# Jan-Celin/SCCG-genome-compression

Measured on AMD Instinct MI355X. Metric: target bases compressed/sec at 1/2/4/8 GPUs; bit-exact record stream vs CPU ref, higher is better.
Workload: dtype u8

## Files before the change

### sccg-genome-compression_amd/csrc/common.h

```cpp
#pragma once

#include <hip/hip_runtime.h>
#include <stdint.h>

#define SCCG_WAVE 64
#define SCCG_BLOCK 256

__host__ __device__ __forceinline__ bool c_isspace(uint8_t c) { return c == ' ' || (c >= 9 && c <= 13); }
__host__ __device__ __forceinline__ bool c_islower(uint8_t c) { return c >= 'a' && c <= 'z'; }
__host__ __device__ __forceinline__ uint8_t c_toupper(uint8_t c) { return c_islower(c) ? (uint8_t)(c - 32) : c; }
__host__ __device__ __forceinline__ uint8_t c_tolower(uint8_t c) { return (c >= 'A' && c <= 'Z') ? (uint8_t)(c + 32) : c; }
__host__ __device__ __forceinline__ uint32_t base2(uint8_t c) {
    return c == 'A' ? 0u : c == 'C' ? 1u : c == 'G' ? 2u : c == 'T' ? 3u : 4u;
}

#define KEY_EXOTIC 0x80000000u
__host__ __device__ __forceinline__ uint32_t exotic_key(const uint8_t* s, int k) {
    uint32_t h = 2166136261u;
    for (int i = 0; i < k; i++) { h ^= s[i]; h *= 16777619u; }
    return KEY_EXOTIC | (h & 0x7fffffffu);
}
__host__ __device__ __forceinline__ uint32_t kmer_key(const uint8_t* s, int k) {
    uint32_t code = 0;
    for (int i = 0; i < k; i++) {
        uint32_t b = base2(s[i]);
        if (b > 3) return exotic_key(s, k);
        code = (code << 2) | b;
    }
    return code;
}
__host__ __device__ __forceinline__ uint32_t slot_hash(uint32_t key, int bits) {
    return (key * 0x9E3779B1u) >> (32 - bits);
}
__host__ __device__ __forceinline__ int ndigits_u32(uint32_t v) {
    int n = 1;
    while (v >= 10) { v /= 10; n++; }
    return n;
}
__host__ __device__ __forceinline__ int ndigits_i32(int32_t v) {
    return v < 0 ? 1 + ndigits_u32((uint32_t)0 - (uint32_t)v) : ndigits_u32((uint32_t)v);
}
__device__ __forceinline__ int write_i32(uint8_t* dst, int32_t v) {
    uint32_t u = v < 0 ? (uint32_t)0 - (uint32_t)v : (uint32_t)v;
    int n = ndigits_u32(u) + (v < 0);
    int w = n;
    do { dst[--w] = (uint8_t)('0' + u % 10); u /= 10; } while (u);
    if (v < 0) dst[0] = '-';
    return n;
}

__device__ __forceinline__ uint32_t swar_codes(uint32_t w, uint32_t& diff) {
    const uint32_t c = ((w >> 1) ^ (w >> 2)) & 0x03030303u;
    diff = __builtin_amdgcn_perm(0x54474341u, 0x54474341u, c) ^ w;
    const uint32_t p = c | (c >> 6);
    return (p | (p >> 12)) & 0xffu;
}
__device__ __forceinline__ uint32_t nz_bytes(uint32_t diff) {
    const uint32_t nz = ((((diff & 0x7f7f7f7fu) + 0x7f7f7f7fu) | diff) & 0x80808080u) >> 7;
    return (nz | (nz >> 7) | (nz >> 14) | (nz >> 21)) & 0xfu;
}
template <int ND>
__device__ __forceinline__ void pack_codes(const uint32_t (&w)[ND], uint64_t& code, uint32_t& bad) {
    uint32_t d[ND], acc = 0;
    code = 0;
#pragma unroll
    for (int i = 0; i < ND; i++) {
        code |= (uint64_t)swar_codes(w[i], d[i]) << (8 * i);
        acc |= d[i];
    }
    bad = 0;
    if (acc) {
#pragma unroll
        for (int i = 0; i < ND; i++) bad |= nz_bytes(d[i]) << (4 * i);
    }
}
template <int ND>
__device__ __forceinline__ void loadw(const uint8_t* p, uint32_t (&o)[ND]) {
    const uint32_t sh = (uint32_t)((uintptr_t)p & 3);
    const uint32_t* w = reinterpret_cast<const uint32_t*>(p - sh);
    uint32_t v[ND + 1];
#pragma unroll
    for (int i = 0; i <= ND; i++) v[i] = w[i];
#pragma unroll
    for (int i = 0; i < ND; i++) o[i] = __builtin_amdgcn_alignbyte(v[i + 1], v[i], sh);
}
__device__ __forceinline__ uint32_t walk_key(const uint8_t* s, int k) {
    uint32_t code = 0;
    for (int i = 0; i < k; i++) {
        const uint32_t b = base2(s[i]);
        if (b > 3) return exotic_key(s, k);
        code |= b << (2 * i);
    }
    return code;
}

__device__ __forceinline__ int lane_id() { return (int)(threadIdx.x & 63); }
__device__ __forceinline__ int wave_in_block() { return (int)(threadIdx.x >> 6); }

__device__ __forceinline__ void wave_sync() {
    __builtin_amdgcn_fence(__ATOMIC_RELEASE, "wavefront");
    __builtin_amdgcn_wave_barrier();
    __builtin_amdgcn_fence(__ATOMIC_ACQUIRE, "wavefront");
}

template <typename T>
__device__ __forceinline__ T wave_incl_add(T v) {
    const int lane = lane_id();
#pragma unroll
    for (int d = 1; d < 64; d <<= 1) {
        T o = __shfl_up(v, d, 64);
        if (lane >= d) v += o;
    }
    return v;
}
__device__ __forceinline__ uint32_t wave_incl_add_dpp(uint32_t v) {
    v += (uint32_t)__builtin_amdgcn_update_dpp(0, (int)v, 0x111, 0xf, 0xf, true);
    v += (uint32_t)__builtin_amdgcn_update_dpp(0, (int)v, 0x112, 0xf, 0xf, true);
    v += (uint32_t)__builtin_amdgcn_update_dpp(0, (int)v, 0x114, 0xf, 0xf, true);
    v += (uint32_t)__builtin_amdgcn_update_dpp(0, (int)v, 0x118, 0xf, 0xf, true);
    v += (uint32_t)__builtin_amdgcn_update_dpp(0, (int)v, 0x142, 0xa, 0xf, false);
    v += (uint32_t)__builtin_amdgcn_update_dpp(0, (int)v, 0x143, 0xc, 0xf, false);
    return v;
}
template <typename T>
__device__ __forceinline__ T wave_sum(T v) {
#pragma unroll
    for (int d = 32; d > 0; d >>= 1) v += __shfl_xor(v, d, 64);
    return v;
}
template <typename T>
__device__ __forceinline__ T wave_max(T v) {
#pragma unroll
    for (int d = 32; d > 0; d >>= 1) { T o = __shfl_xor(v, d, 64); v = o > v ? o : v; }
    return v;
}
template <typename T>
__device__ __forceinline__ T wave_min(T v) {
#pragma unroll
    for (int d = 32; d > 0; d >>= 1) { T o = __shfl_xor(v, d, 64); v = o < v ? o : v; }
    return v;
}
__device__ __forceinline__ int first_lane(unsigned long long m) { return m ? __ffsll((long long)m) - 1 : 64; }
__device__ __forceinline__ int32_t uni(int32_t v) { return __builtin_amdgcn_readfirstlane(v); }
__device__ __forceinline__ int32_t lane_val(int32_t v, int l) { return __builtin_amdgcn_readlane(v, l); }
__device__ __forceinline__ uint32_t lane_val(uint32_t v, int l) { return (uint32_t)__builtin_amdgcn_readlane((int32_t)v, l); }

template <typename T>
__device__ __forceinline__ T block_excl_add(T v, T* tmp, T* total) {
    T incl = wave_incl_add(v);
    const int w = wave_in_block(), lane = lane_id();
    if (lane == 63) tmp[w] = incl;
    __syncthreads();
    if (threadIdx.x == 0) {
        T s = 0;
        for (int i = 0; i < (int)(blockDim.x >> 6); i++) { T t = tmp[i]; tmp[i] = s; s += t; }
        tmp[4] = s;
    }
    __syncthreads();
    T r = incl - v + tmp[w];
    if (total) *total = tmp[4];
    __syncthreads();
    return r;
}

#define SCCG_HIP(expr)                                              \
    do {                                                            \
        hipError_t e_ = (expr);                                     \
        if (e_ != hipSuccess) return sccg_hip_fail(e_, #expr, __FILE__, __LINE__); \
    } while (0)

int sccg_hip_fail(hipError_t e, const char* what, const char* file, int line);

static inline unsigned grid_for(int64_t n, int per_block) {
    int64_t g = (n + per_block - 1) / per_block;
    return (unsigned)(g < 1 ? 1 : g);
}
```

### sccg-genome-compression_amd/csrc/ingest.hip

```cpp
#include "internal.h"

namespace {

constexpr int PER_T = INGEST_TILE / SCCG_BLOCK;
constexpr int WPB = SCCG_BLOCK / 64;


constexpr int64_t FM_CHUNK = 16384;
template <int NW>
__device__ __forceinline__ uint8_t wb(const uint32_t (&w)[NW], int i) { return (uint8_t)(w[i >> 2] >> (8 * (i & 3))); }
template <int NW>
__device__ __forceinline__ void load_words(const uint8_t* __restrict__ buf, int64_t n, int64_t off, uint32_t (&w)[NW]);
__global__ __launch_bounds__(SCCG_BLOCK) void k_first_match(const uint8_t* __restrict__ buf, int64_t n,
                                                            const int64_t* __restrict__ from_slot, int mode, uint8_t c,
                                                            int64_t* __restrict__ res, unsigned int* __restrict__ ticket) {
    __shared__ int64_t s_cs;
    const int64_t from = from_slot ? *from_slot + 1 : 0;
    const int64_t base = from & ~(int64_t)63;
    constexpr int PER = FM_CHUNK / SCCG_BLOCK;
    for (;;) {
        if (threadIdx.x == 0) {
            const int64_t cs = base + (int64_t)atomicAdd(ticket, 1u) * FM_CHUNK;
            const int64_t best = (int64_t)__hip_atomic_load((unsigned long long*)res, __ATOMIC_RELAXED, __HIP_MEMORY_SCOPE_AGENT);
            s_cs = (cs >= n || cs >= best) ? -1 : cs;
// ... 198 lines not shown
        if (c == '(') par |= bit;
    }
    const uint64_t fk = ~drop;
    const int64_t lim = n - off;
    const uint64_t valid = lim >= 64 ? ~0ull : (lim > 0 ? (1ull << lim) - 1ull : 0ull);
    StripMasks r{0, 0, fk, par, -1, lo, nn, odd ? 1ull : 0ull};
    if (MODE == INGEST_TGT) {
        const int64_t lo = h - off < 0 ? 0 : (h - off > 64 ? 64 : h - off);
        const int64_t hi = he - off < 0 ? 0 : (he - off > 64 ? 64 : he - off);
        r.known = ~ws & valid & ~(below64((int)hi) & ~below64((int)lo));
        return r;
    }
    const uint64_t ls = ((nl << 1) | (uint64_t)(off == 0 || prev == '\n')) & valid;
    const int first = ls ? __builtin_ctzll(ls) : 64;
    r.unknown = ~ws & valid & below64(first);
    uint64_t keep = 0;
    if ((gt & ls) == 0) {
        keep = ~below64(first);
        r.last = ls ? 1 : -1;
    } else {
        uint64_t rem = ls;
        while (rem) {
            const int j = __builtin_ctzll(rem);
            rem &= rem - 1;
            const int nx = rem ? __builtin_ctzll(rem) : 64;
            const int32_t st = !((gt >> j) & 1ull);
            if (st) keep |= below64(nx) & ~below64(j);
            r.last = st;
        }
    }
    r.known = ~ws & valid & keep;
    return r;
}

template <IngestMode MODE, bool RUNS = false, bool ODD = false>
__device__ __forceinline__ StripMasks strip_tile(FilterMode fm, const uint8_t* __restrict__ buf, int64_t n, int64_t h,
                                                 int64_t he, int64_t off, uint32_t (&w)[SNW], int32_t& prior,
                                                 uint64_t& lsm, uint4* tin) {
    const int lane = lane_id();
    load_words<SNW>(buf, n, off, w);
    wave_sync();
#pragma unroll
    for (int q = 0; q < SNW / 4; q++) tin[4 * lane + q] = make_uint4(w[4 * q], w[4 * q + 1], w[4 * q + 2], w[4 * q + 3]);
    wave_sync();
    uint8_t prev = '\n';
    if (MODE == INGEST_REF) {
        const uint32_t up = (uint32_t)__shfl_up((int)w[SNW - 1], 1, 64) >> 24;
        prev = lane ? (uint8_t)up : ((off > 0 && off - 1 < n) ? buf[off - 1] : (uint8_t)'\n');
    }
    const StripMasks r = strip_masks<MODE, RUNS, ODD>(fm, w, prev, off, n, h, he, reinterpret_cast<const uint8_t*>(tin + 4 * lane));
    wave_sync();
    prior = -1;
    lsm = 0;
    if (MODE == INGEST_REF) {
        lsm = __ballot(r.last >= 0);
        const uint64_t m = lsm & below64(lane);
        const int src = m ? 63 - __builtin_clzll(m) : 0;
        const int32_t v = __shfl(r.last, src, 64);
        prior = m ? v : -1;
    }
    return r;
}

template <IngestMode MODE, bool KC>
__global__ __launch_bounds__(SCCG_BLOCK) void k_strip_summary(FilterMode fm, const uint8_t* __restrict__ buf, int64_t n,
                                                              const int64_t* __restrict__ hdr, int64_t* __restrict__ ta,
                                                              int64_t* __restrict__ tb, int64_t* __restrict__ tfa,
                                                              int64_t* __restrict__ tfb, int32_t* __restrict__ tlast,
                                                              uint16_t* __restrict__ kc, int32_t* __restrict__ kflag) {
    __shared__ uint4 tin_all[WPB][STRIP_WTILE / 16];
    const int64_t tile = (int64_t)blockIdx.x * WPB + wave_in_block();
    if (tile * STRIP_WTILE >= n) return;
    const int lane = lane_id();
    const int64_t off = tile * STRIP_WTILE + (int64_t)lane * SL;
    const int64_t h = MODE == INGEST_TGT ? hdr[0] : 0, he = MODE == INGEST_TGT ? hdr[1] : 0;
    uint32_t w[SNW];
    int32_t prior;
    uint64_t lsm;
    const StripMasks r = strip_tile<MODE, false, KC>(fm, buf, n, h, he, off, w, prior, lsm, tin_all[wave_in_block()]);
    if (KC) {
        const uint64_t hole = ~(r.known | (prior != 0 ? r.unknown : 0ull));
        const uint32_t h1 = hole ? (uint32_t)__builtin_ctzll(hole) : 64u, h2 = hole ? 63u - (uint32_t)__builtin_clzll(hole) : 64u;
        kc[tile * 64 + lane] = (uint16_t)(h1 | (h2 << 7));
        const uint64_t odd = __ballot(r.odd != 0 || __popcll(hole) > 2);
        const uint64_t sens = __ballot(MODE == INGEST_REF && prior < 0 && r.unknown != 0);
        if (lane == 0) kflag[tile] = (odd ? 0 : 1) | (sens ? 2 : 0);
    }
    const uint64_t ra = (uint64_t)__popcll(r.unknown), rb = (uint64_t)__popcll(r.known);
    const uint64_t rfa = (uint64_t)__popcll(r.unknown & r.fk), rfb = (uint64_t)__popcll(r.known & r.fk);
    const uint64_t A = prior < 0 ? ra : 0, B = rb + (prior == 1 ? ra : 0);
    const uint64_t FA = prior < 0 ? rfa : 0, FB = rfb + (prior == 1 ? rfa : 0);
    const uint32_t t_ab = lane_val(wave_incl_add_dpp((uint32_t)(A | (B << 16))), 63);
    const uint32_t t_f = lane_val(wave_incl_add_dpp((uint32_t)(FA | (FB << 16))), 63);
    const uint64_t tot = (uint64_t)t_ab | ((uint64_t)t_f << 32);
    if (lane == 0) {
        ta[tile] = (int64_t)(tot & 0xffff);
        tb[tile] = (int64_t)((tot >> 16) & 0xffff);
        tfa[tile] = (int64_t)((tot >> 32) & 0xffff);
        tfb[tile] = (int64_t)(tot >> 48);
    }
    if (MODE == INGEST_REF) {
        const int32_t last = lsm ? __shfl(r.last, 63 - __builtin_clzll(lsm), 64) : -1;
        if (lane == 0) tlast[tile] = last;
    } else if (lane == 0) {
        tlast[tile] = -1;
    }
}

struct TileSum {
    int64_t a, b, fa, fb;
    int32_t last;
};
__device__ __forceinline__ TileSum ts_compose(const TileSum& x, const TileSum& y) {
    TileSum r;
    r.a = x.a + (x.last < 0 ? y.a : 0);
    r.b = x.b + y.b + (x.last == 1 ? y.a : 0);
    r.fa = x.fa + (x.last < 0 ? y.fa : 0);
    r.fb = x.fb + y.fb + (x.last == 1 ? y.fa : 0);
    r.last = y.last >= 0 ? y.last : x.last;
    return r;
}
__device__ __forceinline__ TileSum ts_shfl_up(const TileSum& v, int d) {
    TileSum r;
    r.a = __shfl_up(v.a, d, 64); r.b = __shfl_up(v.b, d, 64);
    r.fa = __shfl_up(v.fa, d, 64); r.fb = __shfl_up(v.fb, d, 64);
    r.last = __shfl_up(v.last, d, 64);
    return r;
}

constexpr int SCAN_B = 1024;
__device__ __forceinline__ TileSum block_scan_tiles(TileSum v, TileSum* wsum, TileSum* total) {
    const TileSum id{0, 0, 0, 0, -1};
    const int lane = lane_id(), w = (int)(threadIdx.x >> 6), nw = (int)(blockDim.x >> 6);
    TileSum incl = v;
#pragma unroll
    for (int d = 1; d < 64; d <<= 1) {
        const TileSum o = ts_shfl_up(incl, d);
        if (lane >= d) incl = ts_compose(o, incl);
    }
    if (lane == 63) wsum[w] = incl;
    __syncthreads();
    if (threadIdx.x == 0) {
        TileSum run = id;
        for (int i = 0; i < nw; i++) { const TileSum x = wsum[i]; wsum[i] = run; run = ts_compose(run, x); }
        wsum[16] = run;
    }
    __syncthreads();
    TileSum ex = ts_shfl_up(incl, 1);
    if (lane == 0) ex = id;
    if (total) *total = wsum[16];
    return ts_compose(wsum[w], ex);
}

constexpr int SCAN_T = 1024, SCAN_PER = SCAN_B / SCAN_T;
__global__ __launch_bounds__(SCAN_T) void k_strip_scan_local(int64_t ntiles, int64_t* __restrict__ ta, int64_t* __restrict__ tb,
                                                          int64_t* __restrict__ tfa, int64_t* __restrict__ tfb,
                                                          int32_t* __restrict__ tlast, TileSum* __restrict__ btot) {
    __shared__ TileSum wsum[17];
    const TileSum id{0, 0, 0, 0, -1};
    const int64_t t0 = (int64_t)blockIdx.x * SCAN_B + (int64_t)threadIdx.x * SCAN_PER;
    TileSum v[SCAN_PER], agg = id;
#pragma unroll
    for (int k = 0; k < SCAN_PER; k++) {
        const int64_t t = t0 + k;
        v[k] = t < ntiles ? TileSum{ta[t], tb[t], tfa[t], tfb[t], tlast[t]} : id;
        agg = ts_compose(agg, v[k]);
    }
    TileSum tot;
    TileSum run = block_scan_tiles(agg, wsum, &tot);
#pragma unroll
    for (int k = 0; k < SCAN_PER; k++) {
        const int64_t t = t0 + k;
        if (t < ntiles) { ta[t] = run.a; tb[t] = run.b; tfa[t] = run.fa; tfb[t] = run.fb; tlast[t] = run.last; }
        run = ts_compose(run, v[k]);
    }
    if (threadIdx.x == 0) btot[blockIdx.x] = tot;
}

__global__ __launch_bounds__(SCAN_T) void k_strip_scan_blocks(int64_t nblk, TileSum* __restrict__ btot) {
    __shared__ TileSum wsum[17];
    const TileSum id{0, 0, 0, 0, -1};
    const int64_t i0 = (int64_t)threadIdx.x * SCAN_PER;
    TileSum v[SCAN_PER], agg = id;
#pragma unroll
    for (int k = 0; k < SCAN_PER; k++) {
        v[k] = i0 + k < nblk ? btot[i0 + k] : id;
        agg = ts_compose(agg, v[k]);
    }
    TileSum tot;
    TileSum run = block_scan_tiles(agg, wsum, &tot);
#pragma unroll
    for (int k = 0; k < SCAN_PER; k++) {
        if (i0 + k < nblk) btot[i0 + k] = run;
        run = ts_compose(run, v[k]);
    }
    if (threadIdx.x == 0) btot[SCAN_B] = tot;
}

__global__ void k_strip_scan_apply(int64_t ntiles, const int64_t* __restrict__ ta, const int64_t* __restrict__ tb,
                                   const int64_t* __restrict__ tfa, const int64_t* __restrict__ tfb,
                                   const int32_t* __restrict__ tlast, const TileSum* __restrict__ btot,
                                   int64_t* __restrict__ toff, int64_t* __restrict__ toff2, int32_t* __restrict__ tcarry,
                                   int64_t* __restrict__ d_len, int64_t* __restrict__ d_len2) {
    const TileSum start{0, 0, 0, 0, 1};
    for (int64_t t = (int64_t)blockIdx.x * blockDim.x + threadIdx.x; t < ntiles; t += (int64_t)gridDim.x * blockDim.x) {
        const TileSum r = ts_compose(ts_compose(start, btot[t / SCAN_B]), TileSum{ta[t], tb[t], tfa[t], tfb[t], tlast[t]});
        toff[t] = r.b;
        toff2[t] = r.fb;
        tcarry[t] = r.last;
    }
    if (blockIdx.x == 0 && threadIdx.x == 0) {
        const TileSum r = ts_compose(start, btot[SCAN_B]);
        *d_len = r.b;
        if (d_len2) *d_len2 = r.fb;
    }
}

__device__ __forceinline__ void run_events(uint64_t p, uint64_t K, uint32_t cin, uint64_t& st, uint64_t& en) {
    const uint64_t D = ~K;
    const uint64_t x = p & K;
    const uint64_t sd = ((x << 1) | cin) & D;
    const uint64_t g = x | (D & ~(D + sd));
    const uint64_t prev = (g << 1) | cin;
    st = K & g & ~prev;
    en = K & ~g & prev;
}

template <IngestMode MODE, bool RUNS>
__global__ __launch_bounds__(SCCG_BLOCK) void k_strip_write(FilterMode fm, const uint8_t* __restrict__ buf, int64_t n,
                                                            const int64_t* __restrict__ hdr,
                                                            const int64_t* __restrict__ toff,
                                                            const int64_t* __restrict__ toff2,
                                                            const int32_t* __restrict__ tcarry,
                                                            uint8_t* __restrict__ out, uint8_t* __restrict__ out2,
                                                            int32_t* __restrict__ flags, RunSlots rsl,
                                                            const uint16_t* __restrict__ kc, const int32_t* __restrict__ kflag) {
    __shared__ uint4 stage_all4[WPB][(STAGE_WORDS + 3) / 4];
    __shared__ uint32_t tab[16];
    if (threadIdx.x < 16) tab[threadIdx.x] = compact_sel(threadIdx.x);
    __syncthreads();
    const int64_t tile = (int64_t)blockIdx.x * WPB + wave_in_block();
    if (tile * STRIP_WTILE >= n) return;
    const int lane = lane_id();
    uint32_t* st4 = reinterpret_cast<uint32_t*>(stage_all4[wave_in_block()]);
    uint8_t* s1 = reinterpret_cast<uint8_t*>(st4);
    const int64_t off = tile * STRIP_WTILE + (int64_t)lane * SL;
    const int64_t h = MODE == INGEST_TGT ? hdr[0] : 0, he = MODE == INGEST_TGT ? hdr[1] : 0;
    uint32_t w[SNW];
    int32_t prior;
    uint64_t lsm;
    StripMasks r;
    const int32_t kf = kc ? uni(kflag[tile]) : 0;
    if ((kf & 1) && (MODE == INGEST_TGT || !(kf & 2) || uni(tcarry[tile]) == 1)) {
        load_words<SNW>(buf, n, off, w);
        const uint32_t code = kc[tile * 64 + lane], h1 = code & 127u, h2 = code >> 7;
        const uint64_t keep = ~((h1 < 64 ? 1ull << h1 : 0ull) | (h2 < 64 ? 1ull << h2 : 0ull));
        r = StripMasks{keep, 0ull, ~0ull, 0ull, -1, RUNS ? lower_fast(w) : 0ull, 0ull, 0ull};
        prior = 1;
    } else {
        r = strip_tile<MODE, RUNS>(fm, buf, n, h, he, off, w, prior, lsm, stage_all4[wave_in_block()]);
        if (MODE == INGEST_REF && prior < 0) prior = tcarry[tile];
    }
    const uint64_t keep = r.known | (prior == 1 ? r.unknown : 0ull), fkeep = keep & r.fk;
    const uint32_t c = (uint32_t)__popcll(keep) | ((uint32_t)__popcll(fkeep) << 16);
    const uint32_t incl = wave_incl_add_dpp(c), tot = lane_val(incl, 63);
    const uint32_t ex = incl - c;
    if (RUNS) {
        const bool has = keep != 0;
        const int fb = has ? __builtin_ctzll(keep) : 0, lb = has ? 63 - __builtin_clzll(keep) : 0;
        const uint32_t first2 = (uint32_t)((r.lower >> fb) & 1u) | ((uint32_t)((r.nn >> fb) & 1u) << 1);
        const uint32_t last2 = (uint32_t)((r.lower >> lb) & 1u) | ((uint32_t)((r.nn >> lb) & 1u) << 1);
        const uint64_t hm = __ballot(has);
        const uint64_t before = hm & below64(lane);
        const int src = before ? 63 - __builtin_clzll(before) : 0;
        const uint32_t pl = (uint32_t)__shfl((int)last2, src, 64);
        const uint32_t cin = before ? pl : first2;
        uint64_t sl = 0, el = 0, sn = 0, en = 0;
        if (has) {
            run_events(r.lower, keep, cin & 1u, sl, el);
            run_events(r.nn, keep, cin >> 1, sn, en);
        }
        const uint64_t cc = (uint64_t)__popcll(sl) | ((uint64_t)__popcll(el) << 16) | ((uint64_t)__popcll(sn) << 32) |
                            ((uint64_t)__popcll(en) << 48);
        const uint32_t ci_lo = wave_incl_add_dpp((uint32_t)cc), ci_hi = wave_incl_add_dpp((uint32_t)(cc >> 32));
        const uint64_t ci = (uint64_t)ci_lo | ((uint64_t)ci_hi << 32);
        const uint64_t ct = (uint64_t)lane_val(ci_lo, 63) | ((uint64_t)lane_val(ci_hi, 63) << 32);
        const uint64_t cx = ci - cc;
        const int fl = hm ? first_lane(hm) : 0, ll = hm ? 63 - __builtin_clzll(hm) : 0;
        const uint32_t tf = (uint32_t)__shfl((int)first2, fl, 64), tl = (uint32_t)__shfl((int)last2, ll, 64);
        if (lane == 0) {
            rsl.rc[tile] = ct;
            rsl.rf[tile] = (hm ? 1 : 0) | (int32_t)(tf << 1) | (int32_t)(tl << 3);
        }
        if ((sl | el | sn | en) != 0) {
            const int64_t o0 = toff[tile] + (int64_t)(ex & 0xffff);
            int32_t* const dst[4] = {rsl.sl, rsl.el, rsl.sn, rsl.en};
            const uint64_t ev[4] = {sl, el, sn, en};
#pragma unroll
            for (int q = 0; q < 4; q++) {
                uint32_t at = (uint32_t)(cx >> (16 * q)) & 0xffffu;
                for (uint64_t m = ev[q]; m; m &= m - 1) {
                    const int b = __builtin_ctzll(m);
                    if (at < RUN_SLOT) dst[q][(size_t)tile * RUN_SLOT + at] = (int32_t)(o0 + __popcll(keep & below64(b)));
                    else atomicOr(rsl.ovf, 1);
                    at++;
                }
            }
        }
    }
    if (flags && __ballot((keep & r.par) != 0) && lane == 0) atomicOr(flags, 1);
    if (out) {
        stage_lane<false>(s1, tab, w, keep, (int)(ex & 0xffff));
        wave_sync();
        stage_out(st4, (int)(tot & 0xffff), out, toff[tile]);
    }
    if (out2) {
        if (out && !__ballot(fkeep != keep)) {
            stage_out<true>(st4, (int)(tot >> 16), out2, toff2[tile]);
        } else {
            wave_sync();
            stage_lane<true>(s1, tab, w, fkeep, (int)(ex >> 16));
            wave_sync();
            stage_out(st4, (int)(tot >> 16), out2, toff2[tile]);
        }
    }
}

template <IngestMode MODE>
__global__ __launch_bounds__(64) void k_strip_gather(const uint8_t* __restrict__ buf, int64_t n,
                                                     const int64_t* __restrict__ hdr, const int64_t* __restrict__ toff,
                                                     const int32_t* __restrict__ tcarry, const int64_t* __restrict__ d_len,
                                                     const int32_t* __restrict__ segs, uint8_t* __restrict__ dst) {
    __shared__ uint4 tin[STRIP_WTILE / 16];
    const int lane = lane_id();
    const int32_t seg = segs[blockIdx.x];
    if (seg < 0) return;
    const int64_t len = *d_len;
    const int64_t q0 = (int64_t)seg * SEG_L;
    const int64_t q1 = q0 + SEG_L < len ? q0 + SEG_L : len;
    uint8_t* out = dst + (size_t)blockIdx.x * SEG_GATHER_B;
    if (q0 >= q1) return;
    const int64_t ntiles = (n + STRIP_WTILE - 1) / STRIP_WTILE;
    int64_t lo = 0, hi = ntiles - 1;
    while (lo < hi) {
        const int64_t span = hi - lo;
        const int64_t p = lo + (span * (lane + 1) + 63) / 64;
        const bool le = p <= hi && toff[p] <= q0;
        const unsigned long long m = __ballot(le);
        if (!m) { hi = lo + (span + 63) / 64 - 1; if (hi < lo) hi = lo; continue; }
        const int l = 63 - __builtin_clzll(m);
        const int64_t pl = lo + (span * (l + 1) + 63) / 64;
        const int64_t pn = l < 63 ? lo + (span * (l + 2) + 63) / 64 - 1 : hi;
        lo = pl;
        hi = pn < hi ? pn : hi;
        if (hi < lo) hi = lo;
    }
    const int64_t h = MODE == INGEST_TGT ? hdr[0] : 0, he = MODE == INGEST_TGT ? hdr[1] : 0;
    for (int64_t tile = lo; tile < ntiles && toff[tile] < q1; tile++) {
        const int64_t off = tile * STRIP_WTILE + (int64_t)lane * SL;
        uint32_t w[SNW];
        int32_t prior;
        uint64_t lsm;
        const StripMasks r = strip_tile<MODE>(FILTER_UPPER, buf, n, h, he, off, w, prior, lsm, tin);
        int32_t pr = prior;
        if (MODE == INGEST_REF && pr < 0) pr = tcarry[tile];
        const uint64_t keep = r.known | (pr == 1 ? r.unknown : 0ull);
        const uint32_t c = (uint32_t)__popcll(keep);
        const uint32_t ex = wave_incl_add<uint32_t>(c) - c;
        int64_t pos = toff[tile] + ex;
        if (pos < q1 && pos + c > q0) {
            for (uint64_t m = keep; m; m &= m - 1, pos++) {
                const int b = __builtin_ctzll(m);
                if (pos >= q0 && pos < q1) out[pos - q0] = (uint8_t)(w[b >> 2] >> (8 * (b & 3)));
            }
        }
        wave_sync();
    }
}

__device__ __forceinline__ bool run_pred(RunPred p, uint8_t c) {
    return p == RUN_LOWER ? c_islower(c) : (c == 'N' || c == 'n');
}

__device__ __forceinline__ void pred_masks(const uint8_t* __restrict__ in, int64_t n, int64_t off, uint32_t& ml,
                                           uint32_t& mn) {
    uint32_t w[PER_T / 4];
    load_words(in, n, off, w);
    ml = 0;
    mn = 0;
#pragma unroll
    for (int q = 0; q < PER_T / 4; q++) {
        const uint32_t x = w[q];
        ml |= sw_bits(sw_lt(x, 'z' + 1) & ~sw_lt(x, 'a')) << (4 * q);
        mn |= sw_bits(sw_eq(x, 'N') | sw_eq(x, 'n')) << (4 * q);
    }
}

__global__ __launch_bounds__(SCCG_BLOCK) void k_runs_count(const uint8_t* __restrict__ in, int64_t n,
                                                           int64_t* __restrict__ cnt_l, int64_t* __restrict__ cnt_n) {
    __shared__ int32_t tmp32[8];
    const int64_t off = (int64_t)blockIdx.x * INGEST_TILE + (int64_t)threadIdx.x * PER_T;
    uint32_t ml, mn;
    pred_masks(in, n, off, ml, mn);
    const bool in_prev = off > 0 && off - 1 < n;
    const uint32_t pl = in_prev && run_pred(RUN_LOWER, in[off - 1]), pn = in_prev && run_pred(RUN_N, in[off - 1]);
    const int32_t c = __popc(ml & ~((ml << 1) | pl)) | (__popc(mn & ~((mn << 1) | pn)) << 16);
    int32_t tot;
    block_excl_add<int32_t>(c, tmp32, &tot);
    if (threadIdx.x == 0) { cnt_l[blockIdx.x] = tot & 0xffff; cnt_n[blockIdx.x] = tot >> 16; }
}

__device__ __forceinline__ void put_positions(uint32_t bits, int64_t off, int32_t* __restrict__ dst, int64_t at) {
    while (bits) {
        dst[at++] = (int32_t)(off + __ffs((int)bits) - 1);
        bits &= bits - 1;
    }
}

__global__ __launch_bounds__(SCCG_BLOCK) void k_runs_write(const uint8_t* __restrict__ in, int64_t n,
                                                           const int64_t* __restrict__ toff_l,
                                                           const int64_t* __restrict__ toff_n, int32_t* __restrict__ rs_l,
                                                           int32_t* __restrict__ re_l, int32_t* __restrict__ rs_n,
                                                           int32_t* __restrict__ re_n) {
    __shared__ int32_t tmp32[8];
    const int64_t tile0 = (int64_t)blockIdx.x * INGEST_TILE;
    const int64_t off = tile0 + (int64_t)threadIdx.x * PER_T;
    uint32_t ml, mn;
    pred_masks(in, n, off, ml, mn);
    const bool in_prev = off > 0 && off - 1 < n, in_next = off + PER_T < n;
    const uint32_t pl = in_prev && run_pred(RUN_LOWER, in[off - 1]), pn = in_prev && run_pred(RUN_N, in[off - 1]);
    const uint32_t nl = in_next && run_pred(RUN_LOWER, in[off + PER_T]), nn = in_next && run_pred(RUN_N, in[off + PER_T]);
    const uint32_t sl = ml & ~((ml << 1) | pl), el = ml & ~((ml >> 1) | (nl << 31));
    const uint32_t sn = mn & ~((mn << 1) | pn), en = mn & ~((mn >> 1) | (nn << 31));
    const bool t_in = tile0 > 0 && tile0 < n;
    const bool open_l = t_in && run_pred(RUN_LOWER, in[tile0 - 1]) && run_pred(RUN_LOWER, in[tile0]);
    const bool open_n = t_in && run_pred(RUN_N, in[tile0 - 1]) && run_pred(RUN_N, in[tile0]);
    const int32_t xs = block_excl_add<int32_t>(__popc(sl) | (__popc(sn) << 16), tmp32, nullptr);
    const int32_t xe = block_excl_add<int32_t>(__popc(el) | (__popc(en) << 16), tmp32, nullptr);
    put_positions(sl, off, rs_l, toff_l[blockIdx.x] + (xs & 0xffff));
    put_positions(el, off, re_l, toff_l[blockIdx.x] - (open_l ? 1 : 0) + (xe & 0xffff));
    put_positions(sn, off, rs_n, toff_n[blockIdx.x] + (xs >> 16));
    put_positions(en, off, re_n, toff_n[blockIdx.x] - (open_n ? 1 : 0) + (xe >> 16));
}

constexpr int RUNS_LOOKBACK = 64;
__global__ void k_runs_tiles(int64_t ntiles, const uint64_t* __restrict__ rc, const int32_t* __restrict__ rf,
                             int64_t* __restrict__ cs, int64_t* __restrict__ ce, int32_t* __restrict__ bev,
                             int32_t* __restrict__ ovf) {
    for (int64_t t = (int64_t)blockIdx.x * blockDim.x + threadIdx.x; t < ntiles; t += (int64_t)gridDim.x * blockDim.x) {
        const int32_t f = rf[t];
        const uint64_t c = rc[t];
        int32_t b = 0;
        if (f & 1) {
            uint32_t prev = 0;
            int64_t q = t - 1;
            for (; q >= 0 && t - q <= RUNS_LOOKBACK; q--) {
                const int32_t g = rf[q];
                if (g & 1) { prev = (uint32_t)(g >> 3) & 3u; break; }
            }
            if (q >= 0 && t - q > RUNS_LOOKBACK) atomicOr(ovf, 2);
            const uint32_t first = (uint32_t)(f >> 1) & 3u;
#pragma unroll
            for (int p = 0; p < 2; p++) {
                const uint32_t fp = (first >> p) & 1u, pp = (prev >> p) & 1u;
                if (fp && !pp) b |= 1 << (2 * p);
                if (!fp && pp) b |= 2 << (2 * p);
            }
        }
        bev[t] = b;
        cs[t] = (int64_t)((c & 0xffff) + (b & 1)) | ((int64_t)(((c >> 32) & 0xffff) + ((b >> 2) & 1)) << 32);
        ce[t] = (int64_t)(((c >> 16) & 0xffff) + ((b >> 1) & 1)) | ((int64_t)((c >> 48) + ((b >> 3) & 1)) << 32);
    }
}

__global__ void k_runs_copy(int64_t ntiles, const int64_t* __restrict__ toff, const uint64_t* __restrict__ rc,
                            const int32_t* __restrict__ bev, const int64_t* __restrict__ cs, const int64_t* __restrict__ ce,
                            RunSlots rsl, int32_t* __restrict__ rs_l, int32_t* __restrict__ re_l,
                            int32_t* __restrict__ rs_n, int32_t* __restrict__ re_n) {
    for (int64_t t = (int64_t)blockIdx.x * blockDim.x + threadIdx.x; t < ntiles; t += (int64_t)gridDim.x * blockDim.x) {
        const uint64_t c = rc[t];
        const int32_t b = bev[t];
        const int32_t t0 = (int32_t)toff[t];
        const size_t sb = (size_t)t * RUN_SLOT;
        int32_t* const dst[4] = {rs_l, re_l, rs_n, re_n};
        const int32_t* const src[4] = {rsl.sl, rsl.el, rsl.sn, rsl.en};
        const int64_t base[4] = {cs[t] & 0xffffffff, ce[t] & 0xffffffff, cs[t] >> 32, ce[t] >> 32};
#pragma unroll
        for (int q = 0; q < 4; q++) {
            const int end = q & 1;
            int64_t at = base[q];
            if ((b >> q) & 1) dst[q][at++] = t0 - end;
            const int nq = (int)((c >> (16 * q)) & 0xffff);
            for (int k = 0; k < nq && k < RUN_SLOT; k++) dst[q][at++] = src[q][sb + k] - end;
        }
    }
}

__global__ void k_runs_fin(const int64_t* __restrict__ tot, const int64_t* __restrict__ d_nT, int32_t* __restrict__ re_l,
                           int32_t* __restrict__ re_n, int64_t* __restrict__ d_nruns) {
    const int64_t sl = tot[0] & 0xffffffff, sn = tot[0] >> 32, el = tot[1] & 0xffffffff, en = tot[1] >> 32;
    if (sl > el) re_l[sl - 1] = (int32_t)(*d_nT - 1);
    if (sn > en) re_n[sn - 1] = (int32_t)(*d_nT - 1);
    d_nruns[0] = sl;
    d_nruns[1] = sn;
}

__device__ __forceinline__ int64_t run_text_len(int32_t d, int32_t len, bool at_end) {
    return len == 1 ? (int64_t)ndigits_i32(d) + (at_end ? 0 : 1) : (int64_t)(3 + ndigits_i32(d) + ndigits_i32(len));
}

__global__ void k_run_textlen(const int32_t* __restrict__ rs, const int32_t* __restrict__ re, int64_t nr,
                              int64_t n, int64_t* __restrict__ len) {
    for (int64_t r = (int64_t)blockIdx.x * blockDim.x + threadIdx.x; r < nr; r += (int64_t)gridDim.x * blockDim.x) {
        const int32_t d = rs[r] - (r ? rs[r - 1] : 0);
        len[r] = run_text_len(d, re[r] - rs[r] + 1, (int64_t)re[r] == n - 1);
    }
}

__global__ void k_run_textwrite(const int32_t* __restrict__ rs, const int32_t* __restrict__ re, int64_t nr,
                                int64_t n, const int64_t* __restrict__ off, uint8_t* __restrict__ out) {
    for (int64_t r = (int64_t)blockIdx.x * blockDim.x + threadIdx.x; r < nr; r += (int64_t)gridDim.x * blockDim.x) {
        const int32_t d = rs[r] - (r ? rs[r - 1] : 0);
        const int32_t len = re[r] - rs[r] + 1;
        uint8_t* o = out + off[r];
        if (len == 1) {
            o += write_i32(o, d);
            if ((int64_t)re[r] != n - 1) *o = ',';
        } else {
            *o++ = '(';
            o += write_i32(o, d);
            *o++ = ',';
            o += write_i32(o, len);
            *o = ')';
        }
    }
}

}

constexpr int FH_T = 256, FH_PER = 64;
__global__ __launch_bounds__(FH_T) void k_find_header(const uint8_t* __restrict__ buf, int64_t n, int64_t* __restrict__ d_sc) {
    __shared__ unsigned long long s_hit;
    int64_t res[2] = {n, n};
    for (int ph = 0; ph < 2; ph++) {
        if (ph == 1 && res[0] >= n) break;
        const int64_t from = ph == 0 ? 0 : res[0] + 1;
        for (int64_t cs = from & ~(int64_t)63; cs < n; cs += (int64_t)FH_T * FH_PER) {
            if (threadIdx.x == 0) s_hit = ~0ull;
            __syncthreads();
            const int64_t p0 = cs + (int64_t)threadIdx.x * FH_PER;
            if (p0 < n) {
                uint32_t w[FH_PER / 4];
                load_words<FH_PER / 4>(buf, n, p0, w);
                uint8_t prev = p0 > 0 ? buf[p0 - 1] : (uint8_t)'\n';
                int64_t hit = -1;
#pragma unroll
                for (int i = 0; i < FH_PER; i++) {
                    const uint8_t c = wb(w, i);
                    const int64_t p = p0 + i;
                    const bool ok = p >= from && p < n && (ph == 0 ? (c == '>' && prev == '\n') : c == '\n');
                    if (ok && hit < 0) hit = p;
                    prev = c;
                }
                if (hit >= 0) atomicMin(&s_hit, (unsigned long long)hit);
            }
            __syncthreads();
            const unsigned long long h = s_hit;
            __syncthreads();
            if (h != ~0ull) { res[ph] = (int64_t)h; break; }
        }
    }
    if (threadIdx.x == 0) { d_sc[0] = res[0]; d_sc[1] = res[1]; d_sc[2] = 0; d_sc[3] = 0; }
}

int launch_first_match(const uint8_t* buf, int64_t n, const int64_t* from_slot, int mode, uint8_t c, int64_t* res,
                       int64_t* ticket_slot, hipStream_t s) {
    int rc = dev_set_i64(res, 1, {n}, s);
    if (!rc) rc = dev_set_i64(ticket_slot, 1, {0}, s);
    if (rc) return rc;
    if (n > 0) {
        hipLaunchKernelGGL(k_first_match, dim3(64), dim3(SCCG_BLOCK), 0, s, buf, n, from_slot, mode, c, res,
                           reinterpret_cast<unsigned int*>(ticket_slot));
        SCCG_HIP(hipGetLastError());
    }
    return 0;
}

int launch_find_header(const uint8_t* buf, int64_t n, int64_t* d_sc, hipStream_t s) {
    hipLaunchKernelGGL(k_find_header, dim3(1), dim3(FH_T), 0, s, buf, n, d_sc);
    SCCG_HIP(hipGetLastError());
    return 0;
}

int launch_fasta_strip(IngestMode mode, const uint8_t* buf, int64_t n, const int64_t* d_header, uint8_t* out,
                       int64_t* d_len, int32_t* d_flags, const IngestScratch& sc, hipStream_t s, FilterMode fmode,
                       uint8_t* out2, int64_t* d_len2, const RunSlots* runs) {
    if (n <= 0) {
        SCCG_HIP(hipMemsetAsync(d_len, 0, sizeof(int64_t), s));
        if (d_len2) SCCG_HIP(hipMemsetAsync(d_len2, 0, sizeof(int64_t), s));
        return 0;
    }
    if (!out2) fmode = FILTER_UPPER;
    const int64_t ntiles = (n + STRIP_TILE - 1) / STRIP_TILE;
    const unsigned g = grid_for(ntiles, WPB);
    uint16_t* const kc = sc.keep_cache;
    int32_t* const kf = sc.keep_flag;
#define SUMMARY(M, K)                                                                                                   \
    hipLaunchKernelGGL((k_strip_summary<M, K>), dim3(g), dim3(SCCG_BLOCK), 0, s, fmode, buf, n, d_header, sc.tile_a,   \
                       sc.tile_b, sc.tile_fa, sc.tile_fb, sc.tile_last, kc, kf)
    if (mode == INGEST_TGT && kc) SUMMARY(INGEST_TGT, true);
    else if (mode == INGEST_TGT) SUMMARY(INGEST_TGT, false);
    else if (kc) SUMMARY(INGEST_REF, true);
    else SUMMARY(INGEST_REF, false);
#undef SUMMARY
    const int64_t nblk = (ntiles + SCAN_B - 1) / SCAN_B;
    if (nblk > SCAN_B) return SCCG_E_UNSUPPORTED;
    TileSum* btot = reinterpret_cast<TileSum*>(sc.block_sums);
    hipLaunchKernelGGL(k_strip_scan_local, dim3((unsigned)nblk), dim3(SCAN_T), 0, s, ntiles, sc.tile_a, sc.tile_b,
                       sc.tile_fa, sc.tile_fb, sc.tile_last, btot);
    hipLaunchKernelGGL(k_strip_scan_blocks, dim3(1), dim3(SCAN_T), 0, s, nblk, btot);
    hipLaunchKernelGGL(k_strip_scan_apply, dim3(grid_for(ntiles, 256)), dim3(256), 0, s, ntiles, sc.tile_a, sc.tile_b,
                       sc.tile_fa, sc.tile_fb, sc.tile_last, btot, sc.tile_off, sc.tile_off2, sc.tile_carry, d_len,
                       d_len2);
    const RunSlots rsl = runs ? *runs : RunSlots{};
    if (mode == INGEST_TGT && runs)
        PROF_LAUNCH(PROF_STRIP, s, (k_strip_write<INGEST_TGT, true>), dim3(g), dim3(SCCG_BLOCK), 0, s, fmode, buf, n, d_header,
                    sc.tile_off, sc.tile_off2, sc.tile_carry, out, out2, d_flags, rsl, (const uint16_t*)kc, (const int32_t*)kf);
    else if (mode == INGEST_TGT)
        PROF_LAUNCH(PROF_STRIP, s, (k_strip_write<INGEST_TGT, false>), dim3(g), dim3(SCCG_BLOCK), 0, s, fmode, buf, n, d_header,
                    sc.tile_off, sc.tile_off2, sc.tile_carry, out, out2, d_flags, rsl, (const uint16_t*)kc, (const int32_t*)kf);
    else
        PROF_LAUNCH(PROF_STRIP, s, (k_strip_write<INGEST_REF, false>), dim3(g), dim3(SCCG_BLOCK), 0, s, fmode, buf, n, d_header,
                    sc.tile_off, sc.tile_off2, sc.tile_carry, out, out2, d_flags, rsl, (const uint16_t*)kc, (const int32_t*)kf);
    SCCG_HIP(hipGetLastError());
    return 0;
}

int launch_runs2(const uint8_t* in, int64_t n, int32_t* rs_l, int32_t* re_l, int32_t* rs_n, int32_t* re_n,
                 int64_t* d_nruns, int64_t* d_cnt_l, int64_t* d_cnt_n, int64_t* d_partial, hipStream_t s) {
    if (n <= 0) {
        SCCG_HIP(hipMemsetAsync(d_nruns, 0, 2 * sizeof(int64_t), s));
        return 0;
    }
    const int64_t ntiles = (n + INGEST_TILE - 1) / INGEST_TILE;
    hipLaunchKernelGGL(k_runs_count, dim3((unsigned)ntiles), dim3(SCCG_BLOCK), 0, s, in, n, d_cnt_l, d_cnt_n);
    int rc = dev_excl_sum(d_cnt_l, d_cnt_l, ntiles, d_nruns, d_partial, s);
    if (!rc) rc = dev_excl_sum(d_cnt_n, d_cnt_n, ntiles, d_nruns + 1, d_partial, s);
    if (rc) return rc;
    PROF_LAUNCH(PROF_RUNS, s, k_runs_write, dim3((unsigned)ntiles), dim3(SCCG_BLOCK), 0, s, in, n,
                (const int64_t*)d_cnt_l, (const int64_t*)d_cnt_n, rs_l, re_l, rs_n, re_n);
    SCCG_HIP(hipGetLastError());
    return 0;
}

int launch_runs_from_strip(const RunSlots& rs, int64_t ntiles, const int64_t* toff, const int64_t* d_nT, int32_t* rs_l,
                           int32_t* re_l, int32_t* rs_n, int32_t* re_n, int64_t* d_nruns, int64_t* cs, int64_t* ce,
                           int32_t* bev, int64_t* d_tot, int64_t* d_partial, hipStream_t s) {
    const unsigned g = grid_for(ntiles, 256) > 4096 ? 4096 : grid_for(ntiles, 256);
    hipLaunchKernelGGL(k_runs_tiles, dim3(g), dim3(256), 0, s, ntiles, (const uint64_t*)rs.rc, (const int32_t*)rs.rf, cs, ce,
                       bev, rs.ovf);
    if (const int rc = dev_excl_sum2(cs, cs, d_tot, ce, ce, d_tot + 1, ntiles, d_partial, s)) return rc;
    PROF_LAUNCH(PROF_RUNS, s, k_runs_copy, dim3(g), dim3(256), 0, s, ntiles, toff, (const uint64_t*)rs.rc, (const int32_t*)bev,
                (const int64_t*)cs, (const int64_t*)ce, rs, rs_l, re_l, rs_n, re_n);
    hipLaunchKernelGGL(k_runs_fin, dim3(1), dim3(1), 0, s, (const int64_t*)d_tot, d_nT, re_l, re_n, d_nruns);
    SCCG_HIP(hipGetLastError());
    return 0;
}

int launch_run_text(const int32_t* rs, const int32_t* re, int64_t nruns, int64_t n, uint8_t* out, int64_t* d_len,
                    int64_t* d_tmp, int64_t* d_partial, hipStream_t s) {
    if (nruns <= 0) {
        SCCG_HIP(hipMemsetAsync(d_len, 0, sizeof(int64_t), s));
        return 0;
    }
    const unsigned g = grid_for(nruns, 256) > 4096 ? 4096 : grid_for(nruns, 256);
    hipLaunchKernelGGL(k_run_textlen, dim3(g), dim3(256), 0, s, rs, re, nruns, n, d_tmp);
    int rc = dev_excl_sum(d_tmp, d_tmp, nruns, d_len, d_partial, s);
    if (rc) return rc;
    PROF_LAUNCH(PROF_RUNTEXT, s, k_run_textwrite, dim3(g), dim3(256), 0, s, rs, re, nruns, n, (const int64_t*)d_tmp, out);
    SCCG_HIP(hipGetLastError());
    return 0;
}

int launch_strip_gather(IngestMode mode, const uint8_t* buf, int64_t n, const int64_t* d_header, const int64_t* toff,
                        const int32_t* tcarry, const int64_t* d_len, const int32_t* segs, int nslots, uint8_t* dst,
                        hipStream_t s) {
    if (n <= 0 || nslots <= 0) return 0;
    if (mode == INGEST_TGT)
        hipLaunchKernelGGL(k_strip_gather<INGEST_TGT>, dim3(nslots), dim3(64), 0, s, buf, n, d_header, toff, tcarry, d_len,
                           segs, dst);
    else
        hipLaunchKernelGGL(k_strip_gather<INGEST_REF>, dim3(nslots), dim3(64), 0, s, buf, n, d_header, toff, tcarry, d_len,
                           segs, dst);
    SCCG_HIP(hipGetLastError());
    return 0;
}

int launch_strip_rewrite(IngestMode mode, const uint8_t* buf, int64_t n, const int64_t* d_header, uint8_t* out,
                         const IngestScratch& sc, hipStream_t s) {
    if (n <= 0) return 0;
    const int64_t ntiles = (n + STRIP_TILE - 1) / STRIP_TILE;
    const unsigned g = grid_for(ntiles, WPB);
    const RunSlots rsl{};
    if (mode == INGEST_TGT)
        PROF_LAUNCH(PROF_STRIP, s, (k_strip_write<INGEST_TGT, false>), dim3(g), dim3(SCCG_BLOCK), 0, s, FILTER_UPPER, buf, n,
                    d_header, sc.tile_off, sc.tile_off2, sc.tile_carry, out, (uint8_t*)nullptr, (int32_t*)nullptr, rsl,
                    (const uint16_t*)nullptr, (const int32_t*)nullptr);
    else
        PROF_LAUNCH(PROF_STRIP, s, (k_strip_write<INGEST_REF, false>), dim3(g), dim3(SCCG_BLOCK), 0, s, FILTER_UPPER, buf, n,
                    d_header, sc.tile_off, sc.tile_off2, sc.tile_carry, out, (uint8_t*)nullptr, (int32_t*)nullptr, rsl,
                    (const uint16_t*)nullptr, (const int32_t*)nullptr);
    SCCG_HIP(hipGetLastError());
    return 0;
}
```

### sccg-genome-compression_amd/csrc/internal.h

```cpp
#pragma once

#include "common.h"
#include "../../include/sccg.h"

enum ProfId {
    PROF_STRIP = 0,
    PROF_RUNS,
    PROF_RUNTEXT,
    PROF_LOCAL14,
    PROF_LOCAL10,
    PROF_LOCAL_EMIT,
    PROF_FILTER,
    PROF_ANCHOR,
    PROF_WALK,
    PROF_PRESENCE,
    PROF_FULLC,
    PROF_MATCH_EMIT,
    PROF_WALK_CHAIN,
    PROF_DC_DECODE,
    PROF_DC_FORMAT,
    PROF_WALK_CARRY,
    PROF_FETCH,
    PROF_COUNT
};
void prof_begin(hipStream_t s, int id);
void prof_end(hipStream_t s, int id);
#define PROF_LAUNCH(id, strm, ...)        \
    do {                                  \
        prof_begin(strm, id);             \
        hipLaunchKernelGGL(__VA_ARGS__);  \
        prof_end(strm, id);               \
    } while (0)

#include <initializer_list>
struct RbItem {
    const void* src;
    void* dst;
    int bytes;
};
int dev_readback(const RbItem* items, int n, hipStream_t s);
int dev_set_i64(int64_t* p, int n, std::initializer_list<int64_t> vals, hipStream_t s);
int dev_set_i32(int32_t* p, int n, std::initializer_list<int32_t> vals, hipStream_t s);
int dev_put_bytes(uint8_t* p, const char* bytes, int n, hipStream_t s);
int dev_put_frame(uint8_t* out, const uint8_t* hdr, int64_t hlen, int64_t total, hipStream_t s);
int dev_put_framed(uint8_t* dst, const uint8_t* src, int64_t n, char pre, char post, hipStream_t s);
int64_t scan_partials_needed(int64_t n);
int dev_excl_sum(const int64_t* in, int64_t* out, int64_t n, int64_t* d_total, int64_t* d_partial,
                 hipStream_t s);
int dev_excl_sum2(const int64_t* in0, int64_t* out0, int64_t* d_total0, const int64_t* in1, int64_t* out1,
                  int64_t* d_total1, int64_t n, int64_t* d_partial, hipStream_t s);
int dev_excl_max(const int64_t* in, int64_t* out, int64_t n, int64_t* d_total, int64_t* d_partial,
                 hipStream_t s);

constexpr int INGEST_TILE = 8192;
constexpr int STRIP_TILE = 4096;
enum IngestMode { INGEST_REF = 0, INGEST_TGT = 1 };
enum FilterMode { FILTER_DROP_N_UPPER = 0, FILTER_DROP_UPPERN_ONLY = 1, FILTER_UPPER = 2 };
enum RunPred { RUN_LOWER = 0, RUN_N = 1 };

struct IngestScratch {
    int64_t* tile_a;
    int64_t* tile_b;
    int64_t* tile_fa;
    int64_t* tile_fb;
    int32_t* tile_last;
    int64_t* tile_off;
    int64_t* tile_off2;
    int32_t* tile_carry;
    void* block_sums;
    int64_t* scalars;
    uint16_t* keep_cache = nullptr;
    int32_t* keep_flag = nullptr;
};

int launch_find_header(const uint8_t* buf, int64_t n, int64_t* d_scalars, hipStream_t s);
int launch_first_match(const uint8_t* buf, int64_t n, const int64_t* from_slot, int mode, uint8_t c, int64_t* res,
                       int64_t* ticket_slot, hipStream_t s);
constexpr int RUN_SLOT = 32;
struct RunSlots {
    int32_t* sl = nullptr;
    int32_t* el = nullptr;
    int32_t* sn = nullptr;
    int32_t* en = nullptr;
    uint64_t* rc = nullptr;
    int32_t* rf = nullptr;
    int32_t* ovf = nullptr;
};
int launch_runs_from_strip(const RunSlots& rs, int64_t ntiles, const int64_t* toff, const int64_t* d_nT, int32_t* rs_l,
                           int32_t* re_l, int32_t* rs_n, int32_t* re_n, int64_t* d_nruns, int64_t* cs, int64_t* ce,
                           int32_t* bev, int64_t* d_tot, int64_t* d_partial, hipStream_t s);
int launch_fasta_strip(IngestMode mode, const uint8_t* buf, int64_t n, const int64_t* d_header,
                       uint8_t* out, int64_t* d_len, int32_t* d_flags, const IngestScratch& sc,
                       hipStream_t s, FilterMode fmode = FILTER_UPPER, uint8_t* out2 = nullptr,
                       int64_t* d_len2 = nullptr, const RunSlots* runs = nullptr);
constexpr int SEG_GATHER_B = 1024;
int launch_strip_gather(IngestMode mode, const uint8_t* buf, int64_t n, const int64_t* d_header, const int64_t* toff,
                        const int32_t* tcarry, const int64_t* d_len, const int32_t* segs, int nslots, uint8_t* dst,
                        hipStream_t s);
int launch_strip_rewrite(IngestMode mode, const uint8_t* buf, int64_t n, const int64_t* d_header, uint8_t* out,
                         const IngestScratch& sc, hipStream_t s);
int launch_runs2(const uint8_t* s_in, int64_t n, int32_t* rs_l, int32_t* re_l, int32_t* rs_n, int32_t* re_n,
                 int64_t* d_nruns, int64_t* d_cnt_l, int64_t* d_cnt_n, int64_t* d_partial, hipStream_t s);
int launch_run_text(const int32_t* run_s, const int32_t* run_e, int64_t nruns, int64_t n,
                    uint8_t* out, int64_t* d_len, int64_t* d_tmp, int64_t* d_partial, hipStream_t s);

constexpr int SEG_L = 1000;
constexpr int SEG_REC_CAP = 256;
struct SegStat {
    int32_t nrec;
    int32_t nmatch;
    int32_t lit;
    int32_t pass;
    int32_t non_n;
    int32_t first_p;
    int32_t last_p;
    int32_t pad;
};
constexpr int32_t PASS_PROVEN = -1;
int launch_local_proven(const uint8_t* R, int64_t nR, const uint8_t* T, int64_t nT, int64_t iters, uint32_t* recs,
                        SegStat* stat, hipStream_t s);
int launch_local_pass(int k, int pass, int upper, const uint8_t* R, int64_t nR, const uint8_t* T, int64_t nT, int64_t seg0,
                      int64_t seg_end, uint32_t* recs, SegStat* stat, hipStream_t s);
int launch_local_all(const uint8_t* R, const int64_t* d_nR, const uint8_t* T, const int64_t* d_nT, int64_t nseg_max,
                     uint32_t* recs, SegStat* stat, int32_t* cls, int32_t gen, int32_t* ctl, hipStream_t s);
constexpr int PROBE_PAIRS = 16 * 8;
int local_probe_applies(int64_t nseg_max);
int launch_probe_segs(const int64_t* d_nR, const int64_t* d_nT, int32_t* segs, hipStream_t s);
int launch_segment_copy(const uint8_t* src, const int64_t* d_len, const int32_t* segs, int nslots, uint8_t* dst,
                        hipStream_t s);
int launch_local_probe(const uint8_t* gR, const int64_t* d_nR, const uint8_t* gT, const int64_t* d_nT, const int32_t* segs,
                       int32_t* pout, hipStream_t s);
int local_probe_window(const int32_t* pout);
int launch_local_emit(const uint8_t* T, int64_t nT, int64_t iters, const uint32_t* recs,
                      const SegStat* stat, uint8_t* out, int64_t* d_len, int64_t* d_tmp_a,
                      int64_t* d_tmp_b, int64_t* d_partial, hipStream_t s, bool abs_p = false);

struct WalkWorkspace;
struct WalkResult {
    int64_t n_matches;
    int64_t rounds;
    int64_t chunks;
    int64_t chains;
};
size_t walk_workspace_bytes(int64_t nR, int64_t nT, int k, int chunk);
int global_prepare(const uint8_t* Rp, int64_t nRp, const uint8_t* Tp, int64_t nTp, int k, int m, int chunk, void* ws,
                   size_t ws_bytes, hipStream_t s);
void global_prepare_reset();
void walk_forget_workspace(const void* ws);
int global_sweep_early(const uint8_t* Rp, int64_t nRp_bound, const int64_t* d_nRp, const uint8_t* tgt_fa, int64_t tn,
                       const int64_t* d_hdr, int k, int m, int chunk, void* ws, size_t ws_bytes, hipStream_t s);
struct EmitTarget {
    int (*resolve)(void* user, uint8_t** out);
    void* user;
    int (*abandon)(void* user) = nullptr;
    int (*round1_queued)(void* user, hipStream_t s) = nullptr;
};
constexpr int WALK_ABANDONED = -1;
int global_match_and_emit(const uint8_t* Rp, int64_t nRp, const uint8_t* Tp, int64_t nTp, int k, int m,
                          int chunk, void* ws, size_t ws_bytes, uint8_t* out, int64_t* out_len,
                          WalkResult* res, hipStream_t s, bool abs_p = false, const EmitTarget* late_out = nullptr,
                          bool keep_flat = true);
int global_walk_range(const uint8_t* Rp, int64_t nRp, const uint8_t* Tp, int64_t nTp, int k, int m, int chunk, void* ws,
                      size_t ws_bytes, int64_t x0, int64_t P0, int64_t x_end, int64_t* exit_x, int64_t* exit_P,
                      WalkResult* res, hipStream_t s);
int global_matches(void* ws, const int32_t** t, const int32_t** p, const int32_t** l, int64_t* n);

size_t delta_workspace_bytes(int64_t n);
int delta_encode_dev(const uint8_t* X, int64_t n, uint8_t* out, int64_t out_cap, int64_t* out_len,
                     bool* stoi_fail, void* ws, hipStream_t s);
```

### sccg-genome-compression_amd/csrc/sccg_api.cpp

```cpp
#include <algorithm>
#include <hip/hip_runtime.h>

#include <fcntl.h>
#include <sys/stat.h>
#include <unistd.h>

#include <atomic>
#include <chrono>
#include <condition_variable>
#include <cstdarg>
#include <cstdio>
#include <cstdlib>
#include <cstring>
#include <functional>
#include <future>
#include <mutex>
#include <string>
#include <thread>
#include <vector>

#include "decomp.h"
#include "internal.h"

static thread_local char g_hip_err[512];

int sccg_hip_fail(hipError_t e, const char* what, const char* file, int line) {
    snprintf(g_hip_err, sizeof g_hip_err, "%s:%d: %s -> %s", file, line, what, hipGetErrorString(e));
    return e == hipErrorOutOfMemory ? SCCG_E_NOMEM : SCCG_E_HIP;
}

namespace {

enum Slot {
    B_RFA, B_TFA, B_R, B_T, B_TILE_A, B_TILE_B, B_TILE_FA, B_TILE_FB, B_TILE_LAST, B_TILE_OFF, B_TILE_OFF2, B_TILE_CARRY, B_TILE_BSUM,
    B_SCAL, B_PARTIAL,
    B_RUN_S, B_RUN_E, B_TMP64, B_RUN_SN, B_RUN_EN, B_TMP64N, B_NLINE, B_RECS, B_STAT, B_SEGCLS, B_SEG_A, B_SEG_B, B_RP, B_TP, B_WALK, B_OUT,
    B_D_LP, B_D_FLAG, B_D_DLT, B_D_CONTRIB, B_D_OFF, B_D_DSUM, B_D_LS, B_D_LL, B_D_LC, B_D_NS, B_D_NL, B_D_NC, B_D_DEC, B_D_FIDX, B_D_NLPOS, B_D_LP2, B_D_DLT2, B_PARTIAL2,
    B_DX, B_DELTA,
    B_TILE2_A, B_TILE2_B, B_TILE2_FA, B_TILE2_FB, B_TILE2_LAST, B_TILE2_OFF, B_TILE2_OFF2, B_TILE2_CARRY, B_TILE2_BSUM,
    B_RSLOT = 62, B_RTILE,
    B_COUNT
};
static_assert(B_RSLOT == 62 && B_D_DEC == 43 && B_COUNT <= 64, "SCCG_TEST_OOM slot numbers moved");

constexpr int WALK_CHUNK_MIN = 16384, WALK_CHUNK_MAX = 32768;
constexpr int64_t WALK_CHUNKS_TARGET = 7800;
int walk_chunk(int64_t target_bytes) {
    static const int env = [] {
        const char* e = getenv("SCCG_WALK_CHUNK");
        const int c = e ? atoi(e) : 0;
        return c >= 1024 && c <= (1 << 20) ? c : 0;
    }();
    if (env) return env;
    const int64_t c = (target_bytes / WALK_CHUNKS_TARGET) & ~int64_t(4095);
    return (int)(c < WALK_CHUNK_MIN ? WALK_CHUNK_MIN : c > WALK_CHUNK_MAX ? WALK_CHUNK_MAX : c);
}
constexpr int DPAD = 4096;

bool oom_slot(int slot) {
    static const uint64_t mask = [] {
        uint64_t m = 0;
        const char* e = getenv("SCCG_TEST_OOM");
        while (e && *e) {
            char* end = nullptr;
            const long v = strtol(e, &end, 10);
            if (end == e) break;
            if (v >= 0 && v < 64) m |= 1ull << v;
            e = *end ? end + 1 : end;
        }
        return m;
    }();
    static std::atomic<uint64_t> failed{0};
    if (slot < 0 || slot >= 64 || !((mask >> slot) & 1)) return false;
    return !((failed.fetch_or(1ull << slot) >> slot) & 1);
}

}

struct HostWorker {
    std::thread th;
    std::mutex mu;
    std::condition_variable cv;
    std::function<int()> task;
    bool has_task = false, done = true, quit = false;
    int rc = 0;

    void start(int device) {
        th = std::thread([this, device] {
            (void)hipSetDevice(device);
            std::unique_lock<std::mutex> lk(mu);
            for (;;) {
                cv.wait(lk, [this] { return has_task || quit; });
                if (quit) return;
                std::function<int()> f = std::move(task);
                has_task = false;
                lk.unlock();
                const int r = f();
                lk.lock();
                rc = r;
                done = true;
                cv.notify_all();
            }
        });
    }
    void submit(std::function<int()> f) {
        std::lock_guard<std::mutex> lk(mu);
        task = std::move(f);
        has_task = true;
        done = false;
        cv.notify_all();
    }
    int wait() {
        std::unique_lock<std::mutex> lk(mu);
        cv.wait(lk, [this] { return done; });
        return rc;
    }
    void stop() {
        if (!th.joinable()) return;
        {
            std::lock_guard<std::mutex> lk(mu);
            quit = true;
            cv.notify_all();
        }
        th.join();
    }
};

struct sccg_ctx {
    int device = 0;
    HostWorker worker;
    hipStream_t stream = nullptr;
    hipStream_t side = nullptr;
    hipStream_t side2 = nullptr;
    hipEvent_t ev_fork = nullptr, ev_fork2 = nullptr, ev_join = nullptr, ev_lines = nullptr, ev_rstrip = nullptr, ev_hdr = nullptr, ev_tstrip = nullptr,
               ev_local = nullptr, ev_probe = nullptr;
    int64_t* h_switch = nullptr;
    int32_t* h_probe = nullptr;
    std::string err;
    sccg_stats stats{};
    void* buf[B_COUNT] = {};
    size_t cap[B_COUNT] = {};
    uint8_t* stage[16] = {};
    hipEvent_t stage_ev[16] = {};
    hipStream_t copy_ref = nullptr, copy_tgt = nullptr;
    hipEvent_t ev_ref_in = nullptr, ev_tgt_in = nullptr;
    void* cls_buf = nullptr;
    size_t cls_cap = 0;
    int32_t cls_gen = 0;
    bool exact_switch = false;

    int fail(int rc, const char* fmt, ...) {
        char tmp[512];
        va_list ap;
        va_start(ap, fmt);
        vsnprintf(tmp, sizeof tmp, fmt, ap);
        va_end(ap);
        err = tmp;
        return rc;
    }
    int hipfail(int rc) {
        err = g_hip_err;
        return rc;
    }
    void* get(int slot, size_t bytes) {
        bytes = (bytes + DPAD + 255) & ~(size_t)255;
        if (cap[slot] >= bytes) return buf[slot];
        if (buf[slot]) { walk_forget_workspace(buf[slot]); (void)hipFree(buf[slot]); }
        buf[slot] = nullptr;
        cap[slot] = 0;
        void* p = nullptr;
        if (oom_slot(slot)) bytes = (size_t)1 << 62;
        if (hipMalloc(&p, bytes) != hipSuccess) {
            (void)hipGetLastError();
            return nullptr;
        }
        buf[slot] = p;
        cap[slot] = bytes;
        return p;
    }
};

constexpr int REF_ERASED = 0, REF_KEPT = 1;
struct sccg_reference {
    sccg_ctx* ctx = nullptr;
    void* mem[2] = {nullptr, nullptr};
    size_t bytes[2] = {0, 0};
    int64_t holds = 1;
    const int64_t* d_len(int form) const {
        return reinterpret_cast<const int64_t*>(reinterpret_cast<const uint8_t*>(mem[form]) + bytes[form] - 256);
    }
};

struct sccg_reader {
    sccg_ctx* ctx = nullptr;
    sccg_reference* ref = nullptr;
    size_t mem_bytes = 0;
    void* mem = nullptr;
    DcFetchSrc src{};
    int64_t length = 0;
    std::string header;
    void* d_reg = nullptr;
    int64_t* h_reg = nullptr;
    size_t reg_cap = 0;
    void* d_out = nullptr;
    size_t out_cap = 0;
};

struct sccg_cohort {
    sccg_ctx* ctx = nullptr;
    std::vector<int64_t> length;
    void* d_tab = nullptr;
    void* d_reg = nullptr;
    int64_t* h_reg = nullptr;
    size_t reg_cap = 0;
    void* d_out = nullptr;
    size_t out_cap = 0;
};

#define TRY(expr)                                  \
    do {                                           \
        int rc_ = (expr);                          \
        if (rc_) return ctx->hipfail(rc_);         \
    } while (0)
#define HIPTRY(expr)                               \
    do {                                           \
        hipError_t e_ = (expr);                    \
        if (e_ != hipSuccess) return ctx->hipfail(sccg_hip_fail(e_, #expr, __FILE__, __LINE__)); \
    } while (0)
#define GET(T, var, slot, n)                                                            \
    T* var = reinterpret_cast<T*>(ctx->get(slot, (size_t)(n) * sizeof(T)));            \
    if (!var) return ctx->fail(SCCG_E_NOMEM, "device allocation of %zu bytes failed", (size_t)(n) * sizeof(T))

extern "C" {

int sccg_ctx_create(int device, sccg_ctx** out) {
    if (!out) return SCCG_E_INVALID;
    *out = nullptr;
    int n = 0;
    if (hipGetDeviceCount(&n) != hipSuccess || n <= 0) return SCCG_E_HIP;
    if (device < 0 || device >= n) return SCCG_E_INVALID;
    if (hipSetDevice(device) != hipSuccess) return SCCG_E_HIP;
    sccg_ctx* c = new sccg_ctx();
    c->device = device;
    int prio_lo = 0, prio_hi = 0;
    (void)hipDeviceGetStreamPriorityRange(&prio_lo, &prio_hi);
    if (hipStreamCreateWithFlags(&c->stream, hipStreamNonBlocking) != hipSuccess ||
        hipStreamCreateWithPriority(&c->side, hipStreamNonBlocking, prio_lo) != hipSuccess ||
        hipStreamCreateWithFlags(&c->side2, hipStreamNonBlocking) != hipSuccess ||
        hipEventCreateWithFlags(&c->ev_fork, hipEventDisableTiming) != hipSuccess ||
        hipEventCreateWithFlags(&c->ev_fork2, hipEventDisableTiming) != hipSuccess ||
        hipEventCreateWithFlags(&c->ev_join, hipEventDisableTiming) != hipSuccess ||
        hipEventCreateWithFlags(&c->ev_lines, hipEventDisableTiming) != hipSuccess ||
        hipEventCreateWithFlags(&c->ev_tstrip, hipEventDisableTiming) != hipSuccess ||
        hipEventCreateWithFlags(&c->ev_rstrip, hipEventDisableTiming) != hipSuccess ||
        hipEventCreateWithFlags(&c->ev_hdr, hipEventDisableTiming) != hipSuccess ||
        hipEventCreateWithFlags(&c->ev_local, hipEventDisableTiming) != hipSuccess ||
        hipEventCreateWithFlags(&c->ev_probe, hipEventDisableTiming) != hipSuccess ||
        hipHostMalloc(reinterpret_cast<void**>(&c->h_probe), 2 * PROBE_PAIRS * sizeof(int32_t), hipHostMallocDefault) != hipSuccess ||
        hipHostMalloc(reinterpret_cast<void**>(&c->h_switch), 64, hipHostMallocDefault) != hipSuccess) {
        delete c;
        return SCCG_E_HIP;
    }
    c->worker.start(device);
    *out = c;
    return SCCG_OK;
}

void sccg_ctx_destroy(sccg_ctx* ctx) {
    if (!ctx) return;
    ctx->worker.stop();
    (void)hipSetDevice(ctx->device);
    (void)hipStreamSynchronize(ctx->stream);
    (void)hipStreamSynchronize(ctx->side);
    (void)hipStreamSynchronize(ctx->side2);
    for (int i = 0; i < B_COUNT; i++)
        if (ctx->buf[i]) { walk_forget_workspace(ctx->buf[i]); (void)hipFree(ctx->buf[i]); }
    (void)hipEventDestroy(ctx->ev_fork);
    (void)hipEventDestroy(ctx->ev_fork2);
    (void)hipEventDestroy(ctx->ev_join);
    (void)hipEventDestroy(ctx->ev_lines);
    (void)hipEventDestroy(ctx->ev_tstrip);
    (void)hipEventDestroy(ctx->ev_rstrip);
    (void)hipEventDestroy(ctx->ev_hdr);
    (void)hipEventDestroy(ctx->ev_local);
    if (ctx->ev_probe) (void)hipEventDestroy(ctx->ev_probe);
    if (ctx->h_probe) (void)hipHostFree(ctx->h_probe);
    if (ctx->h_switch) (void)hipHostFree(ctx->h_switch);
    for (int i = 0; i < 16; i++) {
        if (ctx->stage[i]) (void)hipHostFree(ctx->stage[i]);
        if (ctx->stage_ev[i]) (void)hipEventDestroy(ctx->stage_ev[i]);
    }
    if (ctx->copy_ref) (void)hipStreamDestroy(ctx->copy_ref);
    if (ctx->copy_tgt) (void)hipStreamDestroy(ctx->copy_tgt);
    if (ctx->ev_ref_in) (void)hipEventDestroy(ctx->ev_ref_in);
    if (ctx->ev_tgt_in) (void)hipEventDestroy(ctx->ev_tgt_in);
    (void)hipStreamDestroy(ctx->side);
    (void)hipStreamDestroy(ctx->side2);
    (void)hipStreamDestroy(ctx->stream);
    delete ctx;
}

const char* sccg_last_error(const sccg_ctx* ctx) { return ctx ? ctx->err.c_str() : "null context"; }

int sccg_ctx_set_option(sccg_ctx* ctx, int option, int64_t value) {
    if (!ctx) return SCCG_E_INVALID;
    switch (option) {
        case SCCG_OPT_EXACT_SWITCH: ctx->exact_switch = value != 0; return SCCG_OK;
        default: return SCCG_E_INVALID;
    }
}

int sccg_last_stats(const sccg_ctx* ctx, sccg_stats* out) {
    if (!ctx || !out) return SCCG_E_INVALID;
    *out = ctx->stats;
    return SCCG_OK;
}

void sccg_buf_free(sccg_buf* b) {
    if (!b) return;
    free(b->data);
    b->data = nullptr;
    b->len = 0;
}

void sccg_records_free(sccg_records* r) {
    if (!r) return;
    free(r->kind); free(r->pos); free(r->len); free(r->t);
    memset(r, 0, sizeof *r);
}

size_t sccg_compress_bound(size_t ref_len, size_t tgt_len) {
    (void)ref_len;
    return 12 * tgt_len + 4096;
}

}

namespace {

int d2h_i64(sccg_ctx* ctx, const int64_t* d, int64_t* h, int n, hipStream_t s = nullptr) {
    const RbItem it{d, h, n * (int)sizeof(int64_t)};
    TRY(dev_readback(&it, 1, s ? s : ctx->stream));
    return 0;
}

int strip(sccg_ctx* ctx, IngestMode mode, const uint8_t* fa, int64_t n, const int64_t* d_hdr, uint8_t* out,
          int64_t* d_len, int32_t* d_flags, int64_t* h_len, FilterMode fmode = FILTER_UPPER, uint8_t* out2 = nullptr,
          int set = 0, hipStream_t s = nullptr, const RunSlots* runs = nullptr) {
    const int64_t ntiles = (n + STRIP_TILE - 1) / STRIP_TILE + 1;
    const int o = set ? B_TILE2_A - B_TILE_A : 0;
    static_assert(B_TILE_BSUM - B_TILE_A == B_TILE2_BSUM - B_TILE2_A, "scratch sets line up");
    IngestScratch sc;
    GET(int64_t, ta, B_TILE_A + o, ntiles);
    GET(int64_t, tb, B_TILE_B + o, ntiles);
    GET(int64_t, tfa, B_TILE_FA + o, ntiles);
    GET(int64_t, tfb, B_TILE_FB + o, ntiles);
    GET(int32_t, tl, B_TILE_LAST + o, ntiles);
    GET(int64_t, to, B_TILE_OFF + o, ntiles);
    GET(int64_t, to2, B_TILE_OFF2 + o, ntiles);
    GET(int32_t, tc, B_TILE_CARRY + o, ntiles);
    static const bool kc_on = [] { const char* e = getenv("SCCG_STRIP_KC"); return !e || atoi(e) > 0; }();
    constexpr int64_t KC_AT = 5152;
    GET(int64_t, bs, B_TILE_BSUM + o, kc_on ? KC_AT + ntiles * 16 + (ntiles + 1) / 2 : 1025 * 5);
    sc.tile_a = ta; sc.tile_b = tb; sc.tile_fa = tfa; sc.tile_fb = tfb; sc.tile_last = tl; sc.tile_off = to;
    sc.tile_off2 = to2; sc.tile_carry = tc; sc.block_sums = bs; sc.scalars = nullptr;
    if (kc_on) {
        sc.keep_cache = reinterpret_cast<uint16_t*>(bs + KC_AT);
        sc.keep_flag = reinterpret_cast<int32_t*>(bs + KC_AT + ntiles * 16);
    }
    TRY(launch_fasta_strip(mode, fa, n, d_hdr, out, d_len, d_flags, sc, s ? s : ctx->stream, fmode, out2,
                           out2 ? d_len + 1 : nullptr, runs));
    return h_len ? d2h_i64(ctx, d_len, h_len, out2 ? 2 : 1, s) : 0;
}

struct StripRuns {
    RunSlots rs;
    int64_t ntiles = 0;
    int64_t* cs = nullptr;
    int64_t* ce = nullptr;
    int32_t* bev = nullptr;
};
bool strip_runs(sccg_ctx* ctx, int64_t fa_len, StripRuns* out) {
    const int64_t nt = (fa_len + STRIP_TILE - 1) / STRIP_TILE + 1;
    const size_t slots = (size_t)nt * RUN_SLOT;
    uint8_t* a = reinterpret_cast<uint8_t*>(ctx->get(B_RSLOT, 4 * slots * 4 + (size_t)nt * 12 + 64));
    uint8_t* b = reinterpret_cast<uint8_t*>(ctx->get(B_RTILE, (size_t)nt * 20 + 64));
    if (!a || !b) return false;
    RunSlots& r = out->rs;
    r.sl = reinterpret_cast<int32_t*>(a);
    r.el = r.sl + slots;
    r.sn = r.el + slots;
    r.en = r.sn + slots;
    r.rc = reinterpret_cast<uint64_t*>(r.en + slots);
    r.rf = reinterpret_cast<int32_t*>(r.rc + nt);
    r.ovf = r.rf + nt;
    out->ntiles = (fa_len + STRIP_TILE - 1) / STRIP_TILE;
    out->cs = reinterpret_cast<int64_t*>(b);
    out->ce = out->cs + nt;
    out->bev = reinterpret_cast<int32_t*>(out->ce + nt);
    return true;
}

int run_lines(sccg_ctx* ctx, const uint8_t* s_in, int64_t n, uint8_t* out_lower, uint8_t** out_n, int64_t* d_sc,
              int64_t* h_lens, hipStream_t s, const StripRuns* sr = nullptr, const int64_t* toff = nullptr,
              const int64_t* d_n = nullptr, const std::function<int(hipStream_t)>& need_input = {}) {
    const int64_t maxruns = n / 2 + 2;
    const int64_t ntiles = (n + INGEST_TILE - 1) / INGEST_TILE + 1;
    const int64_t ntmp = maxruns > ntiles ? maxruns : ntiles;
    GET(int32_t, rs_l, B_RUN_S, maxruns);
    GET(int32_t, re_l, B_RUN_E, maxruns);
    GET(int64_t, tmp_l, B_TMP64, ntmp);
    GET(int32_t, rs_n, B_RUN_SN, maxruns);
    GET(int32_t, re_n, B_RUN_EN, maxruns);
    GET(int64_t, tmp_n, B_TMP64N, ntmp);
    const int64_t npart = ntmp > (sr ? sr->ntiles : 0) ? ntmp : sr->ntiles;
    GET(int64_t, part, B_PARTIAL, 2 * scan_partials_needed(npart) + 16);
    int64_t nruns[3] = {0, 0, 1};
    if (sr) {
        TRY(launch_runs_from_strip(sr->rs, sr->ntiles, toff, d_n, rs_l, re_l, rs_n, re_n, d_sc, sr->cs, sr->ce, sr->bev,
                                   d_sc + 4, part, s));
        int32_t ovf = 0;
        const RbItem it[2] = {{d_sc, nruns, 16}, {sr->rs.ovf, &ovf, 4}};
        TRY(dev_readback(it, 2, s));
        nruns[2] = ovf;
    }
    if (nruns[2]) {
        if (need_input) TRY(need_input(s));
        TRY(launch_runs2(s_in, n, rs_l, re_l, rs_n, re_n, d_sc, tmp_l, tmp_n, part, s));
        TRY(d2h_i64(ctx, d_sc, nruns, 2, s));
    }
    TRY(launch_run_text(rs_l, re_l, nruns[0], n, out_lower, d_sc + 2, tmp_l, part, s));
    GET(uint8_t, nline, B_NLINE, 24 * nruns[1] + 16);
    *out_n = nline;
    TRY(launch_run_text(rs_n, re_n, nruns[1], n, nline, d_sc + 3, tmp_n, part, s));
    return d2h_i64(ctx, d_sc + 2, h_lens, 2, s);
}

int paren_delta(sccg_ctx* ctx, const uint8_t* X, int64_t n, uint8_t* out, int64_t cap, int64_t* len, bool* stoi_fail) {
    void* ws = ctx->get(B_DELTA, delta_workspace_bytes(n));
    if (!ws) return ctx->fail(SCCG_E_NOMEM, "delta workspace of %zu bytes", delta_workspace_bytes(n));
    TRY(delta_encode_dev(X, n, out, cap, len, stoi_fail, ws, ctx->stream));
    return 0;
}

int check_params(sccg_ctx* ctx, const sccg_params& P) {
    if (P.m < 0 || 2 * P.m + 1 > 256)
        return ctx->fail(SCCG_E_UNSUPPORTED, "m = %d: the global walk's window takes 0 <= m <= 127", P.m);
    if (P.local) {
        if (P.k != 14 || P.k2 != 10 || P.L != SEG_L || P.T1 != 0.5f || P.T2 != 4)
            return ctx->fail(SCCG_E_UNSUPPORTED, "local = 1 takes the reference's k = 14, k2 = 10, L = 1000, T1 = 0.5, T2 = 4 "
                                                 "(use local = 0 for other k)");
    } else if (P.k < 1 || P.k > 32) {
        return ctx->fail(SCCG_E_UNSUPPORTED, "k = %d: the global walk takes 1 <= k <= 32", P.k);
    }
    return 0;
}

struct InputReady {
    int (*ref)(void* user, hipEvent_t* ev);
    int (*tgt)(void* user, hipEvent_t* ev);
    void* user;
};

int compress_device_impl(sccg_ctx* ctx, const sccg_params& P, const uint8_t* rfa, int64_t rn, const uint8_t* tfa,
                         int64_t tn, uint8_t* out, int64_t out_cap, int64_t* out_len, const InputReady* rdy = nullptr) {
    hipStream_t s = ctx->stream;
    if (const int rc = check_params(ctx, P)) return rc;
    const bool force_global = !P.local;
    const int kg = P.k, mg = P.m;
    sccg_stats st{};
    st.switch_segment = -1;
    const bool dbg = getenv("SCCG_DEBUG") != nullptr;
    auto t_last = std::chrono::steady_clock::now();
    auto mark = [&](const char* what) {
        if (!dbg) return;
        (void)hipStreamSynchronize(s);
        const auto t = std::chrono::steady_clock::now();
        fprintf(stderr, "[phase] %-14s %8.3f ms\n", what, std::chrono::duration<double, std::milli>(t - t_last).count());
        t_last = t;
    };
    GET(int64_t, sc, B_SCAL, 64);
    GET(uint8_t, T, B_T, tn + 64);
    GET(uint8_t, R, B_R, rn + 64);
    GET(uint8_t, Tp, B_TP, tn + 64);
    GET(uint8_t, Rp, B_RP, rn + 64);
    const int64_t iters_max = ((rn < tn ? rn : tn) + SEG_L - 1) / SEG_L;
    const bool probe_mode = !force_global && !ctx->exact_switch && iters_max > 0 && local_probe_applies(iters_max);
    const bool lean_R = probe_mode || force_global;
    int32_t* d_flags = reinterpret_cast<int32_t*>(sc + 32);
    HIPTRY(hipMemsetAsync(d_flags, 0, sizeof(int32_t), s));
    TRY(dev_set_i64(sc + 20, 2, {(int64_t)INT32_MAX << 32, (int64_t)INT32_MAX}, s));

    global_prepare_reset();
    HIPTRY(hipEventRecord(ctx->ev_fork, s));
    if (!rdy) TRY(launch_find_header(tfa, tn, sc, s));
    HIPTRY(hipStreamWaitEvent(ctx->side, ctx->ev_fork, 0));
    if (rdy) {
        hipEvent_t e = nullptr;
        if (const int rc = rdy->ref(rdy->user, &e)) return rc;
        HIPTRY(hipStreamWaitEvent(ctx->side, e, 0));
    }
    TRY(strip(ctx, INGEST_REF, rfa, rn, nullptr, lean_R ? nullptr : R, sc + 7, nullptr, nullptr, FILTER_DROP_N_UPPER, Rp, 1,
              ctx->side));
    HIPTRY(hipEventRecord(ctx->ev_rstrip, ctx->side));
    if (rdy) {
        hipEvent_t e = nullptr;
        if (const int rc = rdy->tgt(rdy->user, &e)) return rc;
        HIPTRY(hipStreamWaitEvent(s, e, 0));
        TRY(launch_find_header(tfa, tn, sc, s));
    }
    HIPTRY(hipEventRecord(ctx->ev_hdr, s));
    StripRuns sruns;
    const bool have_runs = strip_runs(ctx, tn, &sruns);
    if (have_runs) HIPTRY(hipMemsetAsync(sruns.rs.ovf, 0, sizeof(int32_t), s));
    const bool lean_T = lean_R && have_runs;
    TRY(strip(ctx, INGEST_TGT, tfa, tn, sc, lean_T ? nullptr : T, sc + 2, d_flags, nullptr, FILTER_DROP_N_UPPER, Tp, 0,
              nullptr, have_runs ? &sruns.rs : nullptr));
    auto rewrite = [&](IngestMode mode, hipStream_t st) -> int {
        const int o = mode == INGEST_REF ? B_TILE2_A - B_TILE_A : 0;
        IngestScratch isc{};
        isc.tile_off = reinterpret_cast<int64_t*>(ctx->buf[B_TILE_OFF + o]);
        isc.tile_off2 = reinterpret_cast<int64_t*>(ctx->buf[B_TILE_OFF2 + o]);
        isc.tile_carry = reinterpret_cast<int32_t*>(ctx->buf[B_TILE_CARRY + o]);
        return mode == INGEST_REF ? launch_strip_rewrite(INGEST_REF, rfa, rn, nullptr, R, isc, st)
                                  : launch_strip_rewrite(INGEST_TGT, tfa, tn, sc, T, isc, st);
    };
    HIPTRY(hipEventRecord(ctx->ev_tstrip, s));
    hipStream_t s3 = ctx->side2;
    HIPTRY(hipStreamWaitEvent(s3, ctx->ev_tstrip, 0));
    uint8_t* nline = nullptr;
    int64_t rl_len[2] = {0, 0};
    int64_t h4[4] = {0, 0, 0, 0}, lr[2] = {0, 0};
    HIPTRY(hipStreamWaitEvent(s3, ctx->ev_rstrip, 0));
    int32_t flags = 0;
    std::promise<int> lens_read;
    std::future<int> lens = lens_read.get_future();
    ctx->worker.submit([&, s3]() -> int {
        {
            const RbItem it[3] = {{sc, h4, (int)sizeof h4}, {d_flags, &flags, (int)sizeof flags}, {sc + 7, lr, (int)sizeof lr}};
            const int rc = dev_readback(it, 3, s3);
            lens_read.set_value(rc);
            if (rc) return ctx->hipfail(rc);
        }
        const bool hh = h4[0] < tn;
        const int64_t hl = hh ? h4[1] - h4[0] : 0;
        if (h4[2] >= INT32_MAX - 8 || out_cap < hl + 1 + 11 * h4[2] + 64) return 0;
        if (hh) {
            HIPTRY(hipMemcpyAsync(out, tfa + h4[0], (size_t)hl, hipMemcpyDeviceToDevice, s3));
            TRY(dev_put_bytes(out + hl, "\n", 1, s3));
        }
        TRY(run_lines(ctx, T, h4[2], out + (hh ? hl + 1 : 0), &nline, sc + 10, rl_len, s3, have_runs ? &sruns : nullptr,
                      reinterpret_cast<const int64_t*>(ctx->buf[B_TILE_OFF]), sc + 2,
                      lean_T ? std::function<int(hipStream_t)>([&](hipStream_t st) { return rewrite(INGEST_TGT, st); })
                             : std::function<int(hipStream_t)>()));
        HIPTRY(hipEventRecord(ctx->ev_lines, s3));
        return 0;
    });
    struct WorkerJoin {
        HostWorker* w;
        bool joined = false;
        int join() {
            if (joined) return 0;
            joined = true;
            return w->wait();
        }
        ~WorkerJoin() { join(); }
    } lines{&ctx->worker};
    const size_t wsb = walk_workspace_bytes(rn, tn, kg, walk_chunk(tn));
    if (rn < INT32_MAX - 8 && tn < INT32_MAX - 8) {
        HIPTRY(hipStreamWaitEvent(ctx->side, ctx->ev_hdr, 0));
        void* ws_early = ctx->get(B_WALK, wsb);
        if (!ws_early) return ctx->fail(SCCG_E_NOMEM, "walk workspace of %zu bytes", wsb);
        TRY(global_sweep_early(Rp, rn, sc + 8, tfa, tn, sc, kg, mg, walk_chunk(tn), ws_early, wsb, ctx->side));
    }
    HIPTRY(hipStreamWaitEvent(s, ctx->ev_rstrip, 0));
    hipStream_t s2 = ctx->side;
    HIPTRY(hipEventRecord(ctx->ev_fork, s));
    HIPTRY(hipStreamWaitEvent(s2, ctx->ev_fork, 0));
    GET(uint32_t, recs, B_RECS, (iters_max > 0 ? iters_max : 1) * SEG_REC_CAP);
    GET(SegStat, stat, B_STAT, iters_max > 0 ? iters_max : 1);
    constexpr int64_t PROBE_WORDS = 3 * PROBE_PAIRS + 2 * PROBE_PAIRS * SEG_GATHER_B / 4;
    GET(int32_t, cls, B_SEGCLS, (iters_max > 0 ? iters_max : 1) + PROBE_WORDS + 64);
    int32_t* probe_out = cls + (((iters_max > 0 ? iters_max : 1) + 63) & ~int64_t(63));
    int32_t* probe_segs = probe_out + 2 * PROBE_PAIRS;
    uint8_t* probe_gT = reinterpret_cast<uint8_t*>(probe_segs + PROBE_PAIRS);
    uint8_t* probe_gR = probe_gT + PROBE_PAIRS * SEG_GATHER_B;
    int32_t* ctl = reinterpret_cast<int32_t*>(sc + 20);
    bool probe_pending = false;
    auto launch_inorder = [&]() -> int {
        if (cls != ctx->cls_buf || ctx->cap[B_SEGCLS] != ctx->cls_cap || ctx->cls_gen >= (1 << 28)) {
            HIPTRY(hipMemsetAsync(cls, 0, ctx->cap[B_SEGCLS], s));
            ctx->cls_buf = cls;
            ctx->cls_cap = ctx->cap[B_SEGCLS];
            ctx->cls_gen = 0;
        }
        const int32_t gen = ++ctx->cls_gen;
        TRY(launch_local_all(R, sc + 7, T, sc + 2, iters_max, recs, stat, cls, gen, ctl, s));
        return 0;
    };
    if (probe_mode) {
        TRY(launch_probe_segs(sc + 7, sc + 2, probe_segs, s));
        if (lean_T) {
            TRY(launch_strip_gather(INGEST_TGT, tfa, tn, sc, reinterpret_cast<const int64_t*>(ctx->buf[B_TILE_OFF]),
                                    reinterpret_cast<const int32_t*>(ctx->buf[B_TILE_CARRY]), sc + 2, probe_segs,
                                    PROBE_PAIRS, probe_gT, s));
        } else {
            TRY(launch_segment_copy(T, sc + 2, probe_segs, PROBE_PAIRS, probe_gT, s));
        }
        TRY(launch_strip_gather(INGEST_REF, rfa, rn, nullptr, reinterpret_cast<const int64_t*>(ctx->buf[B_TILE2_OFF]),
                                reinterpret_cast<const int32_t*>(ctx->buf[B_TILE2_CARRY]), sc + 7, probe_segs,
                                PROBE_PAIRS, probe_gR, s));
        TRY(launch_local_probe(probe_gR, sc + 7, probe_gT, sc + 2, probe_segs, probe_out, s));
        HIPTRY(hipMemcpyAsync(ctx->h_probe, probe_out, 2 * PROBE_PAIRS * sizeof(int32_t), hipMemcpyDeviceToHost, s));
        HIPTRY(hipEventRecord(ctx->ev_probe, s));
        probe_pending = true;
    } else if (iters_max > 0 && !force_global) {
        TRY(launch_inorder());
    }
    TRY(lens.get());
    const int64_t hdr[2] = {h4[0], h4[1]}, lt[2] = {h4[2], h4[3]};
    const int64_t nT = lt[0], nR = lr[0];
    if (nT >= INT32_MAX - 8 || nR >= INT32_MAX - 8)
        return ctx->fail(SCCG_E_UNSUPPORTED, "sequence longer than the reference's int positions allow");
    const bool paren = (flags & 1) != 0;
    bool stoi_fail = false;
    st.target_bases = nT;
    st.reference_bases = nR;
    st.walk_reference_bases = lr[1];
    mark("ingest");
    const bool has_hdr = hdr[0] < tn;
    const int64_t hlen = has_hdr ? hdr[1] - hdr[0] : 0;
    if (out_cap < hlen + 1 + 11 * nT + 64) return ctx->fail(SCCG_E_INVALID, "output capacity too small");

    const int64_t nRs = (nR + SEG_L - 1) / SEG_L, nTs = (nT + SEG_L - 1) / SEG_L;
    const int64_t iters = nRs < nTs ? nRs : nTs;
    int64_t sw = -1;

    const int64_t np[2] = {lt[1], lr[1]};
    void* ws = ctx->get(B_WALK, wsb);
    if (!ws) return ctx->fail(SCCG_E_NOMEM, "walk workspace of %zu bytes", wsb);
    TRY(global_prepare(Rp, np[1], Tp, np[0], kg, mg, walk_chunk(tn), ws, wsb, s2));
    HIPTRY(hipEventRecord(ctx->ev_join, s2));

    int64_t pos = 0;
    auto join_lines = [&](hipStream_t on) -> int {
        TRY(lines.join());
        HIPTRY(hipStreamWaitEvent(on, ctx->ev_lines, 0));
        pos = (has_hdr ? hlen + 1 : 0) + rl_len[0];
        return 0;
    };

    bool sw_known = iters <= 0 || force_global;
    auto local_tail = [&]() -> int {
        if (iters > 0 && !force_global) HIPTRY(hipMemcpyAsync(ctx->h_switch, sc + 21, sizeof(int64_t), hipMemcpyDeviceToHost, s));
        HIPTRY(hipEventRecord(ctx->ev_local, s));
        return 0;
    };
    auto decide_probe = [&]() -> int {
        if (!probe_pending) return 0;
        probe_pending = false;
        HIPTRY(hipEventSynchronize(ctx->ev_probe));
        const int32_t w = local_probe_window(ctx->h_probe);
        if (w >= 0) {
            sw = w;
            sw_known = true;
            HIPTRY(hipEventRecord(ctx->ev_local, s));
            return 0;
        }
        if (lean_T) TRY(rewrite(INGEST_TGT, s));
        if (lean_R) TRY(rewrite(INGEST_REF, s));
        TRY(launch_inorder());
        return local_tail();
    };
    auto read_switch = [&]() -> int {
        TRY(decide_probe());
        if (sw_known) return 0;
        HIPTRY(hipEventSynchronize(ctx->ev_local));
        const int64_t h_sw = *ctx->h_switch;
        sw = h_sw >= INT32_MAX ? -1 : h_sw;
        sw_known = true;
        return 0;
    };
    if (!probe_pending) TRY(local_tail());

    bool global_done = false;
    int64_t g_rlen = 0;
    uint8_t* X = nullptr;
    WalkResult wr{};
    if (iters > 0 || force_global) {
        struct Late {
            std::function<int(uint8_t**)> f;
            std::function<int()> poll;
            static int call(void* u, uint8_t** o) { return static_cast<Late*>(u)->f(o); }
            static int abandon(void* u) { return static_cast<Late*>(u)->poll(); }
            std::function<int(hipStream_t)> r1;
            static int round1(void* u, hipStream_t st) { return static_cast<Late*>(u)->r1(st); }
        } late{[&](uint8_t** o) -> int {
                   TRY(read_switch());
                   if (sw < 0 && !force_global) return WALK_ABANDONED;
                   TRY(join_lines(s2));
                   const int64_t nlen = rl_len[1];
                   TRY(dev_put_framed(out + pos, nline, nlen, '\n', '\n', s2));
                   pos += nlen + 2;
                   X = out + pos;
                   if (paren) {
                       GET(uint8_t, xb, B_DX, out_cap - pos);
                       X = xb;
                   }
                   *o = X;
                   return 0;
               },
               [&]() -> int {
                   if (force_global) return 0;
                   if (decide_probe()) return 0;
                   if (!sw_known && hipEventQuery(ctx->ev_local) != hipSuccess) return 0;
                   if (read_switch()) return 0;
                   return sw < 0;
               },
               [&](hipStream_t) -> int {
                   return decide_probe();
               }};
        const EmitTarget target{&Late::call, &late, &Late::abandon, &Late::round1};
        const int rc = global_match_and_emit(Rp, np[1], Tp, np[0], kg, mg, walk_chunk(tn), ws, wsb, nullptr, &g_rlen, &wr,
                                             s2, paren, &target, false);
        if (rc != WALK_ABANDONED) {
            TRY(rc);
            if (!X) return ctx->fail(SCCG_E_INTERNAL, "record text position never resolved");
// ... 1331 lines not shown
```

### sccg-genome-compression_amd/csrc/walk.hip

```cpp
#include "internal.h"

#include <algorithm>
#include <chrono>
#include <map>
#include <mutex>
#include <cstdio>
#include <cstdlib>
#include <vector>

namespace {

constexpr int WPB = 4;
constexpr int WWPB = 4;
constexpr int WCAP = 256;
constexpr int32_t INVALID = INT32_MIN;
constexpr int32_t NEVER = INT32_MIN + 1;
constexpr int ANCHOR_K = 32;
constexpr int KEY_K = 15;
constexpr int KMAX = 32;
constexpr int KB_COUNT = 32;
constexpr int ANCHOR_STEP = 64;
constexpr int ANCHOR_LOAD = 1;
constexpr int ANCHOR_PROBE_BATCHES = 2;
constexpr uint32_t A_MULTI = 0xFFFFFFFFu;
// ... 610 lines not shown
                const int cl_ = __ffsll((long long)cm) - 1;
                cm &= cm - 1;
                const int32_t c = W.lo + 4 * cl_ + qq;
                const int32_t l = ext_k(A, L, B, c, y);
                ncand++;
                if (!l) continue;
                if (l > bl) { bl = l; bcnt = 1; bhas0 = (c == 0); bkey = c ? pick_key(c, P) : ~0ull; }
                else if (l == bl) {
                    bcnt++;
                    if (c == 0) bhas0 = true;
                    else { const uint64_t pk = pick_key(c, P); bkey = pk < bkey ? pk : bkey; }
                }
            }
        }
        if (!bcnt) {
            x = y + 1;
            continue;
        }
        uint64_t pk;
        if (bcnt >= 2 && bhas0) pk = bkey;
        else { const uint64_t k0 = bhas0 ? pick_key(0, P) : ~0ull; pk = k0 < bkey ? k0 : bkey; }
        const int32_t p = (int32_t)(uint32_t)pk;
        if (p == 0) {
            escalated = true;
            if (lane == 0 && !CARRY) {
                if (kind == KIND_SPEC) { KC->cnt[ob][j] = 0; KC->exitX[j] = INVALID; KC->exitP[j] = INVALID; }
                else {
                    KC->status[j] = ST_ESC;
                    KC->escX[j] = y; KC->escP[j] = P; KC->escN[j] = n; KC->escQ[j] = q;
                    atomicAdd(&KC->scal[1], 1);
                }
            }
            break;
        }
        {
            const int slot = n - rb_n0;
            if (lane == slot) { rbt = y; rbp = p; rbl = bl; }
            n++;
            if (slot == 63) flush_recs();
        }
        if (DBG) { dbg_c[0]++; dbg_c[4] += ncand; dbg_c[5] += bl; tick(8); }
        if (cb >= 0) {
            for (;;) {
                if (q >= cq0 + 64) load_prev(q);
                const int32_t qi = cq0 + lane;
                const bool ge = qi >= q && (qi >= cc || ctv >= y);
                const unsigned long long gm = __ballot(ge);
                if (gm) { q = cq0 + first_lane(gm); break; }
                q = cq0 + 64;
            }
            const int ql = q - cq0;
            if (q < cc && q >= old_seedq && lane_val(ctv, ql) == y && lane_val(cpv, ql) == p && lane_val(clv, ql) == bl) {
                flush_recs();
                const int32_t rest = cc - q - 1;
                for (int i = lane; i < rest; i += 64) {
                    W_OT[n + i] = W_CT[q + 1 + i];
                    W_OP[n + i] = W_CP[q + 1 + i];
                    W_OL[n + i] = W_CL[q + 1 + i];
                }
                n += rest;
                rb_n0 = n;
                converged = true;
                break;
            }
        }
        lme = y + bl;
        P = p + bl - 1;
        x = y + bl;
    }
    flush_recs();
    if (escalated) return;
    const int32_t nx = converged ? uni(KC->exitX[j]) : x, np = converged ? uni(KC->exitP[j]) : P;
    const bool frozen_end = !converged && x == hi_j && x - lme >= FROZEN_MIN;
    const bool trapped = !converged && x - x_entry >= A.S / 2 && (P - P_entry < TRAP_P && P_entry - P < TRAP_P);
    const bool exit_changed = nx != uni(KC->exitX[j]) || np != uni(KC->exitP[j]);
    if (!CARRY) {
        if (DBG && lane == 0 && (A.dbg_round < 0 || A.dbg_round == A.round)) {
            tick(9);
            uint64_t* d = KC->dbg + (size_t)j * DBG_SLOTS;
            d[0] = wall_clock64() - dbg_t0;
            for (int i = 0; i < 13; i++) d[1 + i] = dbg_c[i];
            d[14] = (uint64_t)A.round;
            d[15] = dbg_t0;
        }
        if (lane == 0) {
            KC->cnt[ob][j] = n;
            if (cb < 0) {
                KC->exitX[j] = x; KC->exitP[j] = P;
                KC->seedq[j] = seedq;
            } else {
                KC->newX[j] = nx; KC->newP[j] = np;
                KC->conv[j] = converged;
                KC->changed[j] = exit_changed;
                KC->walked[j] = A.round;
                KC->frozen[j] = frozen_end;
                KC->trapped[j] = trapped;
            }
            KC->status[j] = converged ? ST_CONV : ST_DONE;
        }
        if (kind != KIND_FIX || (j > 0 && uni(KC->lround[j - 1]) == A.round)) return;
        if (converged || !exit_changed || frozen_end || trapped) return;
        const int32_t j1 = j + 1;
        if (j1 >= A.C || uni(KC->lround[j1]) == A.round || (j1 + 1 < A.C && uni(KC->lround[j1 + 1]) == A.round)) return;
        if (lane == 0) {
            const int32_t at = atomicAdd(&KC->scal[11], 1);
            if (at < A.C) KC->clist[at] = j1;
            atomicOr(&KC->cbits[j1 >> 5], 1u << (j1 & 31));
        }
        return;
    } else {
        if (frozen_end) return;
        if (lane == 0) {
            KC->cnt[ob][j] = n;
            KC->cur[j] = ob;
            KC->exitX[j] = nx; KC->exitP[j] = np;
            KC->usedX[j] = x_entry; KC->usedP[j] = P_entry;
            KC->seedq[j] = 0;
            KC->conv[j] = converged;
            KC->changed[j] = exit_changed;
            KC->walked[j] = A.round;
            KC->frozen[j] = 0;
            KC->trapped[j] = trapped;
        }
    }
    if (converged || !exit_changed || frozen_end || trapped) return;
    const int32_t j1 = j + 1;
    if (j1 >= A.C || uni(KC->lround[j1]) == A.round || (j1 + 1 < A.C && uni(KC->lround[j1 + 1]) == A.round)) return;
    j = j1;
    lo_j = chunk_lo(A, j);
    hi_j = chunk_hi(A, j);
    scan_end = hi_j < lastk + 1 ? hi_j : lastk + 1;
    cb = uni(KC->cur[j]);
    ob = 1 - cb;
    cc = uni(KC->cnt[cb][j]);
    old_seedq = uni(KC->seedq[j]);
    n = 0;
    q = 0;
    rb_n0 = 0;
    seedq = 0;
    converged = false;
    x_entry = x;
    P_entry = P;
    load_prev(0);
    }
}

#undef W_OT
#undef W_OP
#undef W_OL
#undef W_CT
#undef W_CP
#undef W_CL

__global__ void k_commit(WalkPtrs A, const int32_t* __restrict__ list, int32_t nlist, const int32_t* __restrict__ nlist_dev) {
    if (A.scal[9]) return;
    if (nlist_dev) nlist = *nlist_dev;
    if (blockIdx.x == 0 && threadIdx.x < FROZEN_MAX) A.fy[threadIdx.x] = INT32_MAX;
    if (blockIdx.x == 0 && threadIdx.x == 0) A.scal[11] = 0;
    for (int32_t i = (int32_t)(blockIdx.x * blockDim.x + threadIdx.x); i < nlist; i += (int32_t)(gridDim.x * blockDim.x)) {
        const int32_t j = list[i];
        if (A.kind[j] == KIND_SPEC || A.status[j] == ST_ESC) continue;
        const int32_t round = A.round;
        const bool pred_changed = j > 0 && A.walked[j - 1] == round && A.changed[j - 1];
        if (!(A.conv[j] || !pred_changed)) continue;
        A.cur[j] = 1 - A.cur[j];
        A.exitX[j] = A.newX[j];
        A.exitP[j] = A.newP[j];
        A.usedX[j] = A.snapX[j];
        A.usedP[j] = A.snapP[j];
        A.seedq[j] = 0;
        if (A.frozen[j]) {
            A.flist[atomicAdd(&A.scal[5], 1)] = j;
            atomicOr(&A.fbits[j >> 5], 1u << (j & 31));
        }
    }
}

constexpr int LS_T = 256;
__global__ __launch_bounds__(LS_T) void k_list_sort(WalkPtrs A, int32_t* __restrict__ list, const int32_t* __restrict__ count,
                                                    uint32_t* __restrict__ bits) {
    if (A.scal[9]) return;
    __shared__ int32_t wsum[LS_T / 64 + 1];
    if (*count <= 0) return;
    const int32_t nw = (A.C + 31) >> 5;
    const int32_t per = (nw + LS_T - 1) / LS_T, w0 = (int32_t)threadIdx.x * per;
    const int32_t w1 = w0 + per < nw ? w0 + per : nw;
    int c = 0;
    for (int32_t w = w0; w < w1; w++) c += __popc(bits[w]);
    const int incl = wave_incl_add<int>(c);
    const int wv = (int)(threadIdx.x >> 6), lane = lane_id();
    if (lane == 63) wsum[wv] = incl;
    __syncthreads();
    if (threadIdx.x == 0) {
        int run = 0;
        for (int i = 0; i < LS_T / 64; i++) { const int x = wsum[i]; wsum[i] = run; run += x; }
    }
    __syncthreads();
    int at = wsum[wv] + incl - c;
    for (int32_t w = w0; w < w1; w++) {
        uint32_t b = bits[w];
        if (!b) continue;
        bits[w] = 0;
        for (; b; b &= b - 1) list[at++] = (w << 5) + __ffs((int)b) - 1;
    }
}

constexpr unsigned FZ_GRID = 256;
constexpr int FZ_T = SCCG_BLOCK;
__global__ __launch_bounds__(SCCG_BLOCK) void k_frozen_scan(WalkPtrs A, int fbase) {
    __shared__ WalkLds lds_all[WPB];
    if (A.scal[9]) return;
    const int fi = (int)blockIdx.y, f = fbase + fi;
    if (f >= A.scal[5]) return;
    const int32_t j = A.flist[f];
    const int32_t x0 = A.exitX[j], P = A.exitP[j];
    WalkLds& L = lds_all[wave_in_block()];
    RegWin W;
    reg_window(A, P, W);
    if (W.n <= 0) return;
    bloom_window(W, L);
    const int32_t end = A.nT - A.k + 1 < A.xhi ? A.nT - A.k + 1 : A.xhi;
    const int64_t gw = (int64_t)blockIdx.x * WPB + wave_in_block(), G = (int64_t)gridDim.x * WPB;
    for (int64_t base = x0 + gw * 64 * WIDE; base < end; base += G * 64 * WIDE) {
        if (base >= (int64_t)__hip_atomic_load(&A.fy[fi], __ATOMIC_RELAXED, __HIP_MEMORY_SCOPE_AGENT)) return;
        const int32_t seg_end = base + 64 * WIDE < end ? (int32_t)(base + 64 * WIDE) : end;
        const int32_t y = wide_scan(A, L, W, (int32_t)base, seg_end);
        if (y < seg_end) {
            if (lane_id() == 0) atomicMin(&A.fy[fi], y);
            return;
        }
    }
}

__device__ __forceinline__ int32_t fill_last(const WalkPtrs& A, int32_t j, int32_t y) {
    const int32_t lastk1 = A.nT - A.k + 1;
    const int32_t cap = A.xhi < lastk1 ? A.xhi : lastk1;
    if (y >= cap) return A.C - 1;
    if (y < A.xlo) return j;
    const int32_t q = (y - A.xlo) / A.S - 1;
    return q < j ? j : (q > A.C - 1 ? A.C - 1 : q);
}
template <bool DEV>
__global__ void k_walk_init(WalkPtrs A, int32_t startX, int32_t startP) {
    if (DEV && blockIdx.x == 0 && threadIdx.x == 0) {
        const unsigned long long* r = A.fc + 4;
        if (r[8] != 2 && r[0] == 0 && r[4] > 0) {
            const uint64_t k0 = 1ull << 32;
            const uint64_t pk = (r[5] >= 2 && r[6]) ? r[7] : ((r[6] && k0 < r[7]) ? k0 : r[7]);
            startX = (int32_t)r[4];
            startP = (int32_t)(uint32_t)pk + (int32_t)r[4] - 1;
        } else {
            startX = A.nT - A.k + 1;
            startP = INVALID;
        }
    }
    if (blockIdx.x == 0 && threadIdx.x == 0) A.scal[9] = DEV && startP == INVALID ? 1 : 0;
    for (int32_t j = (int32_t)(blockIdx.x * blockDim.x + threadIdx.x); j < A.C; j += (int32_t)(gridDim.x * blockDim.x)) {
        A.cur[j] = 0;
        A.cnt[0][j] = 0;
        A.cnt[1][j] = 0;
        A.usedX[j] = NEVER;
        A.usedP[j] = NEVER;
        A.exitX[j] = INVALID;
        A.exitP[j] = INVALID;
        A.kind[j] = j ? KIND_SPEC : KIND_FIX;
        A.plist[j] = j;
        A.lround[j] = 1;
        A.seedq[j] = 0;
        A.trapped[j] = 0;
        A.tflag[j] = 0;
        A.hintY[j] = -1;
        A.walked[j] = 0;
        A.changed[j] = 0;
        A.conv[j] = 0;
        A.frozen[j] = 0;
    }
    for (int32_t w = (int32_t)(blockIdx.x * blockDim.x + threadIdx.x); w <= A.C / 32; w += (int32_t)(gridDim.x * blockDim.x)) {
        A.fbits[w] = 0;
        A.cbits[w] = 0;
    }
    if (blockIdx.x == 0 && threadIdx.x == 0) {
        A.scal[0] = 0; A.scal[1] = 0; A.scal[2] = startX; A.scal[3] = startP;
        A.scal[5] = 0;
        A.scal[11] = 0;
        A.snapX[0] = startX;
        A.snapP[0] = startP;
    }
}

__global__ void k_spec_rest(WalkPtrs A) {
    const int32_t next = A.round + 1;
    for (int32_t q = (int32_t)(blockIdx.x * blockDim.x + threadIdx.x); q < A.C; q += (int32_t)(gridDim.x * blockDim.x)) {
        if (A.usedX[q] != NEVER || A.lround[q] == next) continue;
        A.kind[q] = KIND_SPEC;
        A.lround[q] = next;
        A.plist[atomicAdd(&A.scal[0], 1)] = q;
    }
}

constexpr int RESPEC_T = 1024;
__global__ __launch_bounds__(FROZEN_MAX) void k_round_fill(WalkPtrs A, int fbase, int fcap) {
    if (A.scal[9]) return;
    __shared__ int32_t rj[FROZEN_MAX], ry[FROZEN_MAX], sj[FROZEN_MAX], sy[FROZEN_MAX];
    const int t = (int)threadIdx.x;
    int nf = fcap > 0 ? A.scal[5] - fbase : 0;
    if (nf > fcap) nf = fcap;
    if (nf < 0) nf = 0;
    int32_t j = 0, y = 0;
    if (t < nf) { j = A.flist[fbase + t]; y = A.fy[t]; rj[t] = j; ry[t] = y; }
    __syncthreads();
    if (t < nf) {
        int r = 0;
        for (int f = 0; f < nf; f++) r += rj[f] < j || (rj[f] == j && f < t);
        sj[r] = j;
        sy[r] = y;
    }
    __syncthreads();
    if (t == 0) {
        int na = 0;
        int32_t filled_to = -1;
        for (int r = 0; r < nf; r++) {
            const int32_t jr = sj[r];
            if (jr <= filled_to || jr + 1 >= A.C) continue;
            const int32_t last = fill_last(A, jr, sy[r]);
            if (last > jr) { A.fa_j[na] = jr; A.fa_l[na] = last; A.fa_p[na] = A.exitP[jr]; na++; }
            if (last + 1 < A.C && sy[r] != INT32_MAX) { A.hintY[last + 1] = sy[r]; A.hintP[last + 1] = A.exitP[jr]; }
            filled_to = last;
        }
        A.scal[13] = na;
        A.scal[0] = 0;
        A.scal[12] = 0;
    }
}

__global__ __launch_bounds__(256) void k_round_fillg(WalkPtrs A) {
    if (A.scal[9]) return;
    __shared__ int32_t fj[FROZEN_MAX], fl[FROZEN_MAX], fp[FROZEN_MAX];
    const int na = A.scal[13];
    if (!na) return;
    for (int i = (int)threadIdx.x; i < na; i += 256) { fj[i] = A.fa_j[i]; fl[i] = A.fa_l[i]; fp[i] = A.fa_p[i]; }
    __syncthreads();
    const int32_t q = (int32_t)(blockIdx.x * blockDim.x + threadIdx.x);
    if (q >= A.C) return;
    int lo = 0, hi = na;
    while (lo < hi) {
        const int mid = (lo + hi) >> 1;
        if (fj[mid] < q) lo = mid + 1; else hi = mid;
    }
    if (lo == 0 || q > fl[lo - 1]) return;
    const int32_t P = fp[lo - 1];
    const int32_t lastk1 = A.nT - A.k + 1;
    const int32_t lo_q = chunk_lo(A, q), hi_q = chunk_hi(A, q);
    A.cnt[A.cur[q]][q] = 0;
    A.usedX[q] = lo_q < lastk1 ? lo_q : lastk1;
    A.usedP[q] = P;
    A.exitX[q] = hi_q < lastk1 ? hi_q : lastk1;
    A.exitP[q] = P;
    A.changed[q] = 0;
    A.seedq[q] = 0;
    A.trapped[q] = 0;
}

__global__ __launch_bounds__(256) void k_round_pending(WalkPtrs A) {
    if (A.scal[9]) return;
    const int32_t next = A.round + 1;
    const int32_t j = (int32_t)(blockIdx.x * blockDim.x + threadIdx.x);
    if (j >= A.C) return;
    const int32_t ex = j ? A.exitX[j - 1] : A.scal[2];
    const int32_t ep = j ? A.exitP[j - 1] : A.scal[3];
    const int32_t ux = A.usedX[j], up = A.usedP[j], lr = A.lround[j];
    const bool pend = ex != INVALID && !(ex == ux && ep == up);
    if (!pend) {
        if (lr == next) A.lround[j] = A.round;
        return;
    }
    A.snapX[j] = ex;
    A.snapP[j] = ep;
    A.kind[j] = KIND_FIX;
    A.lround[j] = next;
    A.plist[atomicAdd(&A.scal[0], 1)] = j;
    const bool trig = j > 0 && A.trapped[j - 1] && A.walked[j - 1] == A.round;
    A.tflag[j] = trig ? A.round : -1;
    if (trig) atomicAdd(&A.scal[12], 1);
}

__global__ __launch_bounds__(RESPEC_T) void k_round_respec(WalkPtrs A) {
    if (A.scal[9]) return;
    const int ntrig = A.scal[12];
    if (!ntrig) return;
    const int32_t next = A.round + 1;
    __shared__ int32_t trig[RESPEC_MAX_TRIGGERS];
    __shared__ int32_t wsum[RESPEC_T / 64 + 1];
    {
        const int32_t per = (A.C + RESPEC_T - 1) / RESPEC_T, c0 = (int32_t)threadIdx.x * per;
        int cnt = 0;
        for (int32_t q = c0; q < c0 + per && q < A.C; q++) cnt += A.tflag[q] == A.round && A.lround[q] == next;
        const int incl = wave_incl_add<int>(cnt);
        const int w = (int)(threadIdx.x >> 6), lane = lane_id();
        if (lane == 63) wsum[w] = incl;
        __syncthreads();
        if (threadIdx.x == 0) {
            int run = 0;
            for (int i = 0; i < RESPEC_T / 64; i++) { const int x = wsum[i]; wsum[i] = run; run += x; }
            wsum[RESPEC_T / 64] = run;
        }
        __syncthreads();
        int at = wsum[w] + incl - cnt;
        for (int32_t q = c0; q < c0 + per && q < A.C && at < RESPEC_MAX_TRIGGERS; q++)
            if (A.tflag[q] == A.round && A.lround[q] == next) trig[at++] = q;
        __syncthreads();
    }
    const int nt = wsum[RESPEC_T / 64] < RESPEC_MAX_TRIGGERS ? wsum[RESPEC_T / 64] : RESPEC_MAX_TRIGGERS;
    const int w = (int)(threadIdx.x >> 6), nw = (int)(blockDim.x >> 6), lane = lane_id();
    for (int t = w; t < nt; t += nw) {
        const int32_t j = trig[t], P = A.snapP[j];
        for (int32_t q0 = j + 1; q0 <= j + RESPEC_AHEAD && q0 < A.C; q0 += 64) {
            const int32_t q = q0 + lane;
            const bool ok = q < A.C && q <= j + RESPEC_AHEAD && A.lround[q] != next;
            const unsigned long long okm = __ballot(ok);
            const unsigned long long run = ~okm ? okm & ((1ull << first_lane(~okm)) - 1) : okm;
            if ((run >> lane) & 1ull) {
                A.kind[q] = KIND_SPEC;
                A.guess[q] = P;
                A.lround[q] = next;
                A.plist[atomicAdd(&A.scal[0], 1)] = q;
            }
            if (run != ~0ull) break;
        }
    }
}

int launch_round_end(const WalkPtrs& A, int fbase, int fcap, hipStream_t s) {
    hipLaunchKernelGGL(k_round_fill, dim3(1), dim3(FROZEN_MAX), 0, s, A, fbase, fcap);
    if (fcap > 0) hipLaunchKernelGGL(k_round_fillg, dim3(grid_for(A.C, 256)), dim3(256), 0, s, A);
    hipLaunchKernelGGL(k_round_pending, dim3(grid_for(A.C, 256)), dim3(256), 0, s, A);
    hipLaunchKernelGGL(k_round_respec, dim3(1), dim3(RESPEC_T), 0, s, A);
    SCCG_HIP(hipGetLastError());
    return 0;
}

__global__ void k_chain_init(WalkPtrs A) {
    if (A.scal[9]) return;
    const int lane = lane_id();
    const int nf = A.scal[5];
    int32_t pmin = INT32_MAX;
    if (A.ch_settled) {
        const int np = A.scal[0];
        for (int i = lane; i < np; i += 64) { const int32_t q = A.plist[i]; pmin = q < pmin ? q : pmin; }
        pmin = wave_min(pmin);
    }
    int32_t jm = INT32_MAX;
    for (int f = lane; f < nf; f += 64) { const int32_t j = A.flist[f]; jm = j < jm && j < pmin ? j : jm; }
    jm = wave_min(jm);
    if (lane) return;
    if (jm == INT32_MAX) { A.chs[0] = 0; A.chs[4] = -1; A.chs[5] = 0; return; }
    const int32_t x0 = A.exitX[jm], P0 = A.exitP[jm];
    A.chs[0] = 1; A.chs[1] = x0; A.chs[2] = P0; A.chs[3] = 0; A.chs[4] = jm; A.chs[5] = 0;
    A.chs[8] = 0; A.chs[9] = x0; A.chs[10] = P0; A.chs[11] = 0; A.chs[12] = 0; A.chs[13] = INT32_MAX;
}

__device__ __forceinline__ uint32_t ch_slot(uint32_t key) { return slot_hash(key, CH_TBITS); }
constexpr uint32_t CH_EMPTY = 0xFFFFFFFFu;

__global__ __launch_bounds__(1024) void k_chain_scan(WalkPtrs A) {
    __shared__ uint32_t tab[1 << CH_TBITS];
    __shared__ int32_t wsum[17];
    __shared__ int32_t trunc_s;
    __shared__ int32_t s_first;
    if (!A.chs[0]) return;
    const int tid = (int)threadIdx.x, lane = lane_id(), w = wave_in_block(), k = A.k;
    const int32_t x = A.chs[1], P = A.chs[2];
    const bool first_only = A.chs[12] != 0;
    const int32_t half = first_only ? A.m : CH_BAND;
    const int32_t blo = P - half < 0 ? 0 : P - half;
    const int32_t bhi = P + half < A.nR - k ? P + half : A.nR - k;
    if (blockIdx.x == 0 && tid == 0) { A.chs[6] = blo; A.chs[7] = bhi; }
    for (int i = tid; i < (1 << CH_TBITS); i += 1024) tab[i] = CH_EMPTY;
    if (tid == 0) trunc_s = INT32_MAX;
    __syncthreads();
    const int kp = A.kp;
    const uint32_t MASK = (1u << (2 * kp)) - 1u, KM = (1u << kp) - 1u;
    for (int32_t q = blo + tid; q <= bhi; q += 1024) {
        uint32_t wv[4], bad;
        uint64_t code;
        loadw<4>(A.R + q, wv);
        pack_codes<4>(wv, code, bad);
        uint32_t key = bad & KM ? exotic_key(A.R + q, kp) : (uint32_t)code & MASK;
        if (key == CH_EMPTY) key = CH_EMPTY - 1;
        uint32_t sl = ch_slot(key);
        for (;;) {
            const uint32_t prev = atomicCAS(&tab[sl], CH_EMPTY, key);
            if (prev == CH_EMPTY || prev == key) break;
            sl = (sl + 1) & ((1u << CH_TBITS) - 1);
        }
    }
    __syncthreads();
    auto in_band = [&](uint32_t key) -> bool {
        if (key == CH_EMPTY) key = CH_EMPTY - 1;
        uint32_t sl = ch_slot(key);
        for (;;) {
            const uint32_t v = tab[sl];
            if (v == key) return true;
            if (v == CH_EMPTY) return false;
            sl = (sl + 1) & ((1u << CH_TBITS) - 1);
        }
    };
    const int32_t lastk1 = A.nT - k + 1;
    int64_t total = (int64_t)lastk1 - x;
    if (total > CH_FF_SPAN * CH_GRID) total = CH_FF_SPAN * CH_GRID;
    const int64_t end = (int64_t)x + (total > 0 ? total : 0);
    if (blockIdx.x == 0 && tid == 0) A.chs[14] = end < lastk1 ? (int32_t)end : INT32_MAX;
    int64_t span = total > 0 ? (total + CH_GRID - 1) / CH_GRID : 0;
    span = (span + 15) & ~(int64_t)15;
    const int64_t b0 = (int64_t)x + (int64_t)blockIdx.x * span;
    const int64_t b1 = b0 + span < end ? b0 + span : end;
    int32_t* oy = A.chh_y + (size_t)blockIdx.x * CH_HCAP;
    uint32_t* ok = A.chh_k + (size_t)blockIdx.x * CH_HCAP;
    int32_t cnt = 0;
    int64_t covered = b1;
    for (int64_t base = b0; base < b1; base += 16 * 1024) {
        if (first_only) {
            if (tid == 0) s_first = __hip_atomic_load(&A.chs[13], __ATOMIC_RELAXED, __HIP_MEMORY_SCOPE_AGENT);
            __syncthreads();
            const bool stop = base > (int64_t)s_first;
            __syncthreads();
            if (stop) {
                covered = base;
                break;
            }
        }
        const int64_t p0 = base + 16 * tid;
        uint32_t mask = 0;
        uint64_t code = 0;
        uint32_t bad = 0;
        if (p0 < b1) {
            uint32_t wv[8];
            loadw<8>(A.T + p0, wv);
            pack_codes<8>(wv, code, bad);
            const int lim = b1 - p0 < 16 ? (int)(b1 - p0) : 16;
            for (int st = 0; st < lim; st++) {
                const uint32_t key = (bad >> st) & KM ? exotic_key(A.T + p0 + st, kp) : (uint32_t)(code >> (2 * st)) & MASK;
                if (in_band(key)) mask |= 1u << st;
            }
        }
        const int c = __popc(mask);
        const int incl = wave_incl_add(c);
        if (lane == 63) wsum[w] = incl;
        __syncthreads();
        if (tid == 0) {
            int acc = 0;
            for (int i = 0; i < 16; i++) { const int t = wsum[i]; wsum[i] = acc; acc += t; }
            wsum[16] = acc;
        }
        __syncthreads();
        int idx = cnt + wsum[w] + incl - c;
        const int tot = wsum[16];
        for (uint32_t m = mask; m; m &= m - 1) {
            const int st = __ffs((int)m) - 1;
            const int32_t y = (int32_t)(p0 + st);
            if (idx < CH_HCAP) {
                oy[idx] = y;
                ok[idx] = (bad >> st) & KM ? exotic_key(A.T + y, kp) : (uint32_t)(code >> (2 * st)) & MASK;
            } else if (idx == CH_HCAP) {
                trunc_s = y;
            }
            idx++;
        }
        cnt += tot;
        __syncthreads();
        if (cnt > CH_HCAP) { covered = trunc_s; break; }
        if (first_only && cnt > 0) {
            const int32_t y0 = oy[0];
            if (tid == 0) atomicMin(&A.chs[13], y0);
            cnt = 1;
            covered = (int64_t)y0 + 1;
            break;
        }
    }
    if (tid == 0) {
        A.chh_n[blockIdx.x] = cnt < CH_HCAP ? cnt : CH_HCAP;
        const bool cut = covered >= b1 && b0 < b1 && b1 == end && end < lastk1;
        A.chh_tr[blockIdx.x] = covered < b1 ? (int32_t)covered : cut ? (int32_t)end : INT32_MAX;
    }
}

constexpr int CH_WBITS = 9;
__device__ void chain_wtab_build(const RegWin& W, uint32_t* tab) {
    const int lane = lane_id();
    for (int i = lane; i < (1 << CH_WBITS); i += 64) tab[i] = CH_EMPTY;
// ... 415 lines not shown
    const int k = A.k, kp = A.kp;
    const uint32_t key0 = walk_key(A.T + x0, kp);
    CandBest best{0, 0, 0, ~0ull};
    for (int i = threadIdx.x; i < (1 << PBBITS); i += blockDim.x) { hkey[i] = 0xffffffffu; hidx[i] = 0xffffffffu; }
    for (int i = threadIdx.x; i < (1 << (PFBITS - 5)); i += blockDim.x) bits[i] = 0;
    __syncthreads();
    for (int i = threadIdx.x; i < nb; i += blockDim.x) {
        uint32_t w[4], bad;
        uint64_t cw;
        loadw<4>(A.T + x0 + i, w);
        pack_codes<4>(w, cw, bad);
        const uint32_t key = bad & ((1u << kp) - 1u) ? exotic_key(A.T + x0 + i, kp) : (uint32_t)cw & ((1u << (2 * kp)) - 1u);
        if (key >= KEY_EXOTIC) { atomicMin(&A.fc[5], (unsigned long long)(x0 + i)); continue; }
        const uint32_t fb = slot_hash(key, PFBITS);
        atomicOr(&bits[fb >> 5], 1u << (fb & 31));
        int slot = (int)slot_hash(key, PBBITS);
        for (;;) {
            const uint32_t prev = atomicCAS(&hkey[slot], 0xffffffffu, key);
            if (prev == 0xffffffffu || prev == key) { atomicMin(&hidx[slot], (uint32_t)i); break; }
            slot = (slot + 1) & ((1 << PBBITS) - 1);
        }
    }
    __syncthreads();
    sweep_kmers(A.R, (int64_t)A.nR - k + 1, kp, [&](uint32_t code, bool pure) {
        const uint32_t fb = slot_hash(code, PFBITS);
        return pure && ((bits[fb >> 5] >> (fb & 31)) & 1u);
    }, [&](int64_t c) {
        uint64_t cw = 0;
        uint32_t bad;
        uint32_t w[4];
        loadw<4>(A.R + c, w);
        pack_codes<4>(w, cw, bad);
        const uint32_t code = (uint32_t)cw & ((1u << (2 * kp)) - 1u);
        if (code == key0 && (k == kp || bytes_eq(A.R + c + kp, A.T + x0 + kp, k - kp))) {
            const uint32_t l = (uint32_t)serial_ext(A.R, A.nR, A.T, A.nT, (int32_t)c, x0, k);
            best = cb_merge(best, CandBest{l, 1u, c == 0 ? 1u : 0u, c ? pick_key((int32_t)c, -1) : ~0ull});
        }
        int slot = (int)slot_hash(code, PBBITS);
        for (;;) {
            const uint32_t hk = hkey[slot];
            if (hk == 0xffffffffu) break;
            if (hk == code) { atomicMin(&A.fc[4], (unsigned long long)(x0 + hidx[slot])); break; }
            slot = (slot + 1) & ((1 << PBBITS) - 1);
        }
    });
    best = cb_wave(best);
    if (lane_id() == 0) wbest[wave_in_block()] = best;
    __syncthreads();
    if (threadIdx.x == 0) {
        for (int i = 1; i < SCCG_BLOCK / 64; i++) best = cb_merge(best, wbest[i]);
        unsigned long long* o = A.fcb + 4 * blockIdx.x;
        o[0] = best.l; o[1] = best.cnt; o[2] = best.has0; o[3] = best.minkey;
    }
}

template <bool ANCH>
__global__ __launch_bounds__(SCCG_BLOCK) void k_key0(WalkPtrs A, int32_t x0) {
    __shared__ CandBest wbest[SCCG_BLOCK / 64];
    const int k = A.k, kp = A.kp;
    const uint32_t key0 = walk_key(A.T + x0, kp);
    CandBest best{0, 0, 0, ~0ull};
    if (key0 < KEY_EXOTIC || ANCH) {
        const bool want = key0 < KEY_EXOTIC;
        sweep_kmers_w(A.R, (int64_t)A.nR - k + 1, kp, [&](uint32_t code, bool pure) { return want && pure && code == key0; },
                      [&](int64_t c) {
                          if (k > kp && !bytes_eq(A.R + c + kp, A.T + x0 + kp, k - kp)) return;
                          const uint32_t l = (uint32_t)serial_ext(A.R, A.nR, A.T, A.nT, (int32_t)c, x0, k);
                          best = cb_merge(best, CandBest{l, 1u, c == 0 ? 1u : 0u, c ? pick_key((int32_t)c, -1) : ~0ull});
                      },
                      [&](int64_t p0, const uint32_t (&cw)[20], const uint32_t (&dw)[20], uint32_t acc) {
                          if (ANCH) anchor_samples(A, A.nR, p0, cw, dw, acc);
                      });
    }
    best = cb_wave(best);
    if (lane_id() == 0) wbest[wave_in_block()] = best;
    __syncthreads();
    if (threadIdx.x == 0) {
        for (int i = 1; i < SCCG_BLOCK / 64; i++) best = cb_merge(best, wbest[i]);
        unsigned long long* o = A.fcb + 4 * blockIdx.x;
        o[0] = best.l; o[1] = best.cnt; o[2] = best.has0; o[3] = best.minkey;
    }
}

__global__ __launch_bounds__(SCCG_BLOCK) void k_first_kmer(const uint8_t* __restrict__ fa, int64_t n,
                                                           const int64_t* __restrict__ hdr, int k, int64_t limit,
                                                           uint8_t* __restrict__ kb) {
    __shared__ int64_t tmp[5];
    constexpr int PER = 64;
    const int64_t h = hdr[0], he = hdr[1];
    const int64_t end = n < limit ? n : limit;
    int64_t found = 0;
    for (int64_t base = 0; base < end && found < k; base += (int64_t)SCCG_BLOCK * PER) {
        const int64_t p0 = base + (int64_t)threadIdx.x * PER;
        uint32_t w[PER / 4];
        if (p0 + PER + 4 <= end) {
            loadw<PER / 4>(fa + p0, w);
        } else {
#pragma unroll
            for (int q = 0; q < PER / 4; q++) {
                uint32_t v = 0;
                for (int i = 0; i < 4; i++) {
                    const int64_t p = p0 + 4 * q + i;
                    v |= (uint32_t)(p < end ? fa[p] : (uint8_t)' ') << (8 * i);
                }
                w[q] = v;
            }
        }
        uint64_t keep = 0;
#pragma unroll
        for (int i = 0; i < PER; i++) {
            const uint8_t b = (uint8_t)(w[i >> 2] >> (8 * (i & 3)));
            const int64_t p = p0 + i;
            const bool kp = p < end && !(p >= h && p < he) && !c_isspace(b) && c_toupper(b) != 'N';
            keep |= (uint64_t)kp << i;
        }
        int64_t total = 0;
        int64_t idx = found + block_excl_add((int64_t)__popcll(keep), tmp, &total);
        for (uint64_t m = keep; m && idx < k; m &= m - 1, idx++) {
            const int i = __ffsll((long long)m) - 1;
            kb[idx] = c_toupper((uint8_t)(w[i >> 2] >> (8 * (i & 3))));
        }
        found += total;
    }
    if (threadIdx.x == 0) *reinterpret_cast<int32_t*>(kb + KB_COUNT) = found < k ? (int32_t)found : k;
}

__global__ __launch_bounds__(SCCG_BLOCK) void k_sweep_early(WalkPtrs A) {
    const int k = A.k, kp = A.kp;
    const int64_t nR = A.dnR ? *A.dnR : A.nR;
    const bool have = *reinterpret_cast<const int32_t*>(A.kb + KB_COUNT) == k;
    const uint32_t key0 = have ? walk_key(A.kb, kp) : KEY_EXOTIC;
    const bool want = key0 < KEY_EXOTIC;
    sweep_kmers_w(A.R, nR - k + 1, kp, [&](uint32_t code, bool pure) { return want && pure && code == key0; },
                  [&](int64_t c) {
                      if (k > kp && !bytes_eq(A.R + c + kp, A.kb + kp, k - kp)) return;
                      const unsigned long long i = atomicAdd(&A.fc[13], 1ull);
                      if (i < (unsigned long long)CAND_CAP) A.cand[i] = (int32_t)c;
                  },
                  [&](int64_t p0, const uint32_t (&cw)[20], const uint32_t (&dw)[20], uint32_t acc) {
                      anchor_samples(A, nR, p0, cw, dw, acc);
                  });
}

constexpr int CAND_STATS_GRID = 256;
__device__ __forceinline__ bool cand_stats_usable(const WalkPtrs& A) {
    const int k = A.k, lane = lane_id();
    const bool head = *reinterpret_cast<const int32_t*>(A.kb + KB_COUNT) == k && A.fc[13] <= (unsigned long long)CAND_CAP &&
                      A.nT >= k;
    const bool same = lane >= k || A.kb[lane] == A.T[lane];
    return head && __ballot(!same) == 0 && walk_key(A.kb, A.kp) < KEY_EXOTIC;
}
__global__ __launch_bounds__(SCCG_BLOCK) void k_cand_stats(WalkPtrs A) {
    __shared__ CandBest wbest[SCCG_BLOCK / 64];
    __shared__ int ok;
    const int k = A.k;
    const unsigned long long cnt = A.fc[13];
    if (threadIdx.x < 64) {
        const bool u = cand_stats_usable(A);
        if (threadIdx.x == 0) ok = u;
    }
    __syncthreads();
    CandBest v{0, 0, 0, ~0ull};
    if (ok) {
        const unsigned long long nw = (unsigned long long)gridDim.x * (SCCG_BLOCK / 64);
        for (unsigned long long i = blockIdx.x * (SCCG_BLOCK / 64) + (threadIdx.x >> 6); i < cnt; i += nw) {
            const int32_t c = A.cand[i];
            int32_t maxlen = A.nR - (c + k);
            if (A.nT - k < maxlen) maxlen = A.nT - k;
            const uint32_t l = (uint32_t)(k + wave_lce_hbm(A.R, c + k, A.T, k, maxlen));
            v = cb_merge(v, CandBest{l, 1u, c == 0 ? 1u : 0u, c ? pick_key(c, -1) : ~0ull});
        }
    }
    if (lane_id() != 0) v = CandBest{0, 0, 0, ~0ull};
    v = cb_wave(v);
    if (lane_id() == 0) wbest[threadIdx.x >> 6] = v;
    __syncthreads();
    if (threadIdx.x == 0) {
        for (int i = 1; i < SCCG_BLOCK / 64; i++) v = cb_merge(v, wbest[i]);
        unsigned long long* o = A.fcb + 4 * blockIdx.x;
        o[0] = v.l; o[1] = v.cnt; o[2] = v.has0; o[3] = v.minkey;
    }
}

__global__ __launch_bounds__(1024) void k_cand_stats_fin(WalkPtrs A, int nblk) {
    __shared__ CandBest wbest[16];
    __shared__ int ok;
    if (threadIdx.x < 64) {
        const bool u = cand_stats_usable(A);
        if (threadIdx.x == 0) { ok = u; A.fc[12] = u ? 1 : 2; }
    }
    __syncthreads();
    if (!ok) return;
    CandBest v{0, 0, 0, ~0ull};
    for (int b = (int)threadIdx.x; b < nblk; b += (int)blockDim.x) {
        const unsigned long long* o = A.fcb + 4 * b;
        v = cb_merge(v, CandBest{(uint32_t)o[0], (uint32_t)o[1], (uint32_t)o[2], o[3]});
    }
    v = cb_wave(v);
    if (lane_id() == 0) wbest[threadIdx.x >> 6] = v;
    __syncthreads();
    if (threadIdx.x == 0) {
        for (int i = 1; i < (int)(blockDim.x >> 6); i++) v = cb_merge(v, wbest[i]);
        A.fc[8] = v.l; A.fc[9] = v.cnt; A.fc[10] = v.has0; A.fc[11] = v.minkey;
        A.fc[4] = v.cnt ? 0ull : ~0ull;
        A.fc[5] = ~0ull;
    }
}

__global__ __launch_bounds__(1024) void k_cand_reduce(WalkPtrs A, int nblk, int32_t x0) {
    __shared__ CandBest wbest[16];
    CandBest v{0, 0, 0, ~0ull};
    for (int b = (int)threadIdx.x; b < nblk; b += (int)blockDim.x) {
        const unsigned long long* o = A.fcb + 4 * b;
        v = cb_merge(v, CandBest{(uint32_t)o[0], (uint32_t)o[1], (uint32_t)o[2], o[3]});
    }
    v = cb_wave(v);
    if (lane_id() == 0) wbest[threadIdx.x >> 6] = v;
    __syncthreads();
    if (threadIdx.x == 0) {
        for (int i = 1; i < (int)(blockDim.x >> 6); i++) v = cb_merge(v, wbest[i]);
        A.fc[8] = v.l; A.fc[9] = v.cnt; A.fc[10] = v.has0; A.fc[11] = v.minkey;
        if (x0 >= 0) { A.fc[4] = v.cnt ? (unsigned long long)x0 : ~0ull; A.fc[5] = ~0ull; A.fc[12] = 0; }
    }
}

__global__ void k_chunk_counts(WalkPtrs A) {
    for (int32_t j = (int32_t)(blockIdx.x * blockDim.x + threadIdx.x); j < A.C; j += (int32_t)(gridDim.x * blockDim.x))
        A.flat_off[j] = A.cnt[A.cur[j]][j];
}

__global__ __launch_bounds__(SCCG_BLOCK) void k_flatten(WalkPtrs A, int32_t first) {
    const int32_t j = (int32_t)blockIdx.x * WPB + wave_in_block();
    if (j >= A.C) return;
    const int lane = lane_id();
    const int32_t b = A.cur[j];
    const int32_t n = A.cnt[b][j];
    const int64_t o = A.flat_off[j] + first;
    const int32_t* t = A.bt[b] + (size_t)j * A.cap;
    const int32_t* p = A.bp[b] + (size_t)j * A.cap;
    const int32_t* l = A.bl[b] + (size_t)j * A.cap;
    for (int i = lane; i < n; i += 64) { A.ft[o + i] = t[i]; A.fp[o + i] = p[i]; A.fl[o + i] = l[i]; }
}

constexpr int64_t LONG_PIECE = 64 * 1024;
__device__ __forceinline__ void queue_long(const WalkPtrs& A, int64_t src, int64_t dst, int64_t len) {
    const int64_t np = (len + LONG_PIECE - 1) / LONG_PIECE;
    const int64_t e = (int64_t)atomicAdd((unsigned long long*)&A.scal64[2], (unsigned long long)np);
    for (int64_t i = 0; i < np && e + i < A.lgap_cap; i++) {
        int64_t* q = A.lgap + 3 * (e + i);
        q[0] = src + i * LONG_PIECE;
        q[1] = dst + i * LONG_PIECE;
        q[2] = len - i * LONG_PIECE < LONG_PIECE ? len - i * LONG_PIECE : LONG_PIECE;
    }
}

__device__ __forceinline__ void wave_copy(const uint8_t* __restrict__ s, uint8_t* __restrict__ d, int64_t n) {
    const int lane = lane_id();
    int64_t head = (int64_t)((16 - ((uintptr_t)d & 15)) & 15);
    if (head > n) head = n;
    if (lane < head) d[lane] = s[lane];
    s += head; d += head; n -= head;
    const int64_t nb = n >> 4;
    uint4* d4 = reinterpret_cast<uint4*>(d);
    for (int64_t c0 = 0; c0 < nb; c0 += 8 * 64) {
        uint32_t w[8][4];
#pragma unroll
        for (int u = 0; u < 8; u++) {
            const int64_t c = c0 + u * 64 + lane;
            if (c < nb) loadw<4>(s + 16 * c, w[u]);
        }
#pragma unroll
        for (int u = 0; u < 8; u++) {
            const int64_t c = c0 + u * 64 + lane;
            if (c < nb) d4[c] = make_uint4(w[u][0], w[u][1], w[u][2], w[u][3]);
        }
    }
    const int64_t t = nb << 4;
    if (t + lane < n) d[t + lane] = s[t + lane];
}

__global__ void k_match_textlen(WalkPtrs A, int64_t nm, int abs_p) {
    for (int64_t i = (int64_t)blockIdx.x * blockDim.x + threadIdx.x; i < nm; i += (int64_t)gridDim.x * blockDim.x) {
        const int32_t pend = i ? A.ft[i - 1] + A.fl[i - 1] : 0;
        const int32_t pprev = i && !abs_p ? A.fp[i - 1] : 0;
        const int32_t d = (int32_t)((uint32_t)A.fp[i] - (uint32_t)pprev);
        A.tlen[i] = (int64_t)(A.ft[i] - pend) + 3 + ndigits_i32(d) + ndigits_i32(A.fl[i]);
    }
}

__global__ __launch_bounds__(SCCG_BLOCK) void k_match_textwrite(WalkPtrs A, int64_t nm, uint8_t* __restrict__ out,
                                                                int abs_p) {
    constexpr int32_t SHORT_GAP = 32;
    const int64_t i = (int64_t)blockIdx.x * blockDim.x + threadIdx.x;
    const bool valid = i < nm;
    int32_t pend = 0, gap = 0;
    int64_t o = 0;
    if (valid) {
        pend = i ? A.ft[i - 1] + A.fl[i - 1] : 0;
        gap = A.ft[i] - pend;
        o = A.tlen[i];
        if (gap <= SHORT_GAP)
            for (int32_t q = 0; q < gap; q++) out[o + q] = A.T[pend + q];
    }
    if (valid && gap >= LONG_GAP) queue_long(A, pend, o, gap);
    for (unsigned long long lm = __ballot(valid && gap > SHORT_GAP && gap < LONG_GAP); lm; lm &= lm - 1) {
        const int l = __ffsll((long long)lm) - 1;
        const int32_t gp = __shfl(pend, l, 64), gg = __shfl(gap, l, 64);
        const int64_t go = __shfl(o, l, 64);
        for (int32_t q = lane_id(); q < gg; q += 64) out[go + q] = A.T[gp + q];
    }
    if (valid) {
        uint8_t* d = out + o + gap;
        const int32_t pprev = i && !abs_p ? A.fp[i - 1] : 0;
        *d++ = '(';
        d += write_i32(d, (int32_t)((uint32_t)A.fp[i] - (uint32_t)pprev));
        *d++ = ',';
        d += write_i32(d, A.fl[i]);
        *d = ')';
    }
}

struct FirstMatch {
    int32_t y, p, l, valid;
};

__global__ void k_chunk_meta(WalkPtrs A) {
    if (A.scal[9]) return;
    for (int32_t j = (int32_t)(blockIdx.x * blockDim.x + threadIdx.x); j < A.C; j += (int32_t)(gridDim.x * blockDim.x)) {
        const int32_t n = A.cnt[A.cur[j]][j];
        A.cprev[j] = n > 0 ? j : -1;
        A.flat_off[j] = n;
    }
}

constexpr int CP_PER = 16, CP_MAX = 1024 * CP_PER;
__global__ __launch_bounds__(1024) void k_chunk_prefix(WalkPtrs A) {
    __shared__ int64_t wsum[16], wmax[16];
    if (A.scal[9]) return;
    const int tid = (int)threadIdx.x, lane = lane_id(), w = wave_in_block();
    const int32_t per = (A.C + 1023) / 1024, base = tid * per;
    int64_t n[CP_PER];
    int64_t s = 0, mx = -1;
#pragma unroll
    for (int i = 0; i < CP_PER; i++) {
        const int32_t j = base + i;
        n[i] = (i < per && j < A.C) ? A.cnt[A.cur[j]][j] : 0;
        s += n[i];
        if (n[i] > 0) mx = j;
    }
    int64_t is = s, im = mx;
#pragma unroll
    for (int d = 1; d < 64; d <<= 1) {
        const int64_t os = __shfl_up(is, d, 64), om = __shfl_up(im, d, 64);
        if (lane >= d) { is += os; im = om > im ? om : im; }
    }
// ... 321 lines not shown
        const RbItem it1{A.chs, cs, (int)sizeof cs};
        const int rc = dev_readback(&it1, 1, s);
        if (rc) return rc;
    }
    *gens = cs[8];
    *trapped = cs[5] == 2 && cs[3] >= CH_HANDBACK_N;
    if (walk_env().debug)
        fprintf(stderr, "[chain] from chunk %d (x %d, P %d): %d generations, %d matches, end x %d P %d, reason %d\n", cs[4], cs[9],
                cs[10], cs[8], cs[3], cs[1], cs[2], cs[5]);
    return 0;
}

int resolve_escalations(WalkPtrs& A, hipStream_t s, std::vector<int32_t>* resumed) {
    const size_t C = (size_t)A.C;
    std::vector<char> seen(C, 0);
    for (;;) {
        int32_t nesc = 0;
        SCCG_HIP(hipMemcpyAsync(&nesc, A.scal + 1, sizeof nesc, hipMemcpyDeviceToHost, s));
        SCCG_HIP(hipStreamSynchronize(s));
        if (!nesc) return 0;
        std::vector<int32_t> st(C), ex(C), ep(C), en(C), cur(C);
        SCCG_HIP(hipMemcpyAsync(st.data(), A.status, C * 4, hipMemcpyDeviceToHost, s));
        SCCG_HIP(hipMemcpyAsync(ex.data(), A.escX, C * 4, hipMemcpyDeviceToHost, s));
        SCCG_HIP(hipMemcpyAsync(ep.data(), A.escP, C * 4, hipMemcpyDeviceToHost, s));
        SCCG_HIP(hipMemcpyAsync(en.data(), A.escN, C * 4, hipMemcpyDeviceToHost, s));
        SCCG_HIP(hipMemcpyAsync(cur.data(), A.cur, C * 4, hipMemcpyDeviceToHost, s));
        SCCG_HIP(hipStreamSynchronize(s));
        std::vector<int32_t> rl;
        for (size_t j = 0; j < C; j++) {
            if (st[j] != ST_ESC) continue;
            FullC f;
            int rc = run_fullc(A, ex[j], ep[j], &f, s);
            if (rc) return rc;
            if (f.lmax <= 0) return SCCG_E_INTERNAL;
            const int32_t ob = 1 - cur[j];
            const size_t at = j * (size_t)A.cap + (size_t)en[j];
            if ((rc = dev_set_i32(A.bt[ob] + at, 1, {ex[j]}, s)) || (rc = dev_set_i32(A.bp[ob] + at, 1, {f.p}, s)) ||
                (rc = dev_set_i32(A.bl[ob] + at, 1, {(int32_t)f.lmax}, s)) ||
                (rc = dev_set_i32(A.escX + j, 1, {ex[j] + (int32_t)f.lmax}, s)) ||
                (rc = dev_set_i32(A.escP + j, 1, {f.p + (int32_t)f.lmax - 1}, s)) ||
                (rc = dev_set_i32(A.escN + j, 1, {en[j] + 1}, s)) || (rc = dev_set_i32(A.kind + j, 1, {KIND_RESUME}, s)))
                return rc;
            rl.push_back((int32_t)j);
            if (!seen[j]) { seen[j] = 1; resumed->push_back((int32_t)j); }
        }
        int rc = dev_set_i32(A.scal + 1, 1, {0}, s);
        if (rc) return rc;
        if ((rc = h2d_sync(A.rlist, rl.data(), rl.size() * 4, s))) return rc;
        PROF_LAUNCH(PROF_WALK, s, walk_kernel(A), dim3(grid_for((int64_t)rl.size(), WWPB)), dim3(64 * WWPB), 0, s, A,
                    (const int32_t*)A.rlist, (int32_t)rl.size(), (const int32_t*)nullptr);
        SCCG_HIP(hipGetLastError());
    }
}

}

size_t walk_workspace_bytes(int64_t nR, int64_t nT, int k, int chunk) {
    size_t used = 0;
    carve(nullptr, 0, nullptr, nR, nullptr, nT, k, 100, chunk, &used);
    return used + 4096;
}

static thread_local WalkPtrs g_last;
static thread_local int64_t g_last_n = 0;

int global_matches(void* , const int32_t** t, const int32_t** p, const int32_t** l, int64_t* n) {
    *t = g_last.ft; *p = g_last.fp; *l = g_last.fl; *n = g_last_n;
    return 0;
}

#define RC(expr)                      \
    do {                              \
        int rc_ = (expr);             \
        if (rc_) return rc_;          \
    } while (0)

namespace {

struct Prepared {
    const void* ws = nullptr;
    const uint8_t* R = nullptr;
    const uint8_t* T = nullptr;
    int64_t nR = -1, nT = -1;
    int k = 0, m = 0, chunk = 0;
    uint32_t agen = 0;
    int abits = 0;
};
thread_local Prepared g_prep;

struct Early {
    const void* ws = nullptr;
    const uint8_t* R = nullptr;
    int64_t nR = -1;
    int k = 0;
    uint32_t agen = 0;
    int abits = 0;
};
thread_local Early g_early;

unsigned first_sweep_grid(const WalkPtrs& A) {
    const unsigned g = grid_for(A.nR - A.k + 1, 256 * FC_PER_T);
    return g > KEY0_GRID ? KEY0_GRID : g;
}

struct AnchorSeen { const uint64_t* tab; size_t clean; uint32_t gen; };
std::mutex g_anchor_mu;
std::map<const void*, AnchorSeen> g_anchor_seen;

int anchor_generation(WalkPtrs& A, const void* ws, hipStream_t s) {
    const size_t n = (size_t)1 << A.abits;
    uint32_t g;
    bool clear;
    {
        std::lock_guard<std::mutex> lk(g_anchor_mu);
        AnchorSeen& e = g_anchor_seen[ws];
        clear = e.tab != A.atab || n > e.clean || e.gen >= ANCHOR_GEN_MASK;
        if (clear) e.gen = 0;
        e.tab = A.atab;
        e.clean = n;
        g = ++e.gen;
    }
    if (clear) SCCG_HIP(hipMemsetAsync(A.atab, 0, n * sizeof(uint64_t), s));
    A.agen = g;
    return 0;
}

int queue_prepare(WalkPtrs& A, const void* ws, hipStream_t s) {
    const int32_t lastk = A.nT - A.k;
    const bool walkable = A.nR >= A.k && lastk >= 0;
    if (!walkable) return 0;
    const unsigned gsweep = first_sweep_grid(A);
    RC(anchor_generation(A, ws, s));
    PROF_LAUNCH(PROF_ANCHOR, s, k_key0<true>, dim3(gsweep), dim3(SCCG_BLOCK), 0, s, A, 0);
    hipLaunchKernelGGL(k_cand_reduce, dim3(1), dim3(1024), 0, s, A, (int)gsweep, 0);
    SCCG_HIP(hipGetLastError());
    return 0;
}

WalkPtrs make_ptrs(const uint8_t* Rp, int64_t nRp, const uint8_t* Tp, int64_t nTp, int k, int m, int chunk, void* ws,
                   size_t ws_bytes, size_t* used, int abits = 0) {
    WalkPtrs A = carve(ws, ws_bytes, Rp, nRp, Tp, nTp, k, m, chunk, used, abits);
    if (!walk_env().debug) A.dbg = nullptr;
    A.dbg_phases = walk_env().phases;
    A.dbg_round = walk_env().debug_round;
    A.adet = env_int("SCCG_ANCHOR_DET", 0);
    return A;
}

}

void global_prepare_reset() { g_prep = Prepared{}; g_early = Early{}; }

int global_sweep_early(const uint8_t* Rp, int64_t nRp, const int64_t* d_nRp, const uint8_t* tgt_fa, int64_t tn,
                       const int64_t* d_hdr, int k, int m, int chunk, void* ws, size_t ws_bytes, hipStream_t s) {
    g_early = Early{};
    if (m < 0 || 2 * m + 1 > WCAP || k > KMAX || k < 1) return SCCG_E_UNSUPPORTED;
    if (nRp < k || tn <= 0) return 0;
    size_t used = 0;
    WalkPtrs A = make_ptrs(Rp, nRp, nullptr, tn, k, m, chunk, ws, ws_bytes, &used);
    if (used > ws_bytes) return SCCG_E_INTERNAL;
    A.dnR = d_nRp;
    RC(anchor_generation(A, ws, s));
    RC(set_u64(A.fc + 12, {0, 0}, s));
    hipLaunchKernelGGL(k_first_kmer, dim3(1), dim3(SCCG_BLOCK), 0, s, tgt_fa, tn, d_hdr, k, (int64_t)1 << 20, A.kb);
    PROF_LAUNCH(PROF_ANCHOR, s, k_sweep_early, dim3(first_sweep_grid(A)), dim3(SCCG_BLOCK), 0, s, A);
    SCCG_HIP(hipGetLastError());
    g_early = Early{ws, Rp, nRp, k, A.agen, A.abits};
    return 0;
}

int global_prepare(const uint8_t* Rp, int64_t nRp, const uint8_t* Tp, int64_t nTp, int k, int m, int chunk, void* ws,
                   size_t ws_bytes, hipStream_t s) {
    g_prep = Prepared{};
    if (m < 0 || 2 * m + 1 > WCAP || k > KMAX || k < 1) return SCCG_E_UNSUPPORTED;
    const Early e = g_early;
    g_early = Early{};
    const bool early = e.ws == ws && e.R == Rp && e.nR >= nRp && e.k == k;
    size_t used = 0;
    WalkPtrs A = make_ptrs(Rp, nRp, Tp, nTp, k, m, chunk, ws, ws_bytes, &used, early ? e.abits : 0);
    if (used > ws_bytes) return SCCG_E_INTERNAL;
    if (early) {
        A.agen = e.agen;
        if (A.nR >= A.k && A.nT >= A.k) {
            hipLaunchKernelGGL(k_cand_stats, dim3(CAND_STATS_GRID), dim3(SCCG_BLOCK), 0, s, A);
            hipLaunchKernelGGL(k_cand_stats_fin, dim3(1), dim3(1024), 0, s, A, CAND_STATS_GRID);
            SCCG_HIP(hipGetLastError());
        }
    } else {
        RC(queue_prepare(A, ws, s));
    }
    g_prep = Prepared{ws, Rp, Tp, nRp, nTp, k, m, chunk, A.agen, A.abits};
    return 0;
}

namespace {
struct RangeWalk {
    int64_t x0 = 0, P0 = -1, x_end = 0;
    int64_t exit_x = 0, exit_P = -1;
};

struct WalkRun {
    WalkPtrs A;
    hipStream_t s;
    WalkResult* res;
    const EmitTarget* late_out;
    RangeWalk* rw;
    uint8_t* out;
    bool abs_p, keep_flat;
    const uint8_t* Tp;
    int64_t nTp;
    int32_t lastk;
    int32_t first_y = INVALID, first_p = 0, first_l = 0;
    int32_t startX = 0, startP = INVALID;
    bool pre_round = false;
    bool spec_queued = false;
    bool spec_text = false;
    bool text_done = false;
    bool resolved = false;
    int32_t rs_pre[6] = {};
    int64_t spec_r[2] = {0, 0};
    std::chrono::steady_clock::time_point t_last = std::chrono::steady_clock::now();

    void mark(const char* what) {
        if (!walk_env().debug) return;
        (void)hipStreamSynchronize(s);
        const auto t = std::chrono::steady_clock::now();
        fprintf(stderr, "[phase]   walk.%-12s %8.3f ms\n", what, std::chrono::duration<double, std::milli>(t - t_last).count());
        t_last = t;
    }
    int64_t literal_exit(int64_t from) const {
        const int64_t lim = rw->x_end < (int64_t)lastk + 1 ? rw->x_end : (int64_t)lastk + 1;
        return from < lim ? lim : from;
    }
    int resolve_out() {
        if (!resolved && late_out) RC(late_out->resolve(late_out->user, &out));
        resolved = true;
        return 0;
    }
    int queue_round(int fbase_cap, bool dev_nlist);
    int queue_text(bool long_copy, bool dev_first);
    int frozen_batch(int fbase, int fcap, bool init_fy);
    int first_step();
    int probe_frozen_first(bool* frozen_first);
    int run_rounds(bool frozen_first);
    int emit_chunk_text(int64_t* out_len);
    int emit_flat(int64_t* out_len);
};
int debug_round(const WalkRun& w, int64_t round, const int32_t (&rs)[6]);

int WalkRun::queue_round(int fbase_cap, bool dev_nlist) {
    const int32_t* nd = dev_nlist ? A.scal : nullptr;
    PROF_LAUNCH(PROF_WALK, s, walk_kernel(A), dim3(grid_for(A.C, WWPB)), dim3(64 * WWPB), 0, s, A, (const int32_t*)A.plist,
                A.C, nd);
    if (dev_nlist) RC(launch_carry(A, s));
    hipLaunchKernelGGL(k_commit, dim3(grid_for(A.C, 256) > 4096 ? 4096 : grid_for(A.C, 256)), dim3(256), 0, s, A,
                       (const int32_t*)A.plist, A.C, nd);
    hipLaunchKernelGGL(k_list_sort, dim3(1), dim3(LS_T), 0, s, A, A.flist, (const int32_t*)(A.scal + 5), A.fbits);
    if (fbase_cap > 0) hipLaunchKernelGGL(k_frozen_scan, dim3(FZ_GRID, fbase_cap), dim3(FZ_T), 0, s, A, 0);
    SCCG_HIP(hipGetLastError());
    RC(launch_round_end(A, 0, fbase_cap, s));
    return 0;
}

int WalkRun::queue_text(bool long_copy, bool dev_first) {
    const int32_t nf = dev_first ? 2 : first_y != INVALID ? 1 : 0;
    if (A.C <= CP_MAX) {
        hipLaunchKernelGGL(k_chunk_prefix, dim3(1), dim3(1024), 0, s, A);
    } else {
        const unsigned gc = grid_for(A.C, 256) > 4096 ? 4096 : grid_for(A.C, 256);
        hipLaunchKernelGGL(k_chunk_meta, dim3(gc), dim3(256), 0, s, A);
        RC(dev_excl_max(A.cprev, A.cprev, A.C, nullptr, A.partial, s));
        RC(dev_excl_sum(A.flat_off, A.flat_off, A.C, A.scal64, A.partial, s));
        RC(set_u64(reinterpret_cast<unsigned long long*>(A.scal64 + 2), {0}, s));
    }
    const FirstMatch F{first_y, first_p, first_l, nf};
    hipLaunchKernelGGL(k_chunk_text<false>, dim3(grid_for(A.C, WPB)), dim3(SCCG_BLOCK), 0, s, A, F, (int)abs_p, out);
    RC(dev_excl_sum(A.ctext, A.ctext, A.C, A.scal64 + 1, A.partial, s));
    PROF_LAUNCH(PROF_MATCH_EMIT, s, k_chunk_text<true>, dim3(grid_for(A.C, WPB)), dim3(SCCG_BLOCK), 0, s, A, F,
                (int)abs_p, out);
    if (long_copy) hipLaunchKernelGGL(k_long_copy, dim3(1024), dim3(256), 0, s, A, out);
    SCCG_HIP(hipGetLastError());
    return 0;
}

int WalkRun::frozen_batch(int fbase, int fcap, bool init_fy) {
    if (init_fy) SCCG_HIP(hipMemsetD32Async((hipDeviceptr_t)A.fy, INT32_MAX, fcap, s));
    if (fcap > 0) hipLaunchKernelGGL(k_frozen_scan, dim3(FZ_GRID, fcap), dim3(FZ_T), 0, s, A, fbase);
    SCCG_HIP(hipGetLastError());
    RC(launch_round_end(A, fbase, fcap, s));
    return 0;
}

int WalkRun::first_step() {
    const int k = A.k;
    int32_t x0 = 0;
    unsigned long long r[9];
    if (pre_round) {
        if (!keep_flat && !walk_env().debug) {
            RC(resolve_out());
            RC(queue_text(true, true));
            spec_queued = true;
        }
        const RbItem it[3] = {{A.fc + 4, r, (int)sizeof r}, {A.scal, rs_pre, (int)sizeof rs_pre},
                              {A.scal64, spec_r, (int)sizeof spec_r}};
        RC(dev_readback(it, 3, s));
        if (!(r[8] != 2 && r[0] == 0 && r[4] > 0)) { pre_round = false; spec_queued = false; }
    } else {
        const RbItem it{A.fc + 4, r, (int)sizeof r};
        RC(dev_readback(&it, 1, s));
    }
    if (r[8] == 2) {
        const unsigned g = first_sweep_grid(A);
        hipLaunchKernelGGL(k_key0<false>, dim3(g), dim3(SCCG_BLOCK), 0, s, A, 0);
        hipLaunchKernelGGL(k_cand_reduce, dim3(1), dim3(1024), 0, s, A, (int)g, 0);
        SCCG_HIP(hipGetLastError());
        const RbItem it{A.fc + 4, r, (int)sizeof r};
        RC(dev_readback(&it, 1, s));
    }
    if (r[0] == 0 && r[4] > 0) {
        first_y = 0;
        const uint64_t k0 = 1ull << 32;
        const uint64_t pk = (r[5] >= 2 && r[6]) ? r[7] : ((r[6] && k0 < r[7]) ? k0 : r[7]);
        first_p = (int32_t)(uint32_t)pk;
        first_l = (int32_t)r[4];
    }
    const int64_t npos = (int64_t)A.nR - k + 1 > 0 ? (int64_t)A.nR - k + 1 : 1;
    const unsigned gsweep = grid_for(npos, 256 * FC_PER_T) > PRESENCE_GRID ? PRESENCE_GRID : grid_for(npos, 256 * FC_PER_T);
    while (x0 <= lastk && first_y == INVALID) {
        const int32_t nb = (lastk - x0 + 1) < PB ? (lastk - x0 + 1) : PB;
        RC(set_u64(A.fc + 4, {-1, -1}, s));
        PROF_LAUNCH(PROF_PRESENCE, s, k_presence, dim3(gsweep), dim3(SCCG_BLOCK), 0, s, A, x0, nb);
        hipLaunchKernelGGL(k_cand_reduce, dim3(1), dim3(1024), 0, s, A, (int)gsweep, -1);
        SCCG_HIP(hipGetLastError());
        {
            const RbItem it{A.fc + 4, r, (int)sizeof r};
            RC(dev_readback(&it, 1, s));
        }
        if (r[0] != ~0ull && r[0] < r[1]) {
            const int32_t y = (int32_t)r[0];
            if (y == x0 && r[4] > 0) {
                const uint64_t k0 = 1ull << 32;
                const uint64_t pk = (r[5] >= 2 && r[6]) ? r[7] : ((r[6] && k0 < r[7]) ? k0 : r[7]);
                first_y = y;
                first_p = (int32_t)(uint32_t)pk;
                first_l = (int32_t)r[4];
                break;
            }
            if (A.k == A.kp) { first_y = y; break; }
            FullC f;
            RC(run_fullc(A, y, -1, &f, s));
            if (f.lmax > 0) { first_y = y; first_p = f.p; first_l = (int32_t)f.lmax; break; }
            x0 = y + 1;
            continue;
        }
        if (r[1] != ~0ull) {
            FullC f;
            RC(run_fullc(A, (int32_t)r[1], -1, &f, s));
            if (f.lmax > 0) { first_y = (int32_t)r[1]; break; }
            x0 = (int32_t)r[1] + 1;
            continue;
        }
        x0 += nb;
    }
    if (first_y != INVALID && first_l == 0) {
        FullC f;
        RC(run_fullc(A, first_y, -1, &f, s));
        first_p = f.p;
        first_l = (int32_t)f.lmax;
    }
    return 0;
}

int WalkRun::probe_frozen_first(bool* frozen_first) {
    RC(dev_set_i32(A.flist, 1, {0}, s));
    RC(dev_set_i32(A.exitX, 1, {startX}, s));
    RC(dev_set_i32(A.exitP, 1, {startP}, s));
    RC(dev_set_i32(A.scal + 5, 1, {1}, s));
    RC(dev_set_i32(A.fy, 1, {INT32_MAX}, s));
    hipLaunchKernelGGL(k_frozen_scan, dim3(FZ_GRID, 1), dim3(FZ_T), 0, s, A, 0);
    SCCG_HIP(hipGetLastError());
    int32_t y0 = INT32_MAX;
    {
        const RbItem it{A.fy, &y0, (int)sizeof y0};
        RC(dev_readback(&it, 1, s));
    }
    RC(dev_set_i32(A.exitX, 1, {INVALID}, s));
    RC(dev_set_i32(A.exitP, 1, {INVALID}, s));
    RC(dev_set_i32(A.scal + 5, 1, {0}, s));
    *frozen_first = (int64_t)y0 >= (int64_t)FF_MIN_CHUNKS * A.S;
    if (walk_env().debug)
        fprintf(stderr, "[walk] frozen-first probe: first window hit %d -> %s\n", y0, *frozen_first ? "on" : "off");
    return 0;
}

int WalkRun::run_rounds(bool frozen_first) {
    const bool range = rw != nullptr;
    int32_t nlist = frozen_first ? 1 : A.C;
    bool chains_on = !range;
    int march = 0;
    int32_t prev_pend = -1;
    A.ch_settled = 0;
    const int64_t round0 = pre_round ? 2 : 1;
    for (int64_t round = round0;; round++) {
        A.round = (int32_t)round;
        const bool queued = pre_round && round == round0;
        if (!queued) {
            PROF_LAUNCH(PROF_WALK, s, walk_kernel(A), dim3(grid_for(nlist, WWPB)), dim3(64 * WWPB), 0, s, A,
                        (const int32_t*)A.plist, nlist, (const int32_t*)nullptr);
            SCCG_HIP(hipGetLastError());
            if (nlist < A.C) RC(launch_carry(A, s));
            hipLaunchKernelGGL(k_commit, dim3(grid_for(nlist, 256) > 4096 ? 4096 : grid_for(nlist, 256)), dim3(256), 0, s, A,
                               (const int32_t*)A.plist, nlist, (const int32_t*)nullptr);
            hipLaunchKernelGGL(k_list_sort, dim3(1), dim3(LS_T), 0, s, A, A.flist, (const int32_t*)(A.scal + 5), A.fbits);
        }
        res->rounds = round;
        int32_t rs[6];
        const RbItem rs_item{A.scal, rs, (int)sizeof rs};
        if (queued) {
            for (int i = 0; i < 6; i++) rs[i] = rs_pre[i];
            spec_text = spec_queued && rs[5] <= FROZEN_FIRST && rs[1] == 0;
        } else {
            RC(frozen_batch(0, FROZEN_FIRST, false));
            RC(dev_readback(&rs_item, 1, s));
        }
        if (!chains_on && rs[0] > 0 && prev_pend >= 0 && rs[0] <= prev_pend && prev_pend - rs[0] <= 2) march++;
        else march = 0;
        prev_pend = rs[0];
        const bool march_chain = !range && !chains_on && march >= MARCH_ROUNDS && rs[5] > 0;
        const bool chain_now = (chains_on && rs[5] > 0 && (round == 1 || round >= CHAIN_ROUND)) || march_chain;
        if (chain_now) {
            A.ch_settled = march_chain ? 1 : 0;
            int gens = 0;
            bool trapped = false, started = true;
            RC(run_chain(A, s, &gens, &trapped, &started));
            if (trapped) chains_on = false;
            if (started) {
                RC(frozen_batch(0, 0, false));
                RC(dev_readback(&rs_item, 1, s));
                spec_text = false;
                res->chains++;
            } else {
                march = 0;
                if (rs[5] > FROZEN_FIRST) {
                    for (int fb = FROZEN_FIRST; fb < rs[5]; fb += FROZEN_MAX) RC(frozen_batch(fb, FROZEN_MAX, true));
                    RC(dev_readback(&rs_item, 1, s));
                }
            }
        } else if (rs[5] > FROZEN_FIRST) {
            for (int fb = FROZEN_FIRST; fb < rs[5]; fb += FROZEN_MAX) RC(frozen_batch(fb, FROZEN_MAX, true));
            RC(dev_readback(&rs_item, 1, s));
        }
        if (rs[1]) {
            {
                std::vector<int32_t> resumed;
                RC(resolve_escalations(A, s, &resumed));
                RC(h2d_sync(A.rlist, resumed.data(), resumed.size() * 4, s));
                const int32_t nr = (int32_t)resumed.size();
                RC(dev_set_i32(A.scal + 5, 1, {0}, s));
                hipLaunchKernelGGL(k_commit, dim3(grid_for(nr, 256) > 4096 ? 4096 : grid_for(nr, 256)), dim3(256), 0, s, A,
                                   (const int32_t*)A.rlist, nr, (const int32_t*)nullptr);
                hipLaunchKernelGGL(k_list_sort, dim3(1), dim3(LS_T), 0, s, A, A.flist, (const int32_t*)(A.scal + 5), A.fbits);
                SCCG_HIP(hipGetLastError());
            }
            {
                const RbItem it{A.scal + 5, &rs[5], (int)sizeof(int32_t)};
                RC(dev_readback(&it, 1, s));
            }
            if (rs[5] == 0) RC(frozen_batch(0, 0, false));
            for (int fb = 0; fb < rs[5]; fb += FROZEN_MAX) RC(frozen_batch(fb, FROZEN_MAX, fb > 0));
            RC(dev_readback(&rs_item, 1, s));
        }
        nlist = rs[0];
        RC(debug_round(*this, round, rs));
        if (frozen_first && round == 1) {
            hipLaunchKernelGGL(k_spec_rest, dim3(grid_for(A.C, 256) > 4096 ? 4096 : grid_for(A.C, 256)), dim3(256), 0, s, A);
            SCCG_HIP(hipGetLastError());
            const RbItem it{A.scal, &nlist, (int)sizeof nlist};
            RC(dev_readback(&it, 1, s));
        }
        if (round == 2 && spec_text && nlist == 0) text_done = true;
        if (!nlist) return 0;
        if (round > 4 * (int64_t)A.C + 16) return SCCG_E_INTERNAL;
        if (late_out && late_out->abandon && late_out->abandon(late_out->user)) return WALK_ABANDONED;
    }
}

int WalkRun::emit_chunk_text(int64_t* out_len) {
    RC(resolve_out());
    int64_t text = 0, nmc = 0;
    if (startP != INVALID && lastk >= 0) {
        if (!text_done) {
            RC(queue_text(true, false));
            const RbItem it{A.scal64, spec_r, (int)sizeof spec_r};
            RC(dev_readback(&it, 1, s));
        }
        nmc = spec_r[0];
        text = spec_r[1];
    } else if (nTp > 0) {
        hipLaunchKernelGGL(k_copy, dim3(grid_for(nTp, WPB * LONG_PIECE)), dim3(SCCG_BLOCK), 0, s, Tp, nTp, out);
        SCCG_HIP(hipGetLastError());
        text = nTp;
    }
    res->n_matches = nmc + (first_y != INVALID ? 1 : 0);
    g_last_n = 0;
    *out_len = text;
    mark("emit");
    return 0;
}

int WalkRun::emit_flat(int64_t* out_len) {
    const int32_t nfirst = first_y != INVALID ? 1 : 0;
    hipLaunchKernelGGL(k_chunk_counts, dim3(grid_for(A.C, 256) > 4096 ? 4096 : grid_for(A.C, 256)), dim3(256), 0, s, A);
    RC(dev_excl_sum(A.flat_off, A.flat_off, A.C, A.scal64, A.partial, s));
    if (nfirst) {
        RC(dev_set_i32(A.ft, 1, {first_y}, s));
        RC(dev_set_i32(A.fp, 1, {first_p}, s));
        RC(dev_set_i32(A.fl, 1, {first_l}, s));
    }
    hipLaunchKernelGGL(k_flatten, dim3(grid_for(A.C, WPB)), dim3(SCCG_BLOCK), 0, s, A, nfirst);
    SCCG_HIP(hipGetLastError());
    int64_t nchunkm = 0;
    {
        const RbItem it{A.scal64, &nchunkm, (int)sizeof nchunkm};
        RC(dev_readback(&it, 1, s));
    }
    const int64_t nm = nchunkm + nfirst;
    res->n_matches = nm;
    g_last = A;
    g_last_n = nm;
    if (rw) {
        int32_t ex[2];
        const RbItem it[2] = {{A.exitX + (A.C - 1), &ex[0], 4}, {A.exitP + (A.C - 1), &ex[1], 4}};
        RC(dev_readback(it, 2, s));
        rw->exit_x = ex[0];
        rw->exit_P = ex[1];
        return 0;
    }

    RC(resolve_out());
    int64_t text = 0;
    int32_t tail_from = 0;
    if (nm > 0) {
        const unsigned g = grid_for(nm, 256) > 4096 ? 4096 : grid_for(nm, 256);
        hipLaunchKernelGGL(k_match_textlen, dim3(g), dim3(256), 0, s, A, nm, (int)abs_p);
        RC(set_u64(reinterpret_cast<unsigned long long*>(A.scal64 + 2), {0}, s));
        RC(dev_excl_sum(A.tlen, A.tlen, nm, A.scal64 + 1, A.partial, s));
        PROF_LAUNCH(PROF_MATCH_EMIT, s, k_match_textwrite, dim3(grid_for(nm, SCCG_BLOCK)), dim3(SCCG_BLOCK), 0, s, A, nm, out,
                    (int)abs_p);
        hipLaunchKernelGGL(k_long_copy, dim3(1024), dim3(256), 0, s, A, out);
        SCCG_HIP(hipGetLastError());
        int32_t lt[2];
        const RbItem it[3] = {{A.scal64 + 1, &text, (int)sizeof text}, {A.ft + nm - 1, &lt[0], 4}, {A.fl + nm - 1, &lt[1], 4}};
        RC(dev_readback(it, 3, s));
        tail_from = lt[0] + lt[1];
    }
    const int64_t tail = nTp - tail_from;
    if (tail > 0) {
        hipLaunchKernelGGL(k_copy, dim3(grid_for(tail, WPB * LONG_PIECE)), dim3(SCCG_BLOCK), 0, s, Tp + tail_from, tail,
                           out + text);
        SCCG_HIP(hipGetLastError());
    }
    *out_len = text + (tail > 0 ? tail : 0);
    mark("emit");
    return 0;
}

int match_and_emit_impl(const uint8_t* Rp, int64_t nRp, const uint8_t* Tp, int64_t nTp, int k, int m, int chunk,
                        void* ws, size_t ws_bytes, uint8_t* out, int64_t* out_len, WalkResult* res, hipStream_t s,
                        bool abs_p, const EmitTarget* late_out, bool keep_flat, RangeWalk* rw = nullptr) {
    if (m < 0 || 2 * m + 1 > WCAP || k > KMAX || k < 1) return SCCG_E_UNSUPPORTED;
    const bool range = rw != nullptr;
    if (range && (rw->x0 < 0 || rw->P0 < -1 || (rw->P0 == -1 && rw->x0 != 0) || rw->x0 > nTp || rw->P0 >= nRp))
        return SCCG_E_UNSUPPORTED;
    const Prepared g = g_prep;
    g_prep = Prepared{};
    const bool prepared = g.ws == ws && g.R == Rp && g.T == Tp && g.nR == nRp && g.nT == nTp && g.k == k && g.m == m &&
                          g.chunk == chunk;
    size_t used = 0;
    const int32_t lastk = (int32_t)nTp - k;
    WalkRun w{make_ptrs(Rp, nRp, Tp, nTp, k, m, chunk, ws, ws_bytes, &used, prepared ? g.abits : 0),
              s, res, late_out, rw, out, abs_p, keep_flat, Tp, nTp, lastk};
    if (used > ws_bytes) return SCCG_E_INTERNAL;
    WalkPtrs& A = w.A;
    res->rounds = 0;
    res->chains = 0;
    res->n_matches = 0;
    if (range) {
        const int64_t xe = rw->x_end < nTp ? rw->x_end : nTp;
        A.xlo = (int32_t)rw->x0;
        A.xhi = (int32_t)(xe > rw->x0 ? xe : rw->x0);
        A.C = (int32_t)(((int64_t)A.xhi - A.xlo + chunk - 1) / chunk);
        if (A.C < 1) A.C = 1;
        g_last_n = 0;
        if (nRp < k || lastk < 0) {
            rw->exit_x = w.literal_exit(rw->x0);
            rw->exit_P = rw->P0;
            return 0;
        }
    }
    res->chunks = A.C;

    const bool walkable = nRp >= k && lastk >= 0;
    if (prepared) A.agen = g.agen;
    else RC(queue_prepare(A, ws, s));

    if (walkable && !range && A.C > 0) {
        hipLaunchKernelGGL(k_walk_init<true>, dim3(grid_for(A.C, 256) > 4096 ? 4096 : grid_for(A.C, 256)), dim3(256), 0, s,
                           A, 0, 0);
        A.round = 1;
        RC(w.queue_round(FROZEN_FIRST, false));
        if (late_out && late_out->round1_queued) RC(late_out->round1_queued(late_out->user, s));
        A.round = 2;
        RC(w.queue_round(FROZEN_FIRST, true));
        w.pre_round = true;
// ... 218 lines not shown
```

Before: 183.5 billion.

## Fuse multi-kernel scans and reductions via last-block grid tickets

Adds a last-block ticket helper and uses it to fold several multi-launch sequences into single kernels. The strip scan's block-total pass moves into the last block of the local scan, and the apply step moves into the strip-write kernel. The round-end fill, pending and respec kernels become one round-close kernel, the cand-stats finalize is merged into cand_stats, and k_list_sort launches appear to be folded into commit. Header-stream work is also moved onto a separate stream joined by an event. The aim is to cut launch count and serialization on the small-kernel-dominated critical path, at the cost of atomics, fences and ticket state that must be reset correctly.

```diff
diff --git a/sccg-genome-compression_amd/csrc/common.h b/sccg-genome-compression_amd/csrc/common.h
--- a/sccg-genome-compression_amd/csrc/common.h
+++ b/sccg-genome-compression_amd/csrc/common.h
@@ -163,6 +163,24 @@
     return r;
 }
 
+__device__ __forceinline__ bool grid_last_block(unsigned int* ticket, int* lds) {
+    asm volatile("s_waitcnt vmcnt(0)" ::: "memory");
+    __syncthreads();
+    if (threadIdx.x == 0) {
+        __builtin_amdgcn_fence(__ATOMIC_RELEASE, "agent");
+        asm volatile("s_waitcnt vmcnt(0)" ::: "memory");
+        const bool last = atomicAdd(ticket, 1u) == gridDim.x * gridDim.y - 1;
+        if (last) {
+            __builtin_amdgcn_fence(__ATOMIC_ACQUIRE, "agent");
+            asm volatile("s_waitcnt vmcnt(0)" ::: "memory");
+            atomicExch(ticket, 0u);
+        }
+        *lds = last;
+    }
+    __syncthreads();
+    return *lds != 0;
+}
+
 #define SCCG_HIP(expr)                                              \
     do {                                                            \
         hipError_t e_ = (expr);                                     \
diff --git a/sccg-genome-compression_amd/csrc/ingest.hip b/sccg-genome-compression_amd/csrc/ingest.hip
--- a/sccg-genome-compression_amd/csrc/ingest.hip
+++ b/sccg-genome-compression_amd/csrc/ingest.hip
@@ -374,34 +374,36 @@
     return ts_compose(wsum[w], ex);
 }
 
-constexpr int SCAN_T = 1024, SCAN_PER = SCAN_B / SCAN_T;
-__global__ __launch_bounds__(SCAN_T) void k_strip_scan_local(int64_t ntiles, int64_t* __restrict__ ta, int64_t* __restrict__ tb,
-                                                          int64_t* __restrict__ tfa, int64_t* __restrict__ tfb,
-                                                          int32_t* __restrict__ tlast, TileSum* __restrict__ btot) {
+constexpr int SCAN_T = 256, SCAN_PER = SCAN_B / SCAN_T;
+__global__ __launch_bounds__(SCAN_T) void k_strip_scan(int64_t ntiles, int64_t* __restrict__ ta, int64_t* __restrict__ tb,
+                                                    int64_t* __restrict__ tfa, int64_t* __restrict__ tfb,
+                                                    int32_t* __restrict__ tlast, TileSum* __restrict__ btot,
+                                                    unsigned int* __restrict__ ticket, int64_t* __restrict__ d_len,
+                                                    int64_t* __restrict__ d_len2) {
     __shared__ TileSum wsum[17];
+    __shared__ int last;
     const TileSum id{0, 0, 0, 0, -1};
-    const int64_t t0 = (int64_t)blockIdx.x * SCAN_B + (int64_t)threadIdx.x * SCAN_PER;
-    TileSum v[SCAN_PER], agg = id;
-#pragma unroll
-    for (int k = 0; k < SCAN_PER; k++) {
-        const int64_t t = t0 + k;
-        v[k] = t < ntiles ? TileSum{ta[t], tb[t], tfa[t], tfb[t], tlast[t]} : id;
-        agg = ts_compose(agg, v[k]);
-    }
-    TileSum tot;
-    TileSum run = block_scan_tiles(agg, wsum, &tot);
-#pragma unroll
-    for (int k = 0; k < SCAN_PER; k++) {
-        const int64_t t = t0 + k;
-        if (t < ntiles) { ta[t] = run.a; tb[t] = run.b; tfa[t] = run.fa; tfb[t] = run.fb; tlast[t] = run.last; }
-        run = ts_compose(run, v[k]);
-    }
-    if (threadIdx.x == 0) btot[blockIdx.x] = tot;
-}
-
-__global__ __launch_bounds__(SCAN_T) void k_strip_scan_blocks(int64_t nblk, TileSum* __restrict__ btot) {
-    __shared__ TileSum wsum[17];
-    const TileSum id{0, 0, 0, 0, -1};
+    {
+        const int64_t t0 = (int64_t)blockIdx.x * SCAN_B + (int64_t)threadIdx.x * SCAN_PER;
+        TileSum v[SCAN_PER], agg = id;
+#pragma unroll
+        for (int k = 0; k < SCAN_PER; k++) {
+            const int64_t t = t0 + k;
+            v[k] = t < ntiles ? TileSum{ta[t], tb[t], tfa[t], tfb[t], tlast[t]} : id;
+            agg = ts_compose(agg, v[k]);
+        }
+        TileSum tot;
+        TileSum run = block_scan_tiles(agg, wsum, &tot);
+#pragma unroll
+        for (int k = 0; k < SCAN_PER; k++) {
+            const int64_t t = t0 + k;
+            if (t < ntiles) { ta[t] = run.a; tb[t] = run.b; tfa[t] = run.fa; tfb[t] = run.fb; tlast[t] = run.last; }
+            run = ts_compose(run, v[k]);
+        }
+        if (threadIdx.x == 0) btot[blockIdx.x] = tot;
+    }
+    if (!grid_last_block(ticket, &last)) return;
+    const int64_t nblk = gridDim.x;
     const int64_t i0 = (int64_t)threadIdx.x * SCAN_PER;
     TileSum v[SCAN_PER], agg = id;
 #pragma unroll
@@ -416,27 +418,22 @@
         if (i0 + k < nblk) btot[i0 + k] = run;
         run = ts_compose(run, v[k]);
     }
-    if (threadIdx.x == 0) btot[SCAN_B] = tot;
-}
-
-__global__ void k_strip_scan_apply(int64_t ntiles, const int64_t* __restrict__ ta, const int64_t* __restrict__ tb,
-                                   const int64_t* __restrict__ tfa, const int64_t* __restrict__ tfb,
-                                   const int32_t* __restrict__ tlast, const TileSum* __restrict__ btot,
-                                   int64_t* __restrict__ toff, int64_t* __restrict__ toff2, int32_t* __restrict__ tcarry,
-                                   int64_t* __restrict__ d_len, int64_t* __restrict__ d_len2) {
-    const TileSum start{0, 0, 0, 0, 1};
-    for (int64_t t = (int64_t)blockIdx.x * blockDim.x + threadIdx.x; t < ntiles; t += (int64_t)gridDim.x * blockDim.x) {
-        const TileSum r = ts_compose(ts_compose(start, btot[t / SCAN_B]), TileSum{ta[t], tb[t], tfa[t], tfb[t], tlast[t]});
-        toff[t] = r.b;
-        toff2[t] = r.fb;
-        tcarry[t] = r.last;
-    }
-    if (blockIdx.x == 0 && threadIdx.x == 0) {
-        const TileSum r = ts_compose(start, btot[SCAN_B]);
+    if (threadIdx.x == 0) {
+        btot[SCAN_B] = tot;
+        const TileSum r = ts_compose(TileSum{0, 0, 0, 0, 1}, tot);
         *d_len = r.b;
         if (d_len2) *d_len2 = r.fb;
     }
 }
+
+struct StripScan {
+    const int64_t* ta = nullptr;
+    const int64_t* tb = nullptr;
+    const int64_t* tfa = nullptr;
+    const int64_t* tfb = nullptr;
+    const int32_t* tlast = nullptr;
+    const TileSum* btot = nullptr;
+};
 
 __device__ __forceinline__ void run_events(uint64_t p, uint64_t K, uint32_t cin, uint64_t& st, uint64_t& en) {
     const uint64_t D = ~K;
@@ -450,10 +447,9 @@
 
 template <IngestMode MODE, bool RUNS>
 __global__ __launch_bounds__(SCCG_BLOCK) void k_strip_write(FilterMode fm, const uint8_t* __restrict__ buf, int64_t n,
-                                                            const int64_t* __restrict__ hdr,
-                                                            const int64_t* __restrict__ toff,
-                                                            const int64_t* __restrict__ toff2,
-                                                            const int32_t* __restrict__ tcarry,
+                                                            const int64_t* __restrict__ hdr, StripScan sp,
+                                                            int64_t* __restrict__ toff, int64_t* __restrict__ toff2,
+                                                            int32_t* __restrict__ tcarry,
                                                             uint8_t* __restrict__ out, uint8_t* __restrict__ out2,
                                                             int32_t* __restrict__ flags, RunSlots rsl,
                                                             const uint16_t* __restrict__ kc, const int32_t* __restrict__ kflag) {
@@ -468,12 +464,22 @@
     uint8_t* s1 = reinterpret_cast<uint8_t*>(st4);
     const int64_t off = tile * STRIP_WTILE + (int64_t)lane * SL;
     const int64_t h = MODE == INGEST_TGT ? hdr[0] : 0, he = MODE == INGEST_TGT ? hdr[1] : 0;
+    int64_t o1, o2;
+    int32_t carry;
+    if (sp.ta) {
+        const TileSum x = ts_compose(TileSum{0, 0, 0, 0, 1}, sp.btot[tile / SCAN_B]);
+        const TileSum y = ts_compose(x, TileSum{sp.ta[tile], sp.tb[tile], sp.tfa[tile], sp.tfb[tile], sp.tlast[tile]});
+        o1 = y.b; o2 = y.fb; carry = y.last;
+        if (lane == 0) { toff[tile] = o1; toff2[tile] = o2; tcarry[tile] = carry; }
+    } else {
+        o1 = toff[tile]; o2 = toff2[tile]; carry = tcarry[tile];
+    }
     uint32_t w[SNW];
     int32_t prior;
     uint64_t lsm;
     StripMasks r;
     const int32_t kf = kc ? uni(kflag[tile]) : 0;
-    if ((kf & 1) && (MODE == INGEST_TGT || !(kf & 2) || uni(tcarry[tile]) == 1)) {
+    if ((kf & 1) && (MODE == INGEST_TGT || !(kf & 2) || uni(carry) == 1)) {
         load_words<SNW>(buf, n, off, w);
         const uint32_t code = kc[tile * 64 + lane], h1 = code & 127u, h2 = code >> 7;
         const uint64_t keep = ~((h1 < 64 ? 1ull << h1 : 0ull) | (h2 < 64 ? 1ull << h2 : 0ull));
@@ -481,7 +487,7 @@
         prior = 1;
     } else {
         r = strip_tile<MODE, RUNS>(fm, buf, n, h, he, off, w, prior, lsm, stage_all4[wave_in_block()]);
-        if (MODE == INGEST_REF && prior < 0) prior = tcarry[tile];
+        if (MODE == INGEST_REF && prior < 0) prior = carry;
     }
     const uint64_t keep = r.known | (prior == 1 ? r.unknown : 0ull), fkeep = keep & r.fk;
     const uint32_t c = (uint32_t)__popcll(keep) | ((uint32_t)__popcll(fkeep) << 16);
@@ -515,7 +521,7 @@
             rsl.rf[tile] = (hm ? 1 : 0) | (int32_t)(tf << 1) | (int32_t)(tl << 3);
         }
         if ((sl | el | sn | en) != 0) {
-            const int64_t o0 = toff[tile] + (int64_t)(ex & 0xffff);
+            const int64_t o0 = o1 + (int64_t)(ex & 0xffff);
             int32_t* const dst[4] = {rsl.sl, rsl.el, rsl.sn, rsl.en};
             const uint64_t ev[4] = {sl, el, sn, en};
 #pragma unroll
@@ -534,16 +540,16 @@
     if (out) {
         stage_lane<false>(s1, tab, w, keep, (int)(ex & 0xffff));
         wave_sync();
-        stage_out(st4, (int)(tot & 0xffff), out, toff[tile]);
+        stage_out(st4, (int)(tot & 0xffff), out, o1);
     }
     if (out2) {
         if (out && !__ballot(fkeep != keep)) {
-            stage_out<true>(st4, (int)(tot >> 16), out2, toff2[tile]);
+            stage_out<true>(st4, (int)(tot >> 16), out2, o2);
         } else {
             wave_sync();
             stage_lane<true>(s1, tab, w, fkeep, (int)(ex >> 16));
             wave_sync();
-            stage_out(st4, (int)(tot >> 16), out2, toff2[tile]);
+            stage_out(st4, (int)(tot >> 16), out2, o2);
         }
     }
 }
@@ -761,7 +767,8 @@
 }
 
 constexpr int FH_T = 256, FH_PER = 64;
-__global__ __launch_bounds__(FH_T) void k_find_header(const uint8_t* __restrict__ buf, int64_t n, int64_t* __restrict__ d_sc) {
+__global__ __launch_bounds__(FH_T) void k_find_header(const uint8_t* __restrict__ buf, int64_t n, int64_t* __restrict__ d_sc,
+                                                      int32_t* __restrict__ ovf) {
     __shared__ unsigned long long s_hit;
     int64_t res[2] = {n, n};
     for (int ph = 0; ph < 2; ph++) {
@@ -792,7 +799,13 @@
             if (h != ~0ull) { res[ph] = (int64_t)h; break; }
         }
     }
-    if (threadIdx.x == 0) { d_sc[0] = res[0]; d_sc[1] = res[1]; d_sc[2] = 0; d_sc[3] = 0; }
+    if (threadIdx.x == 0) {
+        d_sc[0] = res[0]; d_sc[1] = res[1]; d_sc[2] = 0; d_sc[3] = 0;
+        d_sc[20] = (int64_t)INT32_MAX << 32;
+        d_sc[21] = (int64_t)INT32_MAX;
+        *reinterpret_cast<int32_t*>(d_sc + 32) = 0;
+        if (ovf) *ovf = 0;
+    }
 }
 
 int launch_first_match(const uint8_t* buf, int64_t n, const int64_t* from_slot, int mode, uint8_t c, int64_t* res,
@@ -808,8 +821,8 @@
     return 0;
 }
 
-int launch_find_header(const uint8_t* buf, int64_t n, int64_t* d_sc, hipStream_t s) {
-    hipLaunchKernelGGL(k_find_header, dim3(1), dim3(FH_T), 0, s, buf, n, d_sc);
+int launch_find_header(const uint8_t* buf, int64_t n, int64_t* d_sc, int32_t* d_ovf, hipStream_t s) {
+    hipLaunchKernelGGL(k_find_header, dim3(1), dim3(FH_T), 0, s, buf, n, d_sc, d_ovf);
     SCCG_HIP(hipGetLastError());
     return 0;
 }
@@ -838,21 +851,18 @@
     const int64_t nblk = (ntiles + SCAN_B - 1) / SCAN_B;
     if (nblk > SCAN_B) return SCCG_E_UNSUPPORTED;
     TileSum* btot = reinterpret_cast<TileSum*>(sc.block_sums);
-    hipLaunchKernelGGL(k_strip_scan_local, dim3((unsigned)nblk), dim3(SCAN_T), 0, s, ntiles, sc.tile_a, sc.tile_b,
-                       sc.tile_fa, sc.tile_fb, sc.tile_last, btot);
-    hipLaunchKernelGGL(k_strip_scan_blocks, dim3(1), dim3(SCAN_T), 0, s, nblk, btot);
-    hipLaunchKernelGGL(k_strip_scan_apply, dim3(grid_for(ntiles, 256)), dim3(256), 0, s, ntiles, sc.tile_a, sc.tile_b,
-                       sc.tile_fa, sc.tile_fb, sc.tile_last, btot, sc.tile_off, sc.tile_off2, sc.tile_carry, d_len,
-                       d_len2);
+    hipLaunchKernelGGL(k_strip_scan, dim3((unsigned)nblk), dim3(SCAN_T), 0, s, ntiles, sc.tile_a, sc.tile_b, sc.tile_fa,
+                       sc.tile_fb, sc.tile_last, btot, sc.scan_ticket, d_len, d_len2);
+    const StripScan sp{sc.tile_a, sc.tile_b, sc.tile_fa, sc.tile_fb, sc.tile_last, btot};
     const RunSlots rsl = runs ? *runs : RunSlots{};
     if (mode == INGEST_TGT && runs)
-        PROF_LAUNCH(PROF_STRIP, s, (k_strip_write<INGEST_TGT, true>), dim3(g), dim3(SCCG_BLOCK), 0, s, fmode, buf, n, d_header,
+        PROF_LAUNCH(PROF_STRIP, s, (k_strip_write<INGEST_TGT, true>), dim3(g), dim3(SCCG_BLOCK), 0, s, fmode, buf, n, d_header, sp,
                     sc.tile_off, sc.tile_off2, sc.tile_carry, out, out2, d_flags, rsl, (const uint16_t*)kc, (const int32_t*)kf);
     else if (mode == INGEST_TGT)
-        PROF_LAUNCH(PROF_STRIP, s, (k_strip_write<INGEST_TGT, false>), dim3(g), dim3(SCCG_BLOCK), 0, s, fmode, buf, n, d_header,
+        PROF_LAUNCH(PROF_STRIP, s, (k_strip_write<INGEST_TGT, false>), dim3(g), dim3(SCCG_BLOCK), 0, s, fmode, buf, n, d_header, sp,
                     sc.tile_off, sc.tile_off2, sc.tile_carry, out, out2, d_flags, rsl, (const uint16_t*)kc, (const int32_t*)kf);
     else
-        PROF_LAUNCH(PROF_STRIP, s, (k_strip_write<INGEST_REF, false>), dim3(g), dim3(SCCG_BLOCK), 0, s, fmode, buf, n, d_header,
+        PROF_LAUNCH(PROF_STRIP, s, (k_strip_write<INGEST_REF, false>), dim3(g), dim3(SCCG_BLOCK), 0, s, fmode, buf, n, d_header, sp,
                     sc.tile_off, sc.tile_off2, sc.tile_carry, out, out2, d_flags, rsl, (const uint16_t*)kc, (const int32_t*)kf);
     SCCG_HIP(hipGetLastError());
     return 0;
@@ -926,11 +936,11 @@
     const RunSlots rsl{};
     if (mode == INGEST_TGT)
         PROF_LAUNCH(PROF_STRIP, s, (k_strip_write<INGEST_TGT, false>), dim3(g), dim3(SCCG_BLOCK), 0, s, FILTER_UPPER, buf, n,
-                    d_header, sc.tile_off, sc.tile_off2, sc.tile_carry, out, (uint8_t*)nullptr, (int32_t*)nullptr, rsl,
+                    d_header, StripScan{}, sc.tile_off, sc.tile_off2, sc.tile_carry, out, (uint8_t*)nullptr, (int32_t*)nullptr, rsl,
                     (const uint16_t*)nullptr, (const int32_t*)nullptr);
     else
         PROF_LAUNCH(PROF_STRIP, s, (k_strip_write<INGEST_REF, false>), dim3(g), dim3(SCCG_BLOCK), 0, s, FILTER_UPPER, buf, n,
-                    d_header, sc.tile_off, sc.tile_off2, sc.tile_carry, out, (uint8_t*)nullptr, (int32_t*)nullptr, rsl,
+                    d_header, StripScan{}, sc.tile_off, sc.tile_off2, sc.tile_carry, out, (uint8_t*)nullptr, (int32_t*)nullptr, rsl,
                     (const uint16_t*)nullptr, (const int32_t*)nullptr);
     SCCG_HIP(hipGetLastError());
     return 0;
diff --git a/sccg-genome-compression_amd/csrc/internal.h b/sccg-genome-compression_amd/csrc/internal.h
--- a/sccg-genome-compression_amd/csrc/internal.h
+++ b/sccg-genome-compression_amd/csrc/internal.h
@@ -68,12 +68,13 @@
     int64_t* tile_off2;
     int32_t* tile_carry;
     void* block_sums;
+    unsigned int* scan_ticket = nullptr;
     int64_t* scalars;
     uint16_t* keep_cache = nullptr;
     int32_t* keep_flag = nullptr;
 };
 
-int launch_find_header(const uint8_t* buf, int64_t n, int64_t* d_scalars, hipStream_t s);
+int launch_find_header(const uint8_t* buf, int64_t n, int64_t* d_scalars, int32_t* d_ovf, hipStream_t s);
 int launch_first_match(const uint8_t* buf, int64_t n, const int64_t* from_slot, int mode, uint8_t c, int64_t* res,
                        int64_t* ticket_slot, hipStream_t s);
 constexpr int RUN_SLOT = 32;
@@ -148,7 +149,8 @@
 void global_prepare_reset();
 void walk_forget_workspace(const void* ws);
 int global_sweep_early(const uint8_t* Rp, int64_t nRp_bound, const int64_t* d_nRp, const uint8_t* tgt_fa, int64_t tn,
-                       const int64_t* d_hdr, int k, int m, int chunk, void* ws, size_t ws_bytes, hipStream_t s);
+                       const int64_t* d_hdr, int k, int m, int chunk, void* ws, size_t ws_bytes, hipStream_t s_head,
+                       hipEvent_t ev_head, hipStream_t s);
 struct EmitTarget {
     int (*resolve)(void* user, uint8_t** out);
     void* user;
diff --git a/sccg-genome-compression_amd/csrc/sccg_api.cpp b/sccg-genome-compression_amd/csrc/sccg_api.cpp
--- a/sccg-genome-compression_amd/csrc/sccg_api.cpp
+++ b/sccg-genome-compression_amd/csrc/sccg_api.cpp
@@ -132,7 +132,7 @@
     hipStream_t stream = nullptr;
     hipStream_t side = nullptr;
     hipStream_t side2 = nullptr;
-    hipEvent_t ev_fork = nullptr, ev_fork2 = nullptr, ev_join = nullptr, ev_lines = nullptr, ev_rstrip = nullptr, ev_hdr = nullptr, ev_tstrip = nullptr,
+    hipEvent_t ev_fork = nullptr, ev_fork2 = nullptr, ev_join = nullptr, ev_lines = nullptr, ev_rstrip = nullptr, ev_hdr = nullptr, ev_kmer = nullptr, ev_tstrip = nullptr,
                ev_local = nullptr, ev_probe = nullptr;
     int64_t* h_switch = nullptr;
     int32_t* h_probe = nullptr;
@@ -140,6 +140,7 @@
     sccg_stats stats{};
     void* buf[B_COUNT] = {};
     size_t cap[B_COUNT] = {};
+    bool fresh[B_COUNT] = {};
     uint8_t* stage[16] = {};
     hipEvent_t stage_ev[16] = {};
     hipStream_t copy_ref = nullptr, copy_tgt = nullptr;
@@ -176,6 +177,7 @@
         }
         buf[slot] = p;
         cap[slot] = bytes;
+        fresh[slot] = true;
         return p;
     }
 };
@@ -254,6 +256,7 @@
         hipEventCreateWithFlags(&c->ev_tstrip, hipEventDisableTiming) != hipSuccess ||
         hipEventCreateWithFlags(&c->ev_rstrip, hipEventDisableTiming) != hipSuccess ||
         hipEventCreateWithFlags(&c->ev_hdr, hipEventDisableTiming) != hipSuccess ||
+        hipEventCreateWithFlags(&c->ev_kmer, hipEventDisableTiming) != hipSuccess ||
         hipEventCreateWithFlags(&c->ev_local, hipEventDisableTiming) != hipSuccess ||
         hipEventCreateWithFlags(&c->ev_probe, hipEventDisableTiming) != hipSuccess ||
         hipHostMalloc(reinterpret_cast<void**>(&c->h_probe), 2 * PROBE_PAIRS * sizeof(int32_t), hipHostMallocDefault) != hipSuccess ||
@@ -282,6 +285,7 @@
     (void)hipEventDestroy(ctx->ev_tstrip);
     (void)hipEventDestroy(ctx->ev_rstrip);
     (void)hipEventDestroy(ctx->ev_hdr);
+    (void)hipEventDestroy(ctx->ev_kmer);
     (void)hipEventDestroy(ctx->ev_local);
     if (ctx->ev_probe) (void)hipEventDestroy(ctx->ev_probe);
     if (ctx->h_probe) (void)hipHostFree(ctx->h_probe);
@@ -361,9 +365,15 @@
     GET(int32_t, tc, B_TILE_CARRY + o, ntiles);
     static const bool kc_on = [] { const char* e = getenv("SCCG_STRIP_KC"); return !e || atoi(e) > 0; }();
     constexpr int64_t KC_AT = 5152;
-    GET(int64_t, bs, B_TILE_BSUM + o, kc_on ? KC_AT + ntiles * 16 + (ntiles + 1) / 2 : 1025 * 5);
+    constexpr int64_t TICKET_AT = 5128;
+    GET(int64_t, bs, B_TILE_BSUM + o, kc_on ? KC_AT + ntiles * 16 + (ntiles + 1) / 2 : KC_AT);
+    if (ctx->fresh[B_TILE_BSUM + o]) {
+        HIPTRY(hipMemsetAsync(bs + TICKET_AT, 0, sizeof(int64_t), s ? s : ctx->stream));
+        ctx->fresh[B_TILE_BSUM + o] = false;
+    }
     sc.tile_a = ta; sc.tile_b = tb; sc.tile_fa = tfa; sc.tile_fb = tfb; sc.tile_last = tl; sc.tile_off = to;
     sc.tile_off2 = to2; sc.tile_carry = tc; sc.block_sums = bs; sc.scalars = nullptr;
+    sc.scan_ticket = reinterpret_cast<unsigned int*>(bs + TICKET_AT);
     if (kc_on) {
         sc.keep_cache = reinterpret_cast<uint16_t*>(bs + KC_AT);
         sc.keep_flag = reinterpret_cast<int32_t*>(bs + KC_AT + ntiles * 16);
@@ -488,12 +498,13 @@
     const bool probe_mode = !force_global && !ctx->exact_switch && iters_max > 0 && local_probe_applies(iters_max);
     const bool lean_R = probe_mode || force_global;
     int32_t* d_flags = reinterpret_cast<int32_t*>(sc + 32);
-    HIPTRY(hipMemsetAsync(d_flags, 0, sizeof(int32_t), s));
-    TRY(dev_set_i64(sc + 20, 2, {(int64_t)INT32_MAX << 32, (int64_t)INT32_MAX}, s));
+    StripRuns sruns;
+    const bool have_runs = strip_runs(ctx, tn, &sruns);
+    int32_t* const d_ovf = have_runs ? sruns.rs.ovf : nullptr;
 
     global_prepare_reset();
     HIPTRY(hipEventRecord(ctx->ev_fork, s));
-    if (!rdy) TRY(launch_find_header(tfa, tn, sc, s));
+    if (!rdy) TRY(launch_find_header(tfa, tn, sc, d_ovf, s));
     HIPTRY(hipStreamWaitEvent(ctx->side, ctx->ev_fork, 0));
     if (rdy) {
         hipEvent_t e = nullptr;
@@ -507,12 +518,17 @@
         hipEvent_t e = nullptr;
         if (const int rc = rdy->tgt(rdy->user, &e)) return rc;
         HIPTRY(hipStreamWaitEvent(s, e, 0));
-        TRY(launch_find_header(tfa, tn, sc, s));
+        TRY(launch_find_header(tfa, tn, sc, d_ovf, s));
     }
     HIPTRY(hipEventRecord(ctx->ev_hdr, s));
-    StripRuns sruns;
-    const bool have_runs = strip_runs(ctx, tn, &sruns);
-    if (have_runs) HIPTRY(hipMemsetAsync(sruns.rs.ovf, 0, sizeof(int32_t), s));
+    const size_t wsb = walk_workspace_bytes(rn, tn, kg, walk_chunk(tn));
+    if (rn < INT32_MAX - 8 && tn < INT32_MAX - 8) {
+        HIPTRY(hipStreamWaitEvent(ctx->side2, ctx->ev_hdr, 0));
+        void* ws_early = ctx->get(B_WALK, wsb);
+        if (!ws_early) return ctx->fail(SCCG_E_NOMEM, "walk workspace of %zu bytes", wsb);
+        TRY(global_sweep_early(Rp, rn, sc + 8, tfa, tn, sc, kg, mg, walk_chunk(tn), ws_early, wsb, ctx->side2, ctx->ev_kmer,
+                               ctx->side));
+    }
     const bool lean_T = lean_R && have_runs;
     TRY(strip(ctx, INGEST_TGT, tfa, tn, sc, lean_T ? nullptr : T, sc + 2, d_flags, nullptr, FILTER_DROP_N_UPPER, Tp, 0,
               nullptr, have_runs ? &sruns.rs : nullptr));
@@ -566,13 +582,6 @@
         }
         ~WorkerJoin() { join(); }
     } lines{&ctx->worker};
-    const size_t wsb = walk_workspace_bytes(rn, tn, kg, walk_chunk(tn));
-    if (rn < INT32_MAX - 8 && tn < INT32_MAX - 8) {
-        HIPTRY(hipStreamWaitEvent(ctx->side, ctx->ev_hdr, 0));
-        void* ws_early = ctx->get(B_WALK, wsb);
-        if (!ws_early) return ctx->fail(SCCG_E_NOMEM, "walk workspace of %zu bytes", wsb);
-        TRY(global_sweep_early(Rp, rn, sc + 8, tfa, tn, sc, kg, mg, walk_chunk(tn), ws_early, wsb, ctx->side));
-    }
     HIPTRY(hipStreamWaitEvent(s, ctx->ev_rstrip, 0));
     hipStream_t s2 = ctx->side;
     HIPTRY(hipEventRecord(ctx->ev_fork, s));
diff --git a/sccg-genome-compression_amd/csrc/walk.hip b/sccg-genome-compression_amd/csrc/walk.hip
--- a/sccg-genome-compression_amd/csrc/walk.hip
+++ b/sccg-genome-compression_amd/csrc/walk.hip
@@ -786,7 +786,13 @@
 #undef W_CP
 #undef W_CL
 
-__global__ void k_commit(WalkPtrs A, const int32_t* __restrict__ list, int32_t nlist, const int32_t* __restrict__ nlist_dev) {
+constexpr int LS_T = 256;
+__device__ __forceinline__ void sort_list_block(const WalkPtrs& A, int32_t* __restrict__ list, const int32_t* __restrict__ count,
+                                                uint32_t* __restrict__ bits, int32_t* wsum);
+__global__ __launch_bounds__(LS_T) void k_commit(WalkPtrs A, const int32_t* __restrict__ list, int32_t nlist,
+                                                 const int32_t* __restrict__ nlist_dev) {
+    __shared__ int32_t wsum[LS_T / 64 + 1];
+    __shared__ int last;
     if (A.scal[9]) return;
     if (nlist_dev) nlist = *nlist_dev;
     if (blockIdx.x == 0 && threadIdx.x < FROZEN_MAX) A.fy[threadIdx.x] = INT32_MAX;
@@ -808,13 +814,12 @@
             atomicOr(&A.fbits[j >> 5], 1u << (j & 31));
         }
     }
-}
-
-constexpr int LS_T = 256;
-__global__ __launch_bounds__(LS_T) void k_list_sort(WalkPtrs A, int32_t* __restrict__ list, const int32_t* __restrict__ count,
-                                                    uint32_t* __restrict__ bits) {
-    if (A.scal[9]) return;
-    __shared__ int32_t wsum[LS_T / 64 + 1];
+    if (!grid_last_block(reinterpret_cast<unsigned int*>(A.scal + 14), &last)) return;
+    sort_list_block(A, A.flist, A.scal + 5, A.fbits, wsum);
+}
+
+__device__ __forceinline__ void sort_list_block(const WalkPtrs& A, int32_t* __restrict__ list, const int32_t* __restrict__ count,
+                                                uint32_t* __restrict__ bits, int32_t* wsum) {
     if (*count <= 0) return;
     const int32_t nw = (A.C + 31) >> 5;
     const int32_t per = (nw + LS_T - 1) / LS_T, w0 = (int32_t)threadIdx.x * per;
@@ -837,6 +842,12 @@
         bits[w] = 0;
         for (; b; b &= b - 1) list[at++] = (w << 5) + __ffs((int)b) - 1;
     }
+}
+__global__ __launch_bounds__(LS_T) void k_list_sort(WalkPtrs A, int32_t* __restrict__ list, const int32_t* __restrict__ count,
+                                                    uint32_t* __restrict__ bits) {
+    __shared__ int32_t wsum[LS_T / 64 + 1];
+    if (A.scal[9]) return;
+    sort_list_block(A, list, count, bits, wsum);
 }
 
 constexpr unsigned FZ_GRID = 256;
@@ -917,6 +928,7 @@
         A.scal[0] = 0; A.scal[1] = 0; A.scal[2] = startX; A.scal[3] = startP;
         A.scal[5] = 0;
         A.scal[11] = 0;
+        A.scal[14] = 0; A.scal[15] = 0;
         A.snapX[0] = startX;
         A.snapP[0] = startP;
     }
@@ -932,7 +944,6 @@
     }
 }
 
-constexpr int RESPEC_T = 1024;
 __global__ __launch_bounds__(FROZEN_MAX) void k_round_fill(WalkPtrs A, int fbase, int fcap) {
     if (A.scal[9]) return;
     __shared__ int32_t rj[FROZEN_MAX], ry[FROZEN_MAX], sj[FROZEN_MAX], sy[FROZEN_MAX];
@@ -967,66 +978,82 @@
     }
 }
 
-__global__ __launch_bounds__(256) void k_round_fillg(WalkPtrs A) {
+constexpr int RT_T = 256;
+__global__ __launch_bounds__(RT_T) void k_round_close(WalkPtrs A) {
     if (A.scal[9]) return;
     __shared__ int32_t fj[FROZEN_MAX], fl[FROZEN_MAX], fp[FROZEN_MAX];
+    __shared__ int32_t trig[RESPEC_MAX_TRIGGERS];
+    __shared__ int32_t wsum[RT_T / 64 + 1];
+    __shared__ int last;
     const int na = A.scal[13];
-    if (!na) return;
-    for (int i = (int)threadIdx.x; i < na; i += 256) { fj[i] = A.fa_j[i]; fl[i] = A.fa_l[i]; fp[i] = A.fa_p[i]; }
+    for (int i = (int)threadIdx.x; i < na; i += RT_T) { fj[i] = A.fa_j[i]; fl[i] = A.fa_l[i]; fp[i] = A.fa_p[i]; }
     __syncthreads();
-    const int32_t q = (int32_t)(blockIdx.x * blockDim.x + threadIdx.x);
-    if (q >= A.C) return;
-    int lo = 0, hi = na;
-    while (lo < hi) {
-        const int mid = (lo + hi) >> 1;
-        if (fj[mid] < q) lo = mid + 1; else hi = mid;
-    }
-    if (lo == 0 || q > fl[lo - 1]) return;
-    const int32_t P = fp[lo - 1];
+    const int32_t next = A.round + 1;
     const int32_t lastk1 = A.nT - A.k + 1;
-    const int32_t lo_q = chunk_lo(A, q), hi_q = chunk_hi(A, q);
-    A.cnt[A.cur[q]][q] = 0;
-    A.usedX[q] = lo_q < lastk1 ? lo_q : lastk1;
-    A.usedP[q] = P;
-    A.exitX[q] = hi_q < lastk1 ? hi_q : lastk1;
-    A.exitP[q] = P;
-    A.changed[q] = 0;
-    A.seedq[q] = 0;
-    A.trapped[q] = 0;
-}
-
-__global__ __launch_bounds__(256) void k_round_pending(WalkPtrs A) {
-    if (A.scal[9]) return;
-    const int32_t next = A.round + 1;
+    auto filled = [&](int32_t q, int32_t* P) -> bool {
+        int lo = 0, hi = na;
+        while (lo < hi) {
+            const int mid = (lo + hi) >> 1;
+            if (fj[mid] < q) lo = mid + 1; else hi = mid;
+        }
+        if (lo == 0 || q > fl[lo - 1]) return false;
+        *P = fp[lo - 1];
+        return true;
+    };
     const int32_t j = (int32_t)(blockIdx.x * blockDim.x + threadIdx.x);
-    if (j >= A.C) return;
-    const int32_t ex = j ? A.exitX[j - 1] : A.scal[2];
-    const int32_t ep = j ? A.exitP[j - 1] : A.scal[3];
-    const int32_t ux = A.usedX[j], up = A.usedP[j], lr = A.lround[j];
-    const bool pend = ex != INVALID && !(ex == ux && ep == up);
-    if (!pend) {
-        if (lr == next) A.lround[j] = A.round;
-        return;
-    }
-    A.snapX[j] = ex;
-    A.snapP[j] = ep;
-    A.kind[j] = KIND_FIX;
-    A.lround[j] = next;
-    A.plist[atomicAdd(&A.scal[0], 1)] = j;
-    const bool trig = j > 0 && A.trapped[j - 1] && A.walked[j - 1] == A.round;
-    A.tflag[j] = trig ? A.round : -1;
-    if (trig) atomicAdd(&A.scal[12], 1);
-}
-
-__global__ __launch_bounds__(RESPEC_T) void k_round_respec(WalkPtrs A) {
-    if (A.scal[9]) return;
+    if (j < A.C) {
+        int32_t ux, up, P = 0;
+        if (na && filled(j, &P)) {
+            const int32_t lo_j = chunk_lo(A, j), hi_j = chunk_hi(A, j);
+            ux = lo_j < lastk1 ? lo_j : lastk1;
+            up = P;
+            A.cnt[A.cur[j]][j] = 0;
+            A.usedX[j] = ux;
+            A.usedP[j] = up;
+            A.exitX[j] = hi_j < lastk1 ? hi_j : lastk1;
+            A.exitP[j] = P;
+            A.changed[j] = 0;
+            A.seedq[j] = 0;
+            A.trapped[j] = 0;
+        } else {
+            ux = A.usedX[j];
+            up = A.usedP[j];
+        }
+        int32_t ex, ep;
+        bool pred_trapped = false;
+        if (j == 0) {
+            ex = A.scal[2];
+            ep = A.scal[3];
+        } else if (na && filled(j - 1, &P)) {
+            const int32_t hi_p = chunk_hi(A, j - 1);
+            ex = hi_p < lastk1 ? hi_p : lastk1;
+            ep = P;
+        } else {
+            ex = A.exitX[j - 1];
+            ep = A.exitP[j - 1];
+            pred_trapped = A.trapped[j - 1] != 0;
+        }
+        const int32_t lr = A.lround[j];
+        const bool pend = ex != INVALID && !(ex == ux && ep == up);
+        if (!pend) {
+            if (lr == next) A.lround[j] = A.round;
+        } else {
+            A.snapX[j] = ex;
+            A.snapP[j] = ep;
+            A.kind[j] = KIND_FIX;
+            A.lround[j] = next;
+            A.plist[atomicAdd(&A.scal[0], 1)] = j;
+            const bool tr = pred_trapped && A.walked[j - 1] == A.round;
+            A.tflag[j] = tr ? A.round : -1;
+            if (tr) atomicAdd(&A.scal[12], 1);
+        }
+    }
+    if (!grid_last_block(reinterpret_cast<unsigned int*>(A.scal + 15), &last)) return;
+
     const int ntrig = A.scal[12];
     if (!ntrig) return;
-    const int32_t next = A.round + 1;
-    __shared__ int32_t trig[RESPEC_MAX_TRIGGERS];
-    __shared__ int32_t wsum[RESPEC_T / 64 + 1];
     {
-        const int32_t per = (A.C + RESPEC_T - 1) / RESPEC_T, c0 = (int32_t)threadIdx.x * per;
+        const int32_t per = (A.C + RT_T - 1) / RT_T, c0 = (int32_t)threadIdx.x * per;
         int cnt = 0;
         for (int32_t q = c0; q < c0 + per && q < A.C; q++) cnt += A.tflag[q] == A.round && A.lround[q] == next;
         const int incl = wave_incl_add<int>(cnt);
@@ -1035,8 +1062,8 @@
         __syncthreads();
         if (threadIdx.x == 0) {
             int run = 0;
-            for (int i = 0; i < RESPEC_T / 64; i++) { const int x = wsum[i]; wsum[i] = run; run += x; }
-            wsum[RESPEC_T / 64] = run;
+            for (int i = 0; i < RT_T / 64; i++) { const int x = wsum[i]; wsum[i] = run; run += x; }
+            wsum[RT_T / 64] = run;
         }
         __syncthreads();
         int at = wsum[w] + incl - cnt;
@@ -1044,13 +1071,13 @@
             if (A.tflag[q] == A.round && A.lround[q] == next) trig[at++] = q;
         __syncthreads();
     }
-    const int nt = wsum[RESPEC_T / 64] < RESPEC_MAX_TRIGGERS ? wsum[RESPEC_T / 64] : RESPEC_MAX_TRIGGERS;
+    const int nt = wsum[RT_T / 64] < RESPEC_MAX_TRIGGERS ? wsum[RT_T / 64] : RESPEC_MAX_TRIGGERS;
     const int w = (int)(threadIdx.x >> 6), nw = (int)(blockDim.x >> 6), lane = lane_id();
     for (int t = w; t < nt; t += nw) {
-        const int32_t j = trig[t], P = A.snapP[j];
-        for (int32_t q0 = j + 1; q0 <= j + RESPEC_AHEAD && q0 < A.C; q0 += 64) {
+        const int32_t jt = trig[t], P = A.snapP[jt];
+        for (int32_t q0 = jt + 1; q0 <= jt + RESPEC_AHEAD && q0 < A.C; q0 += 64) {
             const int32_t q = q0 + lane;
-            const bool ok = q < A.C && q <= j + RESPEC_AHEAD && A.lround[q] != next;
+            const bool ok = q < A.C && q <= jt + RESPEC_AHEAD && A.lround[q] != next;
             const unsigned long long okm = __ballot(ok);
             const unsigned long long run = ~okm ? okm & ((1ull << first_lane(~okm)) - 1) : okm;
             if ((run >> lane) & 1ull) {
@@ -1066,9 +1093,7 @@
 
 int launch_round_end(const WalkPtrs& A, int fbase, int fcap, hipStream_t s) {
     hipLaunchKernelGGL(k_round_fill, dim3(1), dim3(FROZEN_MAX), 0, s, A, fbase, fcap);
-    if (fcap > 0) hipLaunchKernelGGL(k_round_fillg, dim3(grid_for(A.C, 256)), dim3(256), 0, s, A);
-    hipLaunchKernelGGL(k_round_pending, dim3(grid_for(A.C, 256)), dim3(256), 0, s, A);
-    hipLaunchKernelGGL(k_round_respec, dim3(1), dim3(RESPEC_T), 0, s, A);
+    hipLaunchKernelGGL(k_round_close, dim3(grid_for(A.C, RT_T)), dim3(RT_T), 0, s, A);
     SCCG_HIP(hipGetLastError());
     return 0;
 }
@@ -1790,7 +1815,7 @@
 }
 __global__ __launch_bounds__(SCCG_BLOCK) void k_cand_stats(WalkPtrs A) {
     __shared__ CandBest wbest[SCCG_BLOCK / 64];
-    __shared__ int ok;
+    __shared__ int ok, last;
     const int k = A.k;
     const unsigned long long cnt = A.fc[13];
     if (threadIdx.x < 64) {
@@ -1818,19 +1843,11 @@
         unsigned long long* o = A.fcb + 4 * blockIdx.x;
         o[0] = v.l; o[1] = v.cnt; o[2] = v.has0; o[3] = v.minkey;
     }
-}
-
-__global__ __launch_bounds__(1024) void k_cand_stats_fin(WalkPtrs A, int nblk) {
-    __shared__ CandBest wbest[16];
-    __shared__ int ok;
-    if (threadIdx.x < 64) {
-        const bool u = cand_stats_usable(A);
-        if (threadIdx.x == 0) { ok = u; A.fc[12] = u ? 1 : 2; }
-    }
-    __syncthreads();
+    if (!grid_last_block(reinterpret_cast<unsigned int*>(A.fc + 14), &last)) return;
+    if (threadIdx.x == 0) A.fc[12] = ok ? 1 : 2;
     if (!ok) return;
-    CandBest v{0, 0, 0, ~0ull};
-    for (int b = (int)threadIdx.x; b < nblk; b += (int)blockDim.x) {
+    v = CandBest{0, 0, 0, ~0ull};
+    for (int b = (int)threadIdx.x; b < (int)gridDim.x; b += SCCG_BLOCK) {
         const unsigned long long* o = A.fcb + 4 * b;
         v = cb_merge(v, CandBest{(uint32_t)o[0], (uint32_t)o[1], (uint32_t)o[2], o[3]});
     }
@@ -1838,7 +1855,7 @@
     if (lane_id() == 0) wbest[threadIdx.x >> 6] = v;
     __syncthreads();
     if (threadIdx.x == 0) {
-        for (int i = 1; i < (int)(blockDim.x >> 6); i++) v = cb_merge(v, wbest[i]);
+        for (int i = 1; i < SCCG_BLOCK / 64; i++) v = cb_merge(v, wbest[i]);
         A.fc[8] = v.l; A.fc[9] = v.cnt; A.fc[10] = v.has0; A.fc[11] = v.minkey;
         A.fc[4] = v.cnt ? 0ull : ~0ull;
         A.fc[5] = ~0ull;
@@ -2466,7 +2483,8 @@
 void global_prepare_reset() { g_prep = Prepared{}; g_early = Early{}; }
 
 int global_sweep_early(const uint8_t* Rp, int64_t nRp, const int64_t* d_nRp, const uint8_t* tgt_fa, int64_t tn,
-                       const int64_t* d_hdr, int k, int m, int chunk, void* ws, size_t ws_bytes, hipStream_t s) {
+                       const int64_t* d_hdr, int k, int m, int chunk, void* ws, size_t ws_bytes, hipStream_t s_head,
+                       hipEvent_t ev_head, hipStream_t s) {
     g_early = Early{};
     if (m < 0 || 2 * m + 1 > WCAP || k > KMAX || k < 1) return SCCG_E_UNSUPPORTED;
     if (nRp < k || tn <= 0) return 0;
@@ -2474,9 +2492,11 @@
     WalkPtrs A = make_ptrs(Rp, nRp, nullptr, tn, k, m, chunk, ws, ws_bytes, &used);
     if (used > ws_bytes) return SCCG_E_INTERNAL;
     A.dnR = d_nRp;
-    RC(anchor_generation(A, ws, s));
-    RC(set_u64(A.fc + 12, {0, 0}, s));
-    hipLaunchKernelGGL(k_first_kmer, dim3(1), dim3(SCCG_BLOCK), 0, s, tgt_fa, tn, d_hdr, k, (int64_t)1 << 20, A.kb);
+    RC(anchor_generation(A, ws, s_head));
+    RC(set_u64(A.fc + 12, {0, 0, 0}, s_head));
+    hipLaunchKernelGGL(k_first_kmer, dim3(1), dim3(SCCG_BLOCK), 0, s_head, tgt_fa, tn, d_hdr, k, (int64_t)1 << 20, A.kb);
+    SCCG_HIP(hipEventRecord(ev_head, s_head));
+    SCCG_HIP(hipStreamWaitEvent(s, ev_head, 0));
     PROF_LAUNCH(PROF_ANCHOR, s, k_sweep_early, dim3(first_sweep_grid(A)), dim3(SCCG_BLOCK), 0, s, A);
     SCCG_HIP(hipGetLastError());
     g_early = Early{ws, Rp, nRp, k, A.agen, A.abits};
@@ -2497,7 +2517,6 @@
         A.agen = e.agen;
         if (A.nR >= A.k && A.nT >= A.k) {
             hipLaunchKernelGGL(k_cand_stats, dim3(CAND_STATS_GRID), dim3(SCCG_BLOCK), 0, s, A);
-            hipLaunchKernelGGL(k_cand_stats_fin, dim3(1), dim3(1024), 0, s, A, CAND_STATS_GRID);
             SCCG_HIP(hipGetLastError());
         }
     } else {
@@ -2569,7 +2588,6 @@
     if (dev_nlist) RC(launch_carry(A, s));
     hipLaunchKernelGGL(k_commit, dim3(grid_for(A.C, 256) > 4096 ? 4096 : grid_for(A.C, 256)), dim3(256), 0, s, A,
                        (const int32_t*)A.plist, A.C, nd);
-    hipLaunchKernelGGL(k_list_sort, dim3(1), dim3(LS_T), 0, s, A, A.flist, (const int32_t*)(A.scal + 5), A.fbits);
     if (fbase_cap > 0) hipLaunchKernelGGL(k_frozen_scan, dim3(FZ_GRID, fbase_cap), dim3(FZ_T), 0, s, A, 0);
     SCCG_HIP(hipGetLastError());
     RC(launch_round_end(A, 0, fbase_cap, s));
@@ -2725,7 +2743,6 @@
             if (nlist < A.C) RC(launch_carry(A, s));
             hipLaunchKernelGGL(k_commit, dim3(grid_for(nlist, 256) > 4096 ? 4096 : grid_for(nlist, 256)), dim3(256), 0, s, A,
                                (const int32_t*)A.plist, nlist, (const int32_t*)nullptr);
-            hipLaunchKernelGGL(k_list_sort, dim3(1), dim3(LS_T), 0, s, A, A.flist, (const int32_t*)(A.scal + 5), A.fbits);
         }
         res->rounds = round;
         int32_t rs[6];
@@ -2773,7 +2790,6 @@
                 RC(dev_set_i32(A.scal + 5, 1, {0}, s));
                 hipLaunchKernelGGL(k_commit, dim3(grid_for(nr, 256) > 4096 ? 4096 : grid_for(nr, 256)), dim3(256), 0, s, A,
                                    (const int32_t*)A.rlist, nr, (const int32_t*)nullptr);
-                hipLaunchKernelGGL(k_list_sort, dim3(1), dim3(LS_T), 0, s, A, A.flist, (const int32_t*)(A.scal + 5), A.fbits);
                 SCCG_HIP(hipGetLastError());
             }
             {
```

Measured after the change: 189.3 billion, median of 6. 3.2% higher.
